# callmeray/PointMVSNet

Hardware: NVIDIA H100
Metric: PointFlow iters/sec (higher is better)
Workload: dtype f32

## Files before the change

include/pmvs_b200.h:

```cpp
#ifndef PMVS_B200_H_
#define PMVS_B200_H_

#include <stddef.h>
#include <stdint.h>

#ifdef __cplusplus
extern "C" {
#endif

#define PMVS_OK 0
#define PMVS_ERR_ARG 1
#define PMVS_ERR_CUDA 2
#define PMVS_ERR_WORKSPACE 3

#define PMVS_NUM_HYP 5
#define PMVS_FEAT_CH 136
#define PMVS_KNN 16
#define PMVS_MAX_VIEWS 12

typedef void* pmvs_stream_t;

int pmvs_version(void);
const char* pmvs_last_error(void);
unsigned long long pmvs_launch_count(void);

int pmvs_set_gemm_mode(int mode);
int pmvs_get_gemm_mode(void);

#define PMVS_OPT_EDGE 1
#define PMVS_OPT_KNN 2
#define PMVS_OPT_FETCH 3
#define PMVS_OPT_GEMM 4
#define PMVS_OPT_DEBUG_IDX 5
#define PMVS_OPT_GEMM_STRICT 6
int pmvs_set_option(int key, int value);
int pmvs_get_option(int key);

int pmvs_profile_enable(int on);
int pmvs_profile_collect(char* names, size_t names_bytes, float* ms, int max_records);

int pmvs_gather_knn_forward(const float* input, const int64_t* index, float* output,
                            int B, int C, int N, int K, pmvs_stream_t stream);
int pmvs_gather_knn_backward(const float* grad_output, const int64_t* index, float* grad_input,
                             int B, int C, int N, int K, pmvs_stream_t stream);
size_t pmvs_gather_knn_backward_det_workspace_bytes(int B, int N, int K);
int pmvs_gather_knn_backward_det(const float* grad_output, const int64_t* index, float* grad_input,
                                 int B, int C, int N, int K, void* workspace, size_t workspace_bytes,
                                 pmvs_stream_t stream);

int pmvs_knn3d(const float* xyz, int64_t* idx64, int32_t* idx32, int B, int D, int H, int W,
               int ksize, int knn, pmvs_stream_t stream);

int pmvs_feature_fetch(const float* feature_maps, const float* pts, const float* intrinsics,
                       const float* extrinsics, float* out, int B, int V, int C, int H, int W,
                       int N, pmvs_stream_t stream);
int pmvs_feature_fetch_backward(const float* grad_out, const float* pts, const float* intrinsics,
                                const float* extrinsics, float* grad_maps, int B, int V, int C,
                                int H, int W, int N, pmvs_stream_t stream);
size_t pmvs_feature_fetch_backward_det_workspace_bytes(int B, int V, int C, int H, int W, int N);
int pmvs_feature_fetch_backward_det(const float* grad_out, const float* pts, const float* intrinsics,
                                    const float* extrinsics, float* grad_maps, int B, int V, int C, int H, int W, int N,
                                    void* workspace, size_t workspace_bytes, pmvs_stream_t stream);
int pmvs_feature_fetch_taps(const float* pts, const float* intrinsics, const float* extrinsics, int64_t* texel,
                            float* weight, int B, int V, int H, int W, int N, pmvs_stream_t stream);

int pmvs_cost_volume(const float* features, const float* cam_params, float* cost, void* workspace,
                     size_t workspace_bytes, int B, int V, int C, int h, int w, int D, int is_test,
                     pmvs_stream_t stream);

size_t pmvs_cost_volume_backward_workspace_bytes(int B, int V, int C, int h, int w, int D);
int pmvs_cost_volume_backward(const float* features, const float* cam_params, const float* grad_cost,
                              float* grad_features, void* workspace, size_t workspace_bytes, int B, int V, int C,
                              int h, int w, int D, int is_test, pmvs_stream_t stream);

size_t pmvs_fuse_depth_maps_workspace_bytes(int V, int H, int W);
int pmvs_fuse_depth_maps(const float* depth, const float* cam_block, int V, int H, int W, int num_consistent,
                         float depth_thresh, float reproj_thresh, int* count_out, float* xyz_out,
                         unsigned char* used_out, void* workspace, size_t workspace_bytes, pmvs_stream_t stream);

size_t pmvs_thin_cloud_workspace_bytes(int n);
int pmvs_thin_cloud(const float* xyz, const int64_t* order, int n, float dst, float cell, int first_round, int rounds,
                    int* state, int* undecided, void* workspace, size_t workspace_bytes, pmvs_stream_t stream);
size_t pmvs_nearest_distances_workspace_bytes(int nt);
int pmvs_nearest_distances(const float* query, int nq, const float* target, int nt, float max_dist, float cell,
                           float* dist, void* workspace, size_t workspace_bytes, pmvs_stream_t stream);
int pmvs_cloud_filter(const float* xyz, int n, const float* bb, float margin, const unsigned char* obs_mask,
                      const int* mask_dims, float res, const float* plane, unsigned char* flags,
                      pmvs_stream_t stream);

typedef struct pmvs_conv_bn_weights {
  const float* weight[11];
  const float* gamma[10];
  const float* beta[10];
  const float* running_mean[10];
  const float* running_var[10];
  float eps[10];
} pmvs_conv_bn_weights;

typedef struct pmvs_conv_bn_grads {
  float* weight[11];
  float* gamma[10];
  float* beta[10];
} pmvs_conv_bn_grads;

typedef pmvs_conv_bn_weights pmvs_volume_weights;

size_t pmvs_volume_conv_workspace_bytes(int B, int in_channels, int base_channels, int D, int H, int W);
int pmvs_volume_conv(const float* x, const pmvs_volume_weights* weights, int train, float* out, double* batch_sums,
                     void* workspace, size_t workspace_bytes, int B, int in_channels, int base_channels, int D, int H,
                     int W, pmvs_stream_t stream);
int pmvs_coarse_depth(const float* filtered, const float* cams, int B, int V, int D, int H, int W, float* depth_out,
                      float* prob_out, pmvs_stream_t stream);

typedef pmvs_conv_bn_weights pmvs_image_weights;

size_t pmvs_image_conv_workspace_bytes(int B, int V, int H, int W, int base_channels);
int pmvs_image_conv(const float* img, const pmvs_image_weights* weights, int train, float* const* level_out,
                    int channels_last, double* batch_sums, void* workspace, size_t workspace_bytes, int B, int V,
                    int H, int W, int base_channels, pmvs_stream_t stream);

size_t pmvs_image_conv_keep_workspace_bytes(int B, int V, int H, int W, int base_channels);
int pmvs_image_conv_keep(const float* img, const pmvs_image_weights* weights, int train, float* const* level_out,
                         int channels_last, double* batch_sums, void* workspace, size_t workspace_bytes, int B, int V,
                         int H, int W, int base_channels, pmvs_stream_t stream);

typedef pmvs_conv_bn_grads pmvs_image_grads;

size_t pmvs_image_conv_backward_workspace_bytes(int B, int V, int H, int W, int base_channels);
int pmvs_image_conv_backward(const float* img, const pmvs_image_weights* weights, int train, const void* fwd_workspace,
                             const double* batch_sums, const float* const* grad_level, int channels_last,
                             const pmvs_image_grads* grads, void* workspace, size_t workspace_bytes, int B, int V,
                             int H, int W, int base_channels, pmvs_stream_t stream);

typedef pmvs_conv_bn_grads pmvs_volume_grads;

size_t pmvs_volume_conv_backward_workspace_bytes(int B, int in_channels, int base_channels, int D, int H, int W);
int pmvs_volume_conv_backward(const float* x, const pmvs_volume_weights* weights, int train,
                              const void* fwd_workspace, const double* batch_sums, const float* grad_out,
                              float* grad_x , const pmvs_volume_grads* grads, void* workspace,
                              size_t workspace_bytes, int B, int in_channels, int base_channels, int D, int H, int W,
                              pmvs_stream_t stream);
int pmvs_coarse_depth_backward(const float* filtered, const float* cams, const float* grad_depth,
                               float* grad_filtered, int B, int V, int D, int H, int W, pmvs_stream_t stream);

int pmvs_transpose(const float* in, float* out, int batch, int R, int C, pmvs_stream_t stream);
int pmvs_idx64_to_idx32(const int64_t* in, int32_t* out, long long n, pmvs_stream_t stream);

int pmvs_edgeconv_pm(const float* x, int ldx, const int32_t* idx32, const float* w12,
                     const float* gamma, const float* beta, float eps, int concat_central,
                     int bn_train, float* out, int ldo, float* le_scratch, double* stats_scratch,
                     int groups, int rows_per_group, int N, int K, int cin, int cout,
                     pmvs_stream_t stream);

size_t pmvs_edgeconv_pm_backward_workspace_bytes(int B, int N, int K, int cin, int cout);
int pmvs_edgeconv_pm_backward(const float* x, int ldx, const int32_t* idx32, const int64_t* idx64,
                              const float* w12, const float* gamma, const float* beta, float eps,
                              int concat_central, int bn_train, const float* le, const double* stats,
                              const float* dy, int lddy, float* dx, int lddx, float* dw12,
                              float* dgamma, float* dbeta, void* workspace, size_t workspace_bytes,
                              int B, int N, int K, int cin, int cout, pmvs_stream_t stream);

int pmvs_linear_pm(const float* x, int ldx, const float* w, float* y, int ldy, int groups,
                   int rows_per_group, int cin, int cout, const double* in_stats,
                   const float* in_gamma, const float* in_beta, double in_count, float eps,
                   double* out_stats, pmvs_stream_t stream);

typedef struct pmvs_flow_weights {
  const float* ec_w12[3];
  const float* ec_gamma[3];
  const float* ec_beta[3];
  const float* mlp_w[4];
  const float* mlp_gamma[3];
  const float* mlp_beta[3];
  float* ec_run_mean[3];
  float* ec_run_var[3];
  float* mlp_run_mean[3];
  float* mlp_run_var[3];
  float momentum;
  float eps;
  long long* ec_nbt[3];
  long long* mlp_nbt[3];
} pmvs_flow_weights;

typedef struct pmvs_flow_shape {
  int B;
  int V;
  int pyr_h[3], pyr_w[3];
  int prev_h, prev_w;
  int flow_h, flow_w;
  float image_scale;
  int ratio;
  int is_test;
  float interval_scale;
  int sub_begin, sub_count;
} pmvs_flow_shape;

size_t pmvs_point_flow_workspace_bytes(const pmvs_flow_shape* shape);

int pmvs_point_flow_iter(const pmvs_flow_shape* shape, const pmvs_flow_weights* weights,
                         const float* const pyramids_cl[3], const float* depth_prev,
                         const float* cam_params, const float* interval, const float* mean,
                         const float* std, float* depth_out, float* prob_out, void* workspace,
                         size_t workspace_bytes, pmvs_stream_t stream);

int pmvs_pyramid_to_channels_last(const float* nchw, float* nhwc, int BV, int C, int h, int w,
                                  pmvs_stream_t stream);

int pmvs_point_flow_debug_offsets(const pmvs_flow_shape* shape, size_t off[10]);

int pmvs_point_flow_debug_feature(const pmvs_flow_shape* shape, const float* depth_prev, void* workspace,
                                  pmvs_stream_t stream);

typedef struct pmvs_flow_grads {
  float* ec_dw12[3];
  float* ec_dgamma[3];
  float* ec_dbeta[3];
  float* mlp_dw[4];
  float* mlp_dgamma[3];
  float* mlp_dbeta[3];
  float* dpyramids_cl[3];
  float* ddepth_prev;
} pmvs_flow_grads;

size_t pmvs_point_flow_backward_workspace_bytes(const pmvs_flow_shape* shape);

int pmvs_point_flow_backward(const pmvs_flow_shape* shape, const pmvs_flow_weights* weights,
                             const float* const pyramids_cl[3], const float* depth_prev,
                             const float* cam_params, const float* interval, const float* mean,
                             const float* std, const void* fwd_workspace, const float* grad_depth_out,
                             const float* grad_prob_out, const pmvs_flow_grads* grads, void* workspace,
                             size_t workspace_bytes, pmvs_stream_t stream);

typedef struct pmvs_depth_terms {
  const float* pred[3];
  int h[3], w[3];
  int T;
} pmvs_depth_terms;

int pmvs_depth_loss(const pmvs_depth_terms* terms, const float* gt, int Hg, int Wg, const float* cams, int B, int V,
                    float valid_threshold, float* loss_out, float* metric_out, double* stats, pmvs_stream_t stream);
int pmvs_depth_loss_backward(const pmvs_depth_terms* terms, const float* gt, int Hg, int Wg, const float* cams, int B,
                             int V, const double* stats, const float* grad_loss, float* const grad_pred[3],
                             pmvs_stream_t stream);

#ifdef __cplusplus
}
#endif
#endif
```

pointmvsnet_b200/_lib.py:

```python
import ctypes as C
import os

import torch

_HERE = os.path.dirname(os.path.abspath(__file__))
LIB_PATH = os.path.join(_HERE, "libpmvs_b200.so")

if not os.path.exists(LIB_PATH):
    raise ImportError(
        "pointmvsnet_b200: %s is missing -- build it with pointmvsnet_b200/csrc/build.sh "
        "(nvcc, sm_90a).  There is no CPU fallback." % LIB_PATH)

lib = C.CDLL(LIB_PATH)

c_float_p = C.c_void_p
c_stream = C.c_void_p


class FlowWeights(C.Structure):
    _fields_ = [
        ("ec_w12", C.c_void_p * 3), ("ec_gamma", C.c_void_p * 3), ("ec_beta", C.c_void_p * 3),
        ("mlp_w", C.c_void_p * 4), ("mlp_gamma", C.c_void_p * 3), ("mlp_beta", C.c_void_p * 3),
        ("ec_run_mean", C.c_void_p * 3), ("ec_run_var", C.c_void_p * 3),
        ("mlp_run_mean", C.c_void_p * 3), ("mlp_run_var", C.c_void_p * 3),
        ("momentum", C.c_float), ("eps", C.c_float),
        ("ec_nbt", C.c_void_p * 3), ("mlp_nbt", C.c_void_p * 3),
    ]


class FlowShape(C.Structure):
    _fields_ = [
        ("B", C.c_int), ("V", C.c_int), ("pyr_h", C.c_int * 3), ("pyr_w", C.c_int * 3),
        ("prev_h", C.c_int), ("prev_w", C.c_int), ("flow_h", C.c_int), ("flow_w", C.c_int),
        ("image_scale", C.c_float), ("ratio", C.c_int), ("is_test", C.c_int), ("interval_scale", C.c_float),
        ("sub_begin", C.c_int), ("sub_count", C.c_int),
    ]


class FlowGrads(C.Structure):
    _fields_ = [
        ("ec_dw12", C.c_void_p * 3), ("ec_dgamma", C.c_void_p * 3), ("ec_dbeta", C.c_void_p * 3),
        ("mlp_dw", C.c_void_p * 4), ("mlp_dgamma", C.c_void_p * 3), ("mlp_dbeta", C.c_void_p * 3),
        ("dpyramids_cl", C.c_void_p * 3), ("ddepth_prev", C.c_void_p),
    ]


class ConvBnWeights(C.Structure):
    _fields_ = [
        ("weight", C.c_void_p * 11), ("gamma", C.c_void_p * 10), ("beta", C.c_void_p * 10),
        ("running_mean", C.c_void_p * 10), ("running_var", C.c_void_p * 10), ("eps", C.c_float * 10),
    ]


class ConvBnGrads(C.Structure):
    _fields_ = [("weight", C.c_void_p * 11), ("gamma", C.c_void_p * 10), ("beta", C.c_void_p * 10)]


VolumeWeights = ImageWeights = ConvBnWeights
VolumeGrads = ImageGrads = ConvBnGrads


class DepthTerms(C.Structure):
    _fields_ = [("pred", C.c_void_p * 3), ("h", C.c_int * 3), ("w", C.c_int * 3), ("T", C.c_int)]


def _sig(name, restype, argtypes):
    fn = getattr(lib, name)
    fn.restype = restype
    fn.argtypes = argtypes
    return fn


P, I, LL, F = C.c_void_p, C.c_int, C.c_longlong, C.c_float
_sig("pmvs_version", I, [])
_sig("pmvs_last_error", C.c_char_p, [])
_sig("pmvs_launch_count", C.c_ulonglong, [])
_sig("pmvs_set_gemm_mode", I, [I])
_sig("pmvs_get_gemm_mode", I, [])
_sig("pmvs_set_option", I, [I, I])
_sig("pmvs_get_option", I, [I])
_sig("pmvs_profile_enable", I, [I])
_sig("pmvs_profile_collect", I, [C.c_char_p, C.c_size_t, P, I])
_sig("pmvs_gather_knn_forward", I, [P, P, P, I, I, I, I, P])
_sig("pmvs_gather_knn_backward", I, [P, P, P, I, I, I, I, P])
_sig("pmvs_gather_knn_backward_det_workspace_bytes", C.c_size_t, [I, I, I])
_sig("pmvs_gather_knn_backward_det", I, [P, P, P, I, I, I, I, P, C.c_size_t, P])
_sig("pmvs_knn3d", I, [P, P, P, I, I, I, I, I, I, P])
_sig("pmvs_feature_fetch", I, [P, P, P, P, P, I, I, I, I, I, I, P])
_sig("pmvs_feature_fetch_backward", I, [P, P, P, P, P, I, I, I, I, I, I, P])
_sig("pmvs_feature_fetch_backward_det_workspace_bytes", C.c_size_t, [I, I, I, I, I, I])
_sig("pmvs_feature_fetch_backward_det", I, [P, P, P, P, P, I, I, I, I, I, I, P, C.c_size_t, P])
_sig("pmvs_feature_fetch_taps", I, [P, P, P, P, P, I, I, I, I, I, P])
_sig("pmvs_cost_volume", I, [P, P, P, P, C.c_size_t, I, I, I, I, I, I, I, P])
_sig("pmvs_cost_volume_backward_workspace_bytes", C.c_size_t, [I, I, I, I, I, I])
_sig("pmvs_cost_volume_backward", I, [P, P, P, P, P, C.c_size_t, I, I, I, I, I, I, I, P])
_sig("pmvs_fuse_depth_maps_workspace_bytes", C.c_size_t, [I, I, I])
_sig("pmvs_fuse_depth_maps", I, [P, P, I, I, I, I, F, F, P, P, P, P, C.c_size_t, P])
_sig("pmvs_thin_cloud_workspace_bytes", C.c_size_t, [I])
_sig("pmvs_thin_cloud", I, [P, P, I, F, F, I, I, P, P, P, C.c_size_t, P])
_sig("pmvs_nearest_distances_workspace_bytes", C.c_size_t, [I])
_sig("pmvs_nearest_distances", I, [P, I, P, I, F, F, P, P, C.c_size_t, P])
_sig("pmvs_cloud_filter", I, [P, I, P, F, P, P, F, P, P, P])
_sig("pmvs_volume_conv_workspace_bytes", C.c_size_t, [I, I, I, I, I, I])
_sig("pmvs_volume_conv", I, [P, C.POINTER(ConvBnWeights), I, P, P, P, C.c_size_t, I, I, I, I, I, I, P])
_sig("pmvs_coarse_depth", I, [P, P, I, I, I, I, I, P, P, P])
_sig("pmvs_volume_conv_backward_workspace_bytes", C.c_size_t, [I, I, I, I, I, I])
_sig("pmvs_volume_conv_backward", I, [P, C.POINTER(ConvBnWeights), I, P, P, P, P, C.POINTER(ConvBnGrads), P,
                                      C.c_size_t, I, I, I, I, I, I, P])
_sig("pmvs_coarse_depth_backward", I, [P, P, P, P, I, I, I, I, I, P])
_sig("pmvs_image_conv_workspace_bytes", C.c_size_t, [I, I, I, I, I])
_sig("pmvs_image_conv", I, [P, C.POINTER(ConvBnWeights), I, C.POINTER(C.c_void_p * 4), I, P, P, C.c_size_t, I, I, I,
                            I, I, P])
_sig("pmvs_image_conv_keep_workspace_bytes", C.c_size_t, [I, I, I, I, I])
_sig("pmvs_image_conv_keep", I, [P, C.POINTER(ConvBnWeights), I, C.POINTER(C.c_void_p * 4), I, P, P, C.c_size_t, I,
                                 I, I, I, I, P])
_sig("pmvs_image_conv_backward_workspace_bytes", C.c_size_t, [I, I, I, I, I])
_sig("pmvs_image_conv_backward", I, [P, C.POINTER(ConvBnWeights), I, P, P, C.POINTER(C.c_void_p * 4), I,
                                     C.POINTER(ConvBnGrads), P, C.c_size_t, I, I, I, I, I, P])
_sig("pmvs_transpose", I, [P, P, I, I, I, P])
_sig("pmvs_idx64_to_idx32", I, [P, P, LL, P])
_sig("pmvs_edgeconv_pm", I, [P, I, P, P, P, P, F, I, I, P, I, P, P, I, I, I, I, I, I, P])
_sig("pmvs_edgeconv_pm_backward_workspace_bytes", C.c_size_t, [I, I, I, I, I])
_sig("pmvs_edgeconv_pm_backward", I, [P, I, P, P, P, P, P, F, I, I, P, P, P, I, P, I, P, P, P, P, C.c_size_t,
                                      I, I, I, I, I, P])
_sig("pmvs_linear_pm", I, [P, I, P, P, I, I, I, I, I, P, P, P, C.c_double, F, P, P])
_sig("pmvs_point_flow_workspace_bytes", C.c_size_t, [C.POINTER(FlowShape)])
_sig("pmvs_point_flow_iter", I, [C.POINTER(FlowShape), C.POINTER(FlowWeights), C.POINTER(C.c_void_p * 3),
                                 P, P, P, P, P, P, P, P, C.c_size_t, P])
_sig("pmvs_pyramid_to_channels_last", I, [P, P, I, I, I, I, P])
_sig("pmvs_point_flow_debug_offsets", I, [C.POINTER(FlowShape), C.POINTER(C.c_size_t * 10)])
_sig("pmvs_point_flow_debug_feature", I, [C.POINTER(FlowShape), P, P, P])
_sig("pmvs_point_flow_backward_workspace_bytes", C.c_size_t, [C.POINTER(FlowShape)])
_sig("pmvs_point_flow_backward", I, [C.POINTER(FlowShape), C.POINTER(FlowWeights), C.POINTER(C.c_void_p * 3),
                                     P, P, P, P, P, P, P, P, C.POINTER(FlowGrads), P, C.c_size_t, P])
_sig("pmvs_depth_loss", I, [C.POINTER(DepthTerms), P, I, I, P, I, I, F, P, P, P, P])
_sig("pmvs_depth_loss_backward", I, [C.POINTER(DepthTerms), P, I, I, P, I, I, P, P, C.POINTER(C.c_void_p * 3), P])

EXPORTED = [
    "pmvs_version", "pmvs_last_error", "pmvs_launch_count", "pmvs_set_option", "pmvs_get_option", "pmvs_profile_enable", "pmvs_profile_collect", "pmvs_set_gemm_mode", "pmvs_get_gemm_mode", "pmvs_gather_knn_forward",
    "pmvs_gather_knn_backward", "pmvs_gather_knn_backward_det_workspace_bytes", "pmvs_gather_knn_backward_det", "pmvs_knn3d", "pmvs_feature_fetch", "pmvs_feature_fetch_backward",
    "pmvs_feature_fetch_backward_det_workspace_bytes", "pmvs_feature_fetch_backward_det", "pmvs_feature_fetch_taps",
    "pmvs_cost_volume", "pmvs_cost_volume_backward_workspace_bytes", "pmvs_cost_volume_backward",
    "pmvs_fuse_depth_maps_workspace_bytes", "pmvs_fuse_depth_maps", "pmvs_thin_cloud_workspace_bytes",
    "pmvs_thin_cloud", "pmvs_nearest_distances_workspace_bytes", "pmvs_nearest_distances", "pmvs_cloud_filter",
    "pmvs_volume_conv_workspace_bytes", "pmvs_volume_conv", "pmvs_coarse_depth",
    "pmvs_volume_conv_backward_workspace_bytes", "pmvs_volume_conv_backward", "pmvs_coarse_depth_backward",
    "pmvs_image_conv_workspace_bytes", "pmvs_image_conv", "pmvs_image_conv_keep_workspace_bytes",
    "pmvs_image_conv_keep", "pmvs_image_conv_backward_workspace_bytes", "pmvs_image_conv_backward",
    "pmvs_transpose", "pmvs_idx64_to_idx32", "pmvs_edgeconv_pm", "pmvs_edgeconv_pm_backward_workspace_bytes", "pmvs_edgeconv_pm_backward", "pmvs_linear_pm", "pmvs_point_flow_workspace_bytes",
    "pmvs_point_flow_iter", "pmvs_pyramid_to_channels_last", "pmvs_point_flow_debug_offsets",
    "pmvs_point_flow_debug_feature", "pmvs_point_flow_backward_workspace_bytes", "pmvs_point_flow_backward",
    "pmvs_depth_loss", "pmvs_depth_loss_backward",
]


def check(rc):
    if rc != 0:
        raise RuntimeError("libpmvs_b200: " + lib.pmvs_last_error().decode("utf-8", "replace"))


def stream_ptr():
    return torch.cuda.current_stream().cuda_stream


def ptr(t):
    return None if t is None else t.data_ptr()


def require_cuda(*tensors):
    for t in tensors:
        if t is not None and not t.is_cuda:
            raise RuntimeError("pointmvsnet_b200 operators need CUDA tensors (sm_90a); there is no CPU fallback")


def f32c(t):
    if t.dtype != torch.float32:
        t = t.float()
    return t.contiguous()


def workspace(nbytes, device):
    if nbytes == 0:
        check(1)
    return torch.empty(nbytes, device=device, dtype=torch.uint8)


def launch_count():
    return int(lib.pmvs_launch_count())


def profile_enable(on):
    lib.pmvs_profile_enable(1 if on else 0)


def profile_collect(max_records=65536):
    names = C.create_string_buffer(max_records * 24)
    ms = (C.c_float * max_records)()
    n = lib.pmvs_profile_collect(names, len(names), C.cast(ms, C.c_void_p), max_records)
    nm = names.value.decode().split("\n")[:n]
    return [(nm[i], float(ms[i])) for i in range(n)]


def set_gemm_mode(mode):
    check(lib.pmvs_set_gemm_mode(int(mode)))


OPTIONS = {"edge": 1, "knn": 2, "fetch": 3, "gemm": 4, "debug_idx": 5, "gemm_strict": 6}


def set_option(name, value):
    check(lib.pmvs_set_option(OPTIONS[name], int(value)))


def get_option(name):
    return int(lib.pmvs_get_option(OPTIONS[name]))


def _options_from_env():
    spec = os.environ.get("PMVS_OPTIONS", "")
    for item in spec.split(","):
        if "=" in item:
            k, v = item.split("=", 1)
            set_option(k.strip(), int(v))


_options_from_env()
```

pointmvsnet_b200/csrc/api.cu:

```cuda
#include <algorithm>
#include <atomic>
#include <cstdarg>
#include <mutex>
#include <vector>

#include "common.cuh"

namespace pmvs {

static thread_local char g_err[512] = "";
static std::atomic<unsigned long long> g_launches{0};

void set_error(const char* fmt, ...) {
  va_list ap;
  va_start(ap, fmt);
  vsnprintf(g_err, sizeof(g_err), fmt, ap);
  va_end(ap);
}
void count_launch(int n) { g_launches.fetch_add((unsigned long long)n, std::memory_order_relaxed); }

static std::atomic<int> g_opt[OPT_COUNT];
static struct OptDefaults {
  OptDefaults() {
    g_opt[OPT_EDGE].store(1);
    g_opt[OPT_KNN].store(1);
    g_opt[OPT_FETCH].store(3);
    g_opt[OPT_GEMM].store(3);
  }
} g_opt_defaults;
int opt(int key) { return (key >= 0 && key < OPT_COUNT) ? g_opt[key].load(std::memory_order_relaxed) : 0; }

struct ProfRec {
  const char* name;
  cudaEvent_t a, b;
};
static std::mutex g_prof_mu;
static std::vector<ProfRec> g_prof;
static std::atomic<int> g_prof_on{0};
static thread_local int g_prof_open = -1;

void prof_begin(const char* what, cudaStream_t st) {
  if (!g_prof_on.load(std::memory_order_relaxed)) return;
  ProfRec r;
  r.name = what;
  if (cudaEventCreate(&r.a) != cudaSuccess || cudaEventCreate(&r.b) != cudaSuccess) return;
  cudaEventRecord(r.a, st);
  std::lock_guard<std::mutex> lk(g_prof_mu);
  g_prof.push_back(r);
  g_prof_open = (int)g_prof.size() - 1;
}
void prof_end(cudaStream_t st) {
  if (g_prof_open < 0) return;
  std::lock_guard<std::mutex> lk(g_prof_mu);
  if (g_prof_open < (int)g_prof.size()) cudaEventRecord(g_prof[g_prof_open].b, st);
  g_prof_open = -1;
}

__global__ void __launch_bounds__(256) transpose_kernel(const float* __restrict__ in, float* __restrict__ out, int R,
                                                        int C) {
  __shared__ float tile[32][33];
  const size_t boff = (size_t)blockIdx.z * R * C;
  const int c0 = blockIdx.x * 32, r0 = blockIdx.y * 32;
  const int tx = threadIdx.x & 31, ty = threadIdx.x >> 5;
#pragma unroll
  for (int j = 0; j < 32; j += 8) {
    const int r = r0 + ty + j, c = c0 + tx;
    if (r < R && c < C) tile[ty + j][tx] = __ldg(in + boff + (size_t)r * C + c);
  }
  __syncthreads();
#pragma unroll
  for (int j = 0; j < 32; j += 8) {
    const int c = c0 + ty + j, r = r0 + tx;
    if (r < R && c < C) out[boff + (size_t)c * R + r] = tile[tx][ty + j];
  }
}

int launch_transpose(const float* in, float* out, int batch, int R, int C, cudaStream_t st) {
  PMVS_REQUIRE(in && out && batch > 0 && R > 0 && C > 0, "transpose: bad arguments");
  PMVS_REQUIRE(batch <= 65535 && cdiv(R, 32) <= 65535, "transpose: shape too large");
  dim3 grid(cdiv(C, 32), cdiv(R, 32), batch);
  prof_begin("transpose", st);
  transpose_kernel<<<grid, 256, 0, st>>>(in, out, R, C);
  return check_launch("transpose_kernel", st);
}

__global__ void idx_convert_kernel(const int64_t* __restrict__ in, int32_t* __restrict__ out, long long n) {
  for (long long i = blockIdx.x * (long long)blockDim.x + threadIdx.x; i < n; i += (long long)gridDim.x * blockDim.x)
    out[i] = (int32_t)in[i];
}

__global__ void __launch_bounds__(256)
    gather_fwd_kernel(const float* __restrict__ in, const int64_t* __restrict__ idx, float* __restrict__ out, int C,
                      int N, int K, long long total) {
  for (long long o = blockIdx.x * (long long)blockDim.x + threadIdx.x; o < total;
       o += (long long)gridDim.x * blockDim.x) {
    const int k = (int)(o % K);
    long long t = o / K;
    const int n = (int)(t % N);
    t /= N;
    const long long b = t / C;
    const int64_t j = idx[(b * N + n) * K + k];
    out[o] = (j >= 0 && j < N) ? __ldg(in + t * N + j) : 0.f;
  }
}
__global__ void __launch_bounds__(256)
    gather_bwd_kernel(const float* __restrict__ gout, const int64_t* __restrict__ idx, float* __restrict__ gin, int C,
                      int N, int K, long long total) {
  for (long long o = blockIdx.x * (long long)blockDim.x + threadIdx.x; o < total;
       o += (long long)gridDim.x * blockDim.x) {
    const int k = (int)(o % K);
    long long t = o / K;
    const int n = (int)(t % N);
    t /= N;
    const long long b = t / C;
    const int64_t j = idx[(b * N + n) * K + k];
    if (j >= 0 && j < N) atomicAdd(gin + t * N + j, gout[o]);
  }
}

struct FlowPlan {
  int S, hs, ws, N;
  int sub_begin;
  size_t R;
  size_t cam, feature, xyz, idx, le, ecat, h0, h1, h2, stats, total;
  size_t warp_src;
  size_t cand;
  size_t st_ec[3], st_ecn[3], st_mlp[3];
  size_t st_ticket;
  size_t stats_doubles;
  size_t coef;
};

static int make_plan(const pmvs_flow_shape* s, FlowPlan& p) {
  PMVS_REQUIRE(s != nullptr, "point_flow: NULL shape");
  PMVS_REQUIRE(s->B > 0 && s->V > 0 && s->V <= PMVS_MAX_VIEWS, "point_flow: B=%d V=%d (V <= %d)", s->B, s->V,
               PMVS_MAX_VIEWS);
  PMVS_REQUIRE(s->ratio >= 1 && s->flow_h > 0 && s->flow_w > 0, "point_flow: bad flow size / ratio");
  PMVS_REQUIRE(s->flow_h % s->ratio == 0 && s->flow_w % s->ratio == 0,
               "point_flow: flow size %dx%d not divisible by ratio %d", s->flow_h, s->flow_w, s->ratio);
  PMVS_REQUIRE(s->prev_h > 0 && s->prev_w > 0, "point_flow: bad previous depth size");
  for (int l = 0; l < 3; ++l) PMVS_REQUIRE(s->pyr_h[l] > 0 && s->pyr_w[l] > 0, "point_flow: bad pyramid size");
  PMVS_REQUIRE(s->flow_h > 1 && s->flow_w > 1, "point_flow: flow size must be > 1");
  const int s_all = s->ratio * s->ratio;
  PMVS_REQUIRE(s->sub_count >= 0 && s->sub_begin >= 0 && s->sub_begin + s->sub_count <= s_all &&
                   (s->sub_count > 0 || s->sub_begin == 0),
               "point_flow: sub-cloud range [%d, %d) outside the %d sub-clouds", s->sub_begin,
               s->sub_begin + s->sub_count, s_all);
  p.S = s->sub_count > 0 ? s->sub_count : s_all;
  p.sub_begin = s->sub_begin;
  p.hs = s->flow_h / s->ratio;
  p.ws = s->flow_w / s->ratio;
  p.N = PMVS_NUM_HYP * p.hs * p.ws;
  p.R = (size_t)p.S * s->B * p.N;
  PMVS_REQUIRE(p.R * 224 < (size_t)1 << 40, "point_flow: problem too large");
  size_t o = 0;
  p.cam = o; o += up256(cam_block_bytes(s->B, s->V));
  p.feature = o; o += up256(p.R * PMVS_FEAT_CH * 4);
  p.xyz = o; o += up256(p.R * 3 * 4);
  p.idx = o; o += up256(p.R * PMVS_KNN * 4);
  p.le = o; o += up256(p.R * 128 * 4);
  p.ecat = o; o += up256(p.R * 224 * 4);
  p.h0 = o; o += up256(p.R * 64 * 4);
  p.h1 = o; o += up256(p.R * 64 * 4);
  p.h2 = o; o += up256(p.R * 16 * 4);
  p.warp_src = o; o += up256(warp_source_bytes(s->B, s->V, s->flow_h, s->flow_w));
  p.cand = o; o += up256(p.R * PMVS_KNN * 2);
  size_t d = 0;
  const int ec_cout[3] = {32, 32, 64};
  const int mlp_cout[3] = {64, 64, 16};
  for (int l = 0; l < 3; ++l) {
    p.st_ec[l] = d; d += (size_t)p.S * 4 * ec_cout[l];
    p.st_ecn[l] = d; d += (size_t)p.S * 2 * ec_cout[l];
  }
  for (int l = 0; l < 3; ++l) { p.st_mlp[l] = d; d += (size_t)p.S * 2 * mlp_cout[l]; }
  p.st_ticket = d; d += (3 * (size_t)p.S + 1) / 2 + 1;
  p.stats_doubles = d;
  p.stats = o; o += up256(d * 8);
  p.coef = o; o += up256(3 * (size_t)p.S * 6 * 64 * sizeof(float));
  p.total = o;
  return PMVS_OK;
}

static FusedFetchParams fetch_params(const pmvs_flow_shape* s, const FlowPlan& p, char* ws, const float* depth_prev) {
  FusedFetchParams f{};
  f.src = (const float*)(ws + p.warp_src);
  f.depth_prev = depth_prev; f.cam_blocks = (const float*)(ws + p.cam); f.feature = (float*)(ws + p.feature);
  f.xyz = (float*)(ws + p.xyz);
  f.B = s->B; f.V = s->V; f.h = s->flow_h; f.w = s->flow_w; f.hp = s->prev_h; f.wp = s->prev_w;
  f.ratio = s->ratio; f.sub_begin = p.sub_begin; f.sub_count = p.S;
  return f;
}

int flow_regions(const pmvs_flow_shape* s, FlowRegions& r) {
  FlowPlan p;
  PMVS_TRY(make_plan(s, p));
  r.cam = p.cam; r.feature = p.feature; r.xyz = p.xyz; r.idx = p.idx; r.le = p.le; r.ecat = p.ecat; r.h0 = p.h0;
  r.h1 = p.h1; r.h2 = p.h2; r.warp_src = p.warp_src; r.cand = p.cand; r.stats = p.stats; r.coef = p.coef;
  r.total = p.total;
  for (int l = 0; l < 3; ++l) { r.st_ec[l] = p.st_ec[l]; r.st_ecn[l] = p.st_ecn[l]; r.st_mlp[l] = p.st_mlp[l]; }
  r.S = p.S;
  return PMVS_OK;
}

}

using namespace pmvs;

extern "C" int pmvs_version(void) { return 100; }
extern "C" const char* pmvs_last_error(void) { return g_err; }
extern "C" unsigned long long pmvs_launch_count(void) { return g_launches.load(); }

extern "C" int pmvs_set_option(int key, int value) {
  PMVS_REQUIRE(key > 0 && key < OPT_COUNT, "set_option: unknown key %d", key);
  g_opt[key].store(value);
  return PMVS_OK;
}
extern "C" int pmvs_get_option(int key) { return opt(key); }

extern "C" int pmvs_profile_enable(int on) {
  g_prof_on.store(on ? 1 : 0);
  return PMVS_OK;
}

extern "C" int pmvs_profile_collect(char* names, size_t names_bytes, float* ms, int max_records) {
  std::lock_guard<std::mutex> lk(g_prof_mu);
  int n = 0;
  size_t pos = 0;
  if (names && names_bytes) names[0] = 0;
  for (auto& r : g_prof) {
    float t = -1.f;
    if (cudaEventSynchronize(r.b) == cudaSuccess) cudaEventElapsedTime(&t, r.a, r.b);
    if (n < max_records && ms && names) {
      const size_t len = strlen(r.name);
      if (pos + len + 2 < names_bytes) {
        memcpy(names + pos, r.name, len);
        pos += len;
        names[pos++] = '\n';
        names[pos] = 0;
        ms[n++] = t;
      }
    }
    cudaEventDestroy(r.a);
    cudaEventDestroy(r.b);
  }
  g_prof.clear();
  return n;
}

extern "C" int pmvs_transpose(const float* in, float* out, int batch, int R, int C, pmvs_stream_t stream) {
  return launch_transpose(in, out, batch, R, C, (cudaStream_t)stream);
}

extern "C" int pmvs_pyramid_to_channels_last(const float* nchw, float* nhwc, int BV, int C, int h, int w,
                                             pmvs_stream_t stream) {
  PMVS_REQUIRE((long long)h * w < (1ll << 31), "pyramid_to_channels_last: plane too large");
  return launch_transpose(nchw, nhwc, BV, C, h * w, (cudaStream_t)stream);
}

extern "C" int pmvs_idx64_to_idx32(const int64_t* in, int32_t* out, long long n, pmvs_stream_t stream) {
  PMVS_REQUIRE(in && out && n >= 0, "idx64_to_idx32: bad arguments");
  if (n == 0) return PMVS_OK;
  idx_convert_kernel<<<(int)std::min<long long>(cdiv(n, 256), sm_count() * 8), 256, 0, (cudaStream_t)stream>>>(in, out, n);
  return check_launch("idx_convert_kernel");
}

extern "C" int pmvs_gather_knn_forward(const float* input, const int64_t* index, float* output, int B, int C, int N,
                                       int K, pmvs_stream_t stream) {
  PMVS_REQUIRE(B >= 0 && C >= 0 && N >= 0 && K >= 0, "gather_knn_forward: negative size");
  const long long total = (long long)B * C * N * K;
  if (total == 0) return PMVS_OK;
  PMVS_REQUIRE(input && index && output, "gather_knn_forward: NULL pointer");
  const int grid = (int)std::min<long long>(cdiv(total, 256), sm_count() * 16);
  gather_fwd_kernel<<<grid, 256, 0, (cudaStream_t)stream>>>(input, index, output, C, N, K, total);
  return check_launch("gather_fwd_kernel");
}

extern "C" int pmvs_gather_knn_backward(const float* grad_output, const int64_t* index, float* grad_input, int B,
                                        int C, int N, int K, pmvs_stream_t stream) {
  PMVS_REQUIRE(B >= 0 && C >= 0 && N >= 0 && K >= 0, "gather_knn_backward: negative size");
  if ((long long)B * C * N == 0) return PMVS_OK;
  PMVS_REQUIRE(grad_output && index && grad_input, "gather_knn_backward: NULL pointer");
  cudaStream_t st = (cudaStream_t)stream;
  PMVS_TRY(memset_async("gather_knn_backward", grad_input, (size_t)B * C * N * sizeof(float), st));
  const long long total = (long long)B * C * N * K;
  if (total == 0) return PMVS_OK;
  const int grid = (int)std::min<long long>(cdiv(total, 256), sm_count() * 16);
  gather_bwd_kernel<<<grid, 256, 0, st>>>(grad_output, index, grad_input, C, N, K, total);
  return check_launch("gather_bwd_kernel");
}

extern "C" int pmvs_edgeconv_pm(const float* x, int ldx, const int32_t* idx32, const float* w12, const float* gamma,
                                const float* beta, float eps, int concat_central, int bn_train, float* out, int ldo,
                                float* le_scratch, double* stats_scratch, int groups, int rows_per_group, int N,
                                int K, int cin, int cout, pmvs_stream_t stream) {
  PMVS_REQUIRE(x && idx32 && w12 && gamma && beta && out && le_scratch && stats_scratch, "edgeconv: NULL pointer");
  PMVS_REQUIRE(groups > 0 && rows_per_group > 0 && N > 0 && K > 0, "edgeconv: bad sizes");
  cudaStream_t st = (cudaStream_t)stream;
  if (bn_train) PMVS_TRY(memset_async("edgeconv", stats_scratch, (size_t)groups * 4 * cout * sizeof(double), st));
  GemmArgs g{};
  g.x = x; g.ldx = ldx; g.w = w12; g.y = le_scratch; g.ldy = 2 * cout;
  g.groups = groups; g.rows_per_group = rows_per_group; g.cin = cin; g.cout = 2 * cout; g.eps = eps;
  PMVS_TRY(launch_gemm(g, st));
  EdgeArgs e{};
  e.le = le_scratch; e.idx = idx32; e.stats = stats_scratch; e.gamma = gamma; e.beta = beta; e.eps = eps;
  e.concat_central = concat_central; e.out = out; e.ldo = ldo; e.groups = groups;
  e.rows_per_group = rows_per_group; e.N = N; e.K = K; e.cout = cout;
  if (bn_train) PMVS_TRY(launch_edge_stats(e, st));
  PMVS_TRY(launch_edge_apply(e, st));
  return PMVS_OK;
}

extern "C" int pmvs_linear_pm(const float* x, int ldx, const float* w, float* y, int ldy, int groups,
                              int rows_per_group, int cin, int cout, const double* in_stats, const float* in_gamma,
                              const float* in_beta, double in_count, float eps, double* out_stats,
                              pmvs_stream_t stream) {
  PMVS_REQUIRE(x && w && y, "linear_pm: NULL pointer");
  PMVS_REQUIRE(groups > 0 && rows_per_group > 0 && cin > 0 && cout > 0, "linear_pm: bad sizes");
  PMVS_REQUIRE(in_stats == nullptr || (in_gamma && in_beta && in_count > 0), "linear_pm: incomplete input BN");
  GemmArgs g{};
  g.x = x; g.ldx = ldx; g.w = w; g.y = y; g.ldy = ldy; g.groups = groups; g.rows_per_group = rows_per_group;
  g.cin = cin; g.cout = cout; g.in_stats = in_stats; g.in_gamma = in_gamma; g.in_beta = in_beta;
  g.in_count = in_count; g.eps = eps; g.out_stats = out_stats;
  return launch_gemm(g, (cudaStream_t)stream);
}

extern "C" size_t pmvs_point_flow_workspace_bytes(const pmvs_flow_shape* shape) {
  FlowPlan p;
  if (make_plan(shape, p) != PMVS_OK) return 0;
  return p.total;
}

extern "C" int pmvs_point_flow_debug_offsets(const pmvs_flow_shape* shape, size_t off[10]) {
  FlowPlan p;
  PMVS_TRY(make_plan(shape, p));
  off[0] = p.feature; off[1] = p.xyz; off[2] = p.idx; off[3] = p.ecat; off[4] = p.h2;
  off[5] = p.le; off[6] = p.stats; off[7] = p.total;
  off[8] = p.cand;
  off[9] = (opt(OPT_EDGE) == 0 || opt(OPT_DEBUG_IDX) != 0) ? 1 : 0;
  return PMVS_OK;
}

extern "C" int pmvs_point_flow_debug_feature(const pmvs_flow_shape* shape, const float* depth_prev, void* workspace,
                                             pmvs_stream_t stream) {
  FlowPlan p;
  PMVS_TRY(make_plan(shape, p));
  PMVS_REQUIRE(depth_prev && workspace, "point_flow_debug_feature: NULL pointer");
  return launch_fused_fetch(fetch_params(shape, p, (char*)workspace, depth_prev), (cudaStream_t)stream);
}

extern "C" int pmvs_point_flow_iter(const pmvs_flow_shape* shape, const pmvs_flow_weights* wts,
                                    const float* const pyramids_cl[3], const float* depth_prev,
                                    const float* cam_params, const float* interval, const float* mean,
                                    const float* stdv, float* depth_out, float* prob_out, void* workspace,
                                    size_t workspace_bytes, pmvs_stream_t stream) {
  FlowPlan p;
  PMVS_TRY(make_plan(shape, p));
  PMVS_REQUIRE(wts && pyramids_cl && depth_prev && cam_params && interval && mean && stdv && depth_out && workspace,
               "point_flow: NULL pointer");
  PMVS_TRY(check_workspace("point_flow", workspace, workspace_bytes, p.total));
  cudaStream_t st = (cudaStream_t)stream;
  char* ws = (char*)workspace;
  float* cam = (float*)(ws + p.cam);
  const float* feature = (const float*)(ws + p.feature);
  const float* xyz = (const float*)(ws + p.xyz);
  int32_t* idx = (int32_t*)(ws + p.idx);
  float* le = (float*)(ws + p.le);
  float* ecat = (float*)(ws + p.ecat);
  float* h0 = (float*)(ws + p.h0);
  float* h1 = (float*)(ws + p.h1);
  float* h2 = (float*)(ws + p.h2);
  double* stats = (double*)(ws + p.stats);
  const int B = shape->B, S = p.S;
  const int rows_per_group = B * p.N;

  PMVS_TRY(memset_async("point_flow", stats, p.stats_doubles * sizeof(double), st));
  const float kscale = shape->is_test ? shape->image_scale : (float)(4.0 * (double)shape->image_scale);
  PMVS_TRY(launch_cam_setup(cam_params, interval, mean, stdv, cam, B, shape->V, kscale, shape->interval_scale, st));

  float* warp_src = (float*)(ws + p.warp_src);
  PMVS_TRY(launch_warp_source(pyramids_cl, shape->pyr_h, shape->pyr_w, warp_src, B, shape->V, shape->flow_h,
                              shape->flow_w, st));
  const int edge_impl = opt(OPT_EDGE);
  const FusedFetchParams f = fetch_params(shape, p, ws, depth_prev);
  bool fused_le0 = false;
  if (opt(OPT_FETCH) == 3 && opt(OPT_GEMM) == 3 && pmvs_get_gemm_mode() == 3 && edge_impl != 0) {
    const int rc = launch_fetch_gemm(f, wts->ec_w12[0], le, st);
    if (rc > 0) return rc;
    fused_le0 = rc == 0;
    if (!fused_le0 && opt(OPT_GEMM_STRICT)) {
      set_error("point_flow: fetch_gemm_kernel does not take V=%d (strict mode)", shape->V);
      return PMVS_ERR_ARG;
    }
  }
  if (!fused_le0) PMVS_TRY(launch_fused_fetch(f, st));

  unsigned short* cand = (unsigned short*)(ws + p.cand);
  if (edge_impl != 0)
    PMVS_TRY(launch_knn3d_cand(xyz, opt(OPT_DEBUG_IDX) ? idx : nullptr, cand, S * B, PMVS_NUM_HYP, p.hs, p.ws, st));
  else
    PMVS_TRY(launch_knn3d(xyz, nullptr, idx, S * B, PMVS_NUM_HYP, p.hs, p.ws, PMVS_NUM_HYP, PMVS_KNN, st));

  const int cin[3] = {136, 32, 64}, cout[3] = {32, 32, 64}, in_off[3] = {0, 0, 32}, out_off[3] = {0, 32, 96};
  for (int l = 0; l < 3; ++l) {
    GemmArgs g{};
    g.x = l == 0 ? feature : ecat + in_off[l];
    g.ldx = l == 0 ? PMVS_FEAT_CH : 224;
    g.w = wts->ec_w12[l]; g.y = le; g.ldy = 2 * cout[l];
    g.groups = S; g.rows_per_group = rows_per_group; g.cin = cin[l]; g.cout = 2 * cout[l]; g.eps = wts->eps;
    if (edge_impl != 0 && l > 0) g.out_stats = stats + p.st_ec[l];
    if (l > 0 || !fused_le0) PMVS_TRY(launch_gemm(g, st));
    if (edge_impl != 0) {
      EdgeTileArgs e{};
      e.le = le; e.cand = cand; e.cstats = stats + p.st_ec[l]; e.nstats = stats + p.st_ecn[l];
      e.coef = (float*)(ws + p.coef) + (size_t)l * S * 6 * 64;
      e.ticket = (unsigned*)(stats + p.st_ticket) + (size_t)l * S;
      e.gamma = wts->ec_gamma[l]; e.beta = wts->ec_beta[l]; e.eps = wts->eps; e.concat_central = l > 0;
      e.out = ecat + out_off[l]; e.ldo = 224; e.groups = S; e.clouds_per_group = B; e.gh = p.hs; e.gw = p.ws;
      e.cout = cout[l];
      const int tile_w = edge_impl == 2 ? 16 : 8;
      PMVS_TRY(launch_edge_tile_stats(e, tile_w, st));
      PMVS_TRY(launch_edge_tile_apply(e, tile_w, st));
    } else {
      EdgeArgs e{};
      e.le = le; e.idx = idx; e.stats = stats + p.st_ec[l]; e.gamma = wts->ec_gamma[l]; e.beta = wts->ec_beta[l];
      e.eps = wts->eps; e.concat_central = l > 0; e.out = ecat + out_off[l]; e.ldo = 224; e.groups = S;
      e.rows_per_group = rows_per_group; e.N = p.N; e.K = PMVS_KNN; e.cout = cout[l];
      PMVS_TRY(launch_edge_stats(e, st));
      PMVS_TRY(launch_edge_apply(e, st));
    }
  }

  {
    const float* xin[3] = {ecat, h0, h1};
    float* yout[3] = {h0, h1, h2};
    const int mcin[3] = {224, 64, 64}, mcout[3] = {64, 64, 16};
    for (int l = 0; l < 3; ++l) {
      GemmArgs g{};
      g.x = xin[l]; g.ldx = mcin[l]; g.w = wts->mlp_w[l]; g.y = yout[l]; g.ldy = mcout[l];
      g.groups = S; g.rows_per_group = rows_per_group; g.cin = mcin[l]; g.cout = mcout[l]; g.eps = wts->eps;
      if (l > 0) {
        g.in_stats = stats + p.st_mlp[l - 1]; g.in_gamma = wts->mlp_gamma[l - 1]; g.in_beta = wts->mlp_beta[l - 1];
        g.in_count = (double)rows_per_group;
      }
      g.out_stats = stats + p.st_mlp[l];
      PMVS_TRY(launch_gemm(g, st));
    }
  }
  HeadArgs h{};
  h.h2 = h2; h.stats = stats + p.st_mlp[2]; h.gamma = wts->mlp_gamma[2]; h.beta = wts->mlp_beta[2];
  h.w3 = wts->mlp_w[3]; h.depth_prev = depth_prev; h.interval = interval; h.depth_out = depth_out;
  h.prob_out = prob_out; h.eps = wts->eps; h.interval_scale = shape->interval_scale; h.B = B; h.S = S; h.ratio = shape->ratio; h.sub_begin = p.sub_begin; h.h = shape->flow_h;
  h.w = shape->flow_w; h.hp = shape->prev_h; h.wp = shape->prev_w;
  PMVS_TRY(launch_flow_head(h, st));

  RunUpdateBatch rb{};
  rb.groups = S; rb.momentum = wts->momentum;
  for (int l = 0; l < 3; ++l) {
    if (wts->ec_run_mean[l] && wts->ec_run_var[l]) {
      const int c = cout[l];
      const double* sl = stats + p.st_ec[l];
      const bool tile = edge_impl != 0;
      if (l > 0) {
        RunUpdate& u = rb.u[rb.n++];
        u.stats = sl; u.run_mean = wts->ec_run_mean[l]; u.run_var = wts->ec_run_var[l]; u.C = c;
        u.off_sum = 0; u.off_sq = tile ? 2 * c : c; u.gstride = 4 * c; u.count = (double)rows_per_group;
        u.ncorr = (double)rows_per_group * PMVS_KNN;
      }
      RunUpdate& u = rb.u[rb.n++];
      u.run_mean = wts->ec_run_mean[l] + (l > 0 ? c : 0); u.run_var = wts->ec_run_var[l] + (l > 0 ? c : 0);
      u.C = c;
      if (tile) {
        u.stats = stats + p.st_ecn[l]; u.off_sum = 0; u.off_sq = c; u.gstride = 2 * c;
      } else {
        u.stats = sl; u.off_sum = 2 * c; u.off_sq = 3 * c; u.gstride = 4 * c;
      }
      u.count = (double)rows_per_group * PMVS_KNN;
      u.ncorr = u.count; u.nbt = wts->ec_nbt[l];
    }
  }
  const int mcout2[3] = {64, 64, 16};
  for (int l = 0; l < 3; ++l) {
    if (wts->mlp_run_mean[l] && wts->mlp_run_var[l]) {
      RunUpdate& u = rb.u[rb.n++];
      u.stats = stats + p.st_mlp[l]; u.run_mean = wts->mlp_run_mean[l]; u.run_var = wts->mlp_run_var[l];
      u.C = mcout2[l]; u.off_sum = 0; u.off_sq = mcout2[l]; u.gstride = 2 * mcout2[l];
      u.count = (double)rows_per_group; u.ncorr = u.count; u.nbt = wts->mlp_nbt[l];
    }
  }
  PMVS_TRY(launch_bn_running_update(rb, st));
  return PMVS_OK;
}
```

pointmvsnet_b200/csrc/common.cuh:

```cuda
#pragma once
#include <cuda_runtime.h>
#include <float.h>
#include <stdint.h>
#include <stdio.h>
#include <string.h>

#include "../../include/pmvs_b200.h"

namespace pmvs {

void set_error(const char* fmt, ...);
void count_launch(int n = 1);

void prof_begin(const char* what, cudaStream_t st);
void prof_end(cudaStream_t st);

inline int check_launch(const char* what, cudaStream_t st = nullptr) {
  cudaError_t e = cudaPeekAtLastError();
  if (e != cudaSuccess) {
    cudaGetLastError();
    set_error("%s: %s", what, cudaGetErrorString(e));
    return PMVS_ERR_CUDA;
  }
  prof_end(st);
  count_launch();
  return PMVS_OK;
}

#define PMVS_REQUIRE(cond, ...)     \
  do {                              \
    if (!(cond)) {                  \
      pmvs::set_error(__VA_ARGS__); \
      return PMVS_ERR_ARG;          \
    }                               \
  } while (0)

#define PMVS_TRY(expr)           \
  do {                           \
    int _rc = (expr);            \
    if (_rc != PMVS_OK) return _rc; \
  } while (0)

static inline int cdiv(long long a, long long b) { return (int)((a + b - 1) / b); }

inline size_t up256(size_t x) { return (x + 255) & ~(size_t)255; }

inline bool finite_nonneg(float t) { return t >= 0.f && t <= FLT_MAX; }

inline int check_workspace_size(const char* what, size_t bytes, size_t need) {
  if (bytes < need) {
    set_error("%s: workspace %zu bytes < required %zu", what, bytes, need);
    return PMVS_ERR_WORKSPACE;
  }
  return PMVS_OK;
}
inline int check_workspace(const char* what, const void* ws, size_t bytes, size_t need) {
  PMVS_REQUIRE(ws != nullptr && ((uintptr_t)ws & 255) == 0, "%s: workspace must be non-NULL and 256-byte aligned",
               what);
  return check_workspace_size(what, bytes, need);
}

inline int memset_async(const char* what, void* p, size_t bytes, cudaStream_t st) {
  if (bytes != 0 && cudaMemsetAsync(p, 0, bytes, st) != cudaSuccess) {
    cudaGetLastError();
    set_error("%s: cudaMemsetAsync failed", what);
    return PMVS_ERR_CUDA;
  }
  return PMVS_OK;
}

inline int sm_count() {
  static int n = 0;
  if (n == 0) {
    int dev = 0, v = 0;
    cudaGetDevice(&dev);
    n = (cudaDeviceGetAttribute(&v, cudaDevAttrMultiProcessorCount, dev) == cudaSuccess && v > 0) ? v : 132;
  }
  return n;
}

__device__ __forceinline__ float4 ldg4(const float* p) { return __ldg(reinterpret_cast<const float4*>(p)); }
__device__ __forceinline__ void st4(float* p, float4 v) { *reinterpret_cast<float4*>(p) = v; }

typedef float2 f32x2;
__device__ __forceinline__ f32x2 pack2(float a, float b) { return make_float2(a, b); }
__device__ __forceinline__ void unpack2(f32x2 v, float& a, float& b) { a = v.x; b = v.y; }
__device__ __forceinline__ f32x2 fma2(f32x2 a, f32x2 b, f32x2 c) { return make_float2(__fmaf_rn(a.x, b.x, c.x), __fmaf_rn(a.y, b.y, c.y)); }
__device__ __forceinline__ f32x2 add2(f32x2 a, f32x2 b) { return make_float2(__fadd_rn(a.x, b.x), __fadd_rn(a.y, b.y)); }
__device__ __forceinline__ f32x2 mul2(f32x2 a, f32x2 b) { return make_float2(__fmul_rn(a.x, b.x), __fmul_rn(a.y, b.y)); }
__device__ __forceinline__ f32x2 sub2(f32x2 a, f32x2 b) { return make_float2(__fsub_rn(a.x, b.x), __fsub_rn(a.y, b.y)); }

enum {
  OPT_EDGE = 1,
  OPT_KNN = 2,
  OPT_FETCH = 3,
  OPT_GEMM = 4,
  OPT_DEBUG_IDX = 5,
  OPT_GEMM_STRICT = 6,
  OPT_COUNT = 16
};
int opt(int key);

template <typename K>
inline int ensure_dyn_smem(K kernel, int bytes, unsigned long long& done_mask, const char* what) {
  int dev = 0;
  if (cudaGetDevice(&dev) != cudaSuccess || dev < 0 || dev > 63) dev = 0;
  if (done_mask & (1ull << dev)) return PMVS_OK;
  if (cudaFuncSetAttribute(kernel, cudaFuncAttributeMaxDynamicSharedMemorySize, bytes) != cudaSuccess) {
    cudaGetLastError();
    set_error("%s: cannot reserve %d bytes of shared memory", what, bytes);
    return PMVS_ERR_CUDA;
  }
  done_mask |= 1ull << dev;
  return PMVS_OK;
}

struct BnCoef {
  float mean, invstd;
};
__device__ __forceinline__ BnCoef bn_coef(double s1, double s2, double count, float eps) {
  double m = s1 / count;
  double var = s2 / count - m * m;
  if (var < 0.0) var = 0.0;
  BnCoef c;
  c.mean = (float)m;
  c.invstd = (float)(1.0 / sqrt(var + (double)eps));
  return c;
}
__device__ __forceinline__ float bn_apply(float x, float mean, float invstd, float g, float b) {
  return __fadd_rn(__fmul_rn(__fmul_rn(__fsub_rn(x, mean), invstd), g), b);
}
__device__ __forceinline__ float edge_nb_scale(float invstd, float gamma) { return __fmul_rn(invstd, gamma); }
__device__ __forceinline__ float edge_nb_offset(float mean, float local, float A, float beta) {
  return __fmaf_rn(-__fadd_rn(mean, local), A, beta);
}
__device__ __forceinline__ float edge_nb_pre(float e, float A, float c0) { return __fmaf_rn(e, A, c0); }

int launch_knn3d_cand(const float* xyz, int32_t* idx32, unsigned short* cand, int clouds, int D, int H, int W,
                      cudaStream_t st);
int launch_knn3d(const float* xyz, int64_t* idx64, int32_t* idx32, int clouds, int D, int H, int W,
                 int ksize, int knn, cudaStream_t st);
int launch_transpose(const float* in, float* out, int batch, int R, int C, cudaStream_t st);

struct GemmArgs {
  const float* x;
  int ldx;
  const float* w;
  float* y;
  int ldy;
  int groups, rows_per_group, cin, cout;
  const double* in_stats;
  const float* in_gamma;
  const float* in_beta;
  double in_count;
  float eps;
  double* out_stats;
};
int launch_gemm(const GemmArgs& a, cudaStream_t st);
int launch_gemm_tc(const GemmArgs& a, cudaStream_t st, const char* name);
int launch_gemm_ws(const GemmArgs& a, cudaStream_t st, const char* name);

struct EdgeArgs {
  const float* le;
  const int32_t* idx;
  double* stats;
  const float* gamma;
  const float* beta;
  float eps;
  int concat_central;
  float* out;
  int ldo;
  int groups, rows_per_group, N, K, cout;
};
int launch_edge_stats(const EdgeArgs& a, cudaStream_t st);
int launch_edge_apply(const EdgeArgs& a, cudaStream_t st);

size_t inv_lists_bytes(long long B, long long N, long long K);
int build_inv_lists(const int64_t* idx, int B, int N, int K, void* ws, const int** off, const int** list,
                    const char* prof_name, cudaStream_t st);
int launch_texel_sum(const int* off, const int* list, const float* rec_w, const float* g, float* out, int T, int nrec,
                     int B, int C, long long out_bstride, int out_tstride, const char* prof_name, cudaStream_t st);

struct EdgeLayerBwd {
  const float* x;
  int ldx;
  const int32_t* idx32;
  const int* inv_off;
  const int* inv_list;
  const float* w12;
  const float* gamma;
  const float* beta;
  float eps;
  int concat_central, bn_train;
  const float* le;
  const double* stats;
  const float* tile_coef;
  const float* dy;
  int lddy;
  float* dx;
  int lddx;
  float* dw12;
  float* dgamma;
  float* dbeta;
  float* dle;
  char* scratch;
  int B, N, K, cin, cout;
};
size_t edge_layer_bwd_scratch_bytes(long long R, int cin, int cout);
int edge_layer_backward(const EdgeLayerBwd& L, cudaStream_t st);
size_t weight_grad_scratch_bytes(long long R, int M2, int cin);
int launch_weight_grad(const float* dy, const float* x, int ldx, int cin, int M2, int R, float* wpart, float* dw,
                       const char* simt_name, cudaStream_t st);

struct EdgeTileArgs {
  const float* le;
  const unsigned short* cand;
  const double* cstats;
  double* nstats;
  float* coef;
  unsigned* ticket;
  const float* gamma;
  const float* beta;
  float eps;
  int concat_central;
  float* out;
  int ldo;
  int groups, clouds_per_group, gh, gw, cout;
};
int launch_edge_tile_stats(const EdgeTileArgs& a, int tile_w, cudaStream_t st);
int launch_edge_tile_apply(const EdgeTileArgs& a, int tile_w, cudaStream_t st);

struct FusedFetchParams {
  const float* src;
  const float* depth_prev;
  const float* cam_blocks;
  float* feature;
  float* xyz;
  int B, V, h, w, hp, wp, ratio;
  int sub_begin, sub_count;
  int ppw, hs, ws, rlog2;
};
int launch_warp_source(const float* const pyr[3], const int hl[3], const int wl[3], float* out, int B, int V, int h,
                       int w, cudaStream_t st);
size_t warp_source_bytes(int B, int V, int h, int w);
int launch_cam_setup(const float* cam_params, const float* interval, const float* mean, const float* stdv,
                     float* blocks, int B, int V, float kscale, float iscale, cudaStream_t st);
int launch_fused_fetch(const FusedFetchParams& p, cudaStream_t st);
int launch_fetch_gemm(const FusedFetchParams& p, const float* w12, float* le, cudaStream_t st);
size_t cam_block_bytes(int B, int V);
int cost_volume_check_shape(const char* what, int B, int V, int C, int h, int w, int D);
struct FetchBwdParams {
  FusedFetchParams f;
  const float* ddepth_out;
  float* ddup;
  float* dfv;
  int64_t* rec_idx;
  float* rec_w;
};
int launch_fetch_backward(const FetchBwdParams& p, cudaStream_t st);
int launch_warp_source_backward(const float* dsrc, const int hl[3], const int wl[3], float* const dpyr[3], int B, int V,
                                int h, int w, cudaStream_t st);

struct HeadArgs {
  const float* h2;
  const double* stats;
  const float* gamma;
  const float* beta;
  const float* w3;
  const float* depth_prev;
  const float* interval;
  float* depth_out;
  float* prob_out;
  float eps, interval_scale;
  int B, S, ratio, h, w, hp, wp;
  int sub_begin;
};
int launch_flow_head(const HeadArgs& a, cudaStream_t st);
struct FlowRegions {
  size_t cam, feature, xyz, idx, le, ecat, h0, h1, h2, warp_src, cand, stats, coef, total;
  size_t st_ec[3], st_ecn[3], st_mlp[3];
  int S;
};
int flow_regions(const pmvs_flow_shape* s, FlowRegions& r);
bool gemm_in_bn_fma_form(const GemmArgs& a);

struct RunUpdate {
  const double* stats;
  float* run_mean;
  float* run_var;
  int C, off_sum, off_sq, gstride;
  double count;
  double ncorr;
  long long* nbt;
};
struct RunUpdateBatch {
  RunUpdate u[9];
  int n, groups;
  float momentum;
};
int launch_bn_running_update(const RunUpdateBatch& rb, cudaStream_t st);

}
```

pointmvsnet_b200/csrc/edge_tile.cu:

```cuda
#include <algorithm>

#include "common.cuh"
#include "tensor_map.cuh"

namespace pmvs {

namespace {

constexpr int ET_THREADS = 256;
constexpr int ET_WARPS = ET_THREADS / 32;
constexpr int ET_CP = 32;
constexpr int ET_LPP = ET_CP / 4;
constexpr int ET_PPW = 32 / ET_LPP;

__device__ __forceinline__ unsigned smem_u32(const void* p) { return (unsigned)__cvta_generic_to_shared(p); }

template <int TX, int TY>
struct TileGeom {
  static constexpr int HX = TX + 4, HY = TY + 4;
  static constexpr int ROWS = PMVS_NUM_HYP * HY * HX;
  static constexpr int NPTS = PMVS_NUM_HYP * TY * TX;
  static constexpr int BYTES = ROWS * ET_CP * 4;
  static constexpr int SMEM = BYTES;
};

constexpr int ET_COEF = 6;

template <int COUT, bool APPLY, int TX, int TY>
__global__ void __launch_bounds__(ET_THREADS, 3) edge_tile_kernel(const __grid_constant__ CUtensorMap tm,
                                                                   const EdgeTileArgs a) {
  using G = TileGeom<TX, TY>;
  static_assert(COUT % ET_CP == 0, "edge_tile: channels must be a multiple of 32");
  static_assert(G::NPTS % (ET_WARPS * ET_PPW) == 0, "edge_tile: every thread owns NPTS / 32 points");
  constexpr int LD = 2 * COUT;
  constexpr int SLABS = COUT / ET_CP;
  constexpr int STEPS = G::NPTS / (ET_WARPS * ET_PPW);
  static_assert(G::HX == 12 && G::HY == 8, "the kNN kernel's 16-bit codes are row offsets of a 12 x 8 x 5 halo tile");
  extern __shared__ __align__(128) float halo[];
  __shared__ __align__(8) unsigned long long bar;
  __shared__ float part[APPLY ? 1 : ET_WARPS][APPLY ? 1 : 2 * ET_CP];
  __shared__ __align__(16) float coef[APPLY ? ET_COEF * COUT : 4];
  __shared__ int s_last;

  const int g = blockIdx.z;
  const int tid = threadIdx.x, warp = tid >> 5, lane = tid & 31;
  const int sub = lane / ET_LPP, cl = (lane % ET_LPP) * 4;
  const int gh = a.gh, gw = a.gw;
  const int tiles_x = (gw + TX - 1) / TX, tiles_per_cloud = tiles_x * ((gh + TY - 1) / TY);
  const int tiles_per_group = tiles_per_cloud * a.clouds_per_group;
  const int HW = gh * gw, N = PMVS_NUM_HYP * HW;
  const int rows_per_group = a.clouds_per_group * N;
  const unsigned bar_addr = smem_u32(&bar);

  if (tid == 0) {
    asm volatile("mbarrier.init.shared::cta.b64 [%0], 1;" ::"r"(bar_addr));
    asm volatile("fence.mbarrier_init.release.cluster;" ::: "memory");
  }
  if (APPLY) {
    const float* cg = a.coef + (size_t)g * ET_COEF * COUT;
    for (int c = tid; c < ET_COEF * COUT; c += ET_THREADS) coef[c] = __ldg(cg + c);
  }
  static_assert(TX * TY == ET_WARPS * ET_PPW && STEPS == PMVS_NUM_HYP, "edge_tile: one layer of the tile per step");
  const int tq = warp * ET_PPW + sub, tx = tq % TX, ty = tq / TX;
  const int pb0 = ((-2 * G::HY + ty) * G::HX + tx) * ET_CP + cl;
  constexpr int LAYER = G::HY * G::HX * ET_CP;
  __syncthreads();

  unsigned loads = 0;
#pragma unroll 1
  for (int slab = 0; slab < SLABS; ++slab) {
    const int ch0 = slab * ET_CP;
    f32x2 n1_lo = pack2(0.f, 0.f), n1_hi = n1_lo, n2_lo = n1_lo, n2_hi = n1_lo;
#pragma unroll 1
    for (int tile = blockIdx.x; tile < tiles_per_group; tile += gridDim.x) {
    const int b = tile / tiles_per_cloud, tr = tile - b * tiles_per_cloud;
    const int y0 = (tr / tiles_x) * TY, x0 = (tr % tiles_x) * TX;
    const size_t cloud_base = (size_t)g * rows_per_group + (size_t)b * N;
    const bool ok = y0 + ty < gh && x0 + tx < gw;
    const int pq = (y0 + ty) * gw + x0 + tx;
    auto load_codes = [&](int s, uint4& c0, uint4& c1) {
      if (ok) {
        const uint4* cp = reinterpret_cast<const uint4*>(a.cand + (cloud_base + (size_t)(s * HW + pq)) * PMVS_KNN);
        c0 = __ldg(cp);
        c1 = __ldg(cp + 1);
      } else {
        c0 = c1 = make_uint4(0u, 0u, 0u, 0u);
      }
    };
    if (loads > 0) __syncthreads();
    if (tid == 0) {
      asm volatile("mbarrier.arrive.expect_tx.shared::cta.b64 _, [%0], %1;" ::"r"(bar_addr), "r"((unsigned)G::BYTES)
                   : "memory");
      asm volatile(
          "cp.async.bulk.tensor.4d.shared::cluster.global.mbarrier::complete_tx::bytes [%0], [%1, {%2, %3, %4, %5}], [%6];"
          ::"r"(smem_u32(halo)), "l"(&tm), "r"(COUT + ch0), "r"(x0 - 2), "r"(y0 - 2),
          "r"((g * a.clouds_per_group + b) * PMVS_NUM_HYP), "r"(bar_addr)
          : "memory");
    }
    float4 loc[STEPS];
#pragma unroll
    for (int s = 0; s < STEPS; ++s)
      loc[s] = ok ? ldg4(a.le + (cloud_base + (size_t)(s * HW + pq)) * LD + ch0 + cl) : make_float4(0.f, 0.f, 0.f, 0.f);
    {
      unsigned done = 0;
      const unsigned parity = loads & 1u;
      while (!done) {
        asm volatile(
            "{\n\t.reg .pred p;\n\t"
            "mbarrier.try_wait.parity.shared::cta.b64 p, [%1], %2;\n\t"
            "selp.u32 %0, 1, 0, p;\n\t}"
            : "=r"(done)
            : "r"(bar_addr), "r"(parity)
            : "memory");
      }
      ++loads;
    }

    uint4 nx0, nx1;
    load_codes(0, nx0, nx1);
#pragma unroll
    for (int s = 0; s < STEPS; ++s) {
      const uint4 ca = nx0, cb = nx1;
      if (s + 1 < STEPS) load_codes(s + 1, nx0, nx1);
      if (!ok) continue;
      const int n = s * HW + pq;
      const size_t row = cloud_base + (size_t)n;
      const float4 lc = loc[s];
      const bool esc = ((ca.x | ca.y | ca.z | ca.w | cb.x | cb.y | cb.z | cb.w) & 0x80008000u) != 0u;
      const float* hbase = halo + pb0 + s * LAYER;
      f32x2 o_lo = pack2(0.f, 0.f), o_hi = o_lo, A_lo = o_lo, A_hi = o_lo, c_lo = o_lo, c_hi = o_lo;
      const f32x2 l_lo = pack2(lc.x, lc.y), l_hi = pack2(lc.z, lc.w);
      if (APPLY) {
        const float4 A4 = *reinterpret_cast<const float4*>(&coef[ch0 + cl]);
        const float4 B4 = *reinterpret_cast<const float4*>(&coef[COUT + ch0 + cl]);
        A_lo = pack2(A4.x, A4.y); A_hi = pack2(A4.z, A4.w);
        c_lo = pack2(fmaf(-lc.x, A4.x, B4.x), fmaf(-lc.y, A4.y, B4.y));
        c_hi = pack2(fmaf(-lc.z, A4.z, B4.z), fmaf(-lc.w, A4.w, B4.w));
      }
      auto body = [&](const float4 e) {
        const f32x2 e_lo = pack2(e.x, e.y), e_hi = pack2(e.z, e.w);
        if (APPLY) {
          float t0, t1f, t2, t3;
          unpack2(fma2(e_lo, A_lo, c_lo), t0, t1f);
          unpack2(fma2(e_hi, A_hi, c_hi), t2, t3);
          o_lo = add2(o_lo, pack2(fmaxf(t0, 0.f), fmaxf(t1f, 0.f)));
          o_hi = add2(o_hi, pack2(fmaxf(t2, 0.f), fmaxf(t3, 0.f)));
        } else {
          const f32x2 d_lo = sub2(e_lo, l_lo), d_hi = sub2(e_hi, l_hi);
          n1_lo = add2(n1_lo, d_lo); n1_hi = add2(n1_hi, d_hi);
          n2_lo = fma2(d_lo, d_lo, n2_lo); n2_hi = fma2(d_hi, d_hi, n2_hi);
        }
      };
      auto code_of = [&](int k) -> unsigned {
        const int wq = k >> 1;
        const unsigned wd = wq == 0 ? ca.x : wq == 1 ? ca.y : wq == 2 ? ca.z : wq == 3 ? ca.w
                          : wq == 4 ? cb.x : wq == 5 ? cb.y : wq == 6 ? cb.z : cb.w;
        return (k & 1) ? wd >> 16 : wd & 0xffffu;
      };
      if (!esc) {
#pragma unroll
        for (int k = 0; k < PMVS_KNN; ++k) body(*reinterpret_cast<const float4*>(hbase + code_of(k) * ET_CP));
      } else {
#pragma unroll 1
        for (int k = 0; k < PMVS_KNN; ++k) {
          const unsigned c = code_of(k);
          if (c & 0x8000u) {
            const int j = (int)(c & 127u);
            int t = n + (j / 25 - 2) * HW + ((j % 25) / 5 - 2) * gw + (j % 5 - 2);
            t = t < 0 ? 0 : (t > N - 1 ? N - 1 : t);
            body(ldg4(a.le + (cloud_base + (size_t)t) * LD + COUT + ch0 + cl));
          } else {
            body(*reinterpret_cast<const float4*>(hbase + c * ET_CP));
          }
        }
      }
      if (APPLY) {
        float4 o;
        unpack2(o_lo, o.x, o.y);
        unpack2(o_hi, o.z, o.w);
        float* orow = a.out + row * a.ldo;
        if (a.concat_central) {
          const float4 m = *reinterpret_cast<const float4*>(&coef[2 * COUT + ch0 + cl]);
          const float4 is = *reinterpret_cast<const float4*>(&coef[3 * COUT + ch0 + cl]);
          const float4 gm = *reinterpret_cast<const float4*>(&coef[4 * COUT + ch0 + cl]);
          const float4 bt = *reinterpret_cast<const float4*>(&coef[5 * COUT + ch0 + cl]);
          float4 c;
          c.x = fmaxf(bn_apply(lc.x, m.x, is.x, gm.x, bt.x), 0.f);
          c.y = fmaxf(bn_apply(lc.y, m.y, is.y, gm.y, bt.y), 0.f);
          c.z = fmaxf(bn_apply(lc.z, m.z, is.z, gm.z, bt.z), 0.f);
          c.w = fmaxf(bn_apply(lc.w, m.w, is.w, gm.w, bt.w), 0.f);
          st4(orow + ch0 + cl, c);
          orow += COUT;
        }
        constexpr float rk = 1.f / (float)PMVS_KNN;
        static_assert(PMVS_KNN == 16, "mean over K uses an exact power-of-two reciprocal");
        st4(orow + ch0 + cl, make_float4(__fmul_rn(o.x, rk), __fmul_rn(o.y, rk), __fmul_rn(o.z, rk), __fmul_rn(o.w, rk)));
      }
    }

    }

    if (!APPLY) {
      float v[8];
      unpack2(n1_lo, v[0], v[1]); unpack2(n1_hi, v[2], v[3]);
      unpack2(n2_lo, v[4], v[5]); unpack2(n2_hi, v[6], v[7]);
#pragma unroll
      for (int off = ET_LPP; off < 32; off <<= 1) {
#pragma unroll
        for (int q = 0; q < 8; ++q) v[q] += __shfl_xor_sync(0xffffffffu, v[q], off);
      }
      if (sub == 0) {
#pragma unroll
        for (int q = 0; q < 8; ++q) part[warp][(q >> 2) * ET_CP + cl + (q & 3)] = v[q];
      }
      __syncthreads();
      double* o = a.nstats + (size_t)g * 2 * COUT;
      if (tid < 2 * ET_CP) {
        double t = 0.0;
#pragma unroll
        for (int wq = 0; wq < ET_WARPS; ++wq) t += (double)part[wq][tid];
        atomicAdd(o + (tid / ET_CP) * COUT + ch0 + (tid % ET_CP), t);
      }
    }
  }

  if (!APPLY) {
    __threadfence();
    __syncthreads();
    if (tid == 0) {
      const unsigned t = atomicAdd(a.ticket + g, 1u);
      s_last = t == gridDim.x - 1;
    }
    __syncthreads();
    if (s_last) {
      __threadfence();
      const double* sc = a.cstats + (size_t)g * 4 * COUT;
      const double* sn = a.nstats + (size_t)g * 2 * COUT;
      float* cg = a.coef + (size_t)g * ET_COEF * COUT;
      const double cnt_c = (double)rows_per_group, cnt_n = (double)rows_per_group * PMVS_KNN;
      for (int c = tid; c < COUT; c += ET_THREADS) {
        const BnCoef kn = bn_coef(__ldcg(sn + c), __ldcg(sn + COUT + c), cnt_n, a.eps);
        const int gn = a.concat_central ? COUT + c : c;
        const float A = kn.invstd * a.gamma[gn];
        cg[c] = A;
        cg[COUT + c] = fmaf(-kn.mean, A, a.beta[gn]);
        if (a.concat_central) {
          const BnCoef kc = bn_coef(sc[c], sc[2 * COUT + c], cnt_c, a.eps);
          cg[2 * COUT + c] = kc.mean; cg[3 * COUT + c] = kc.invstd; cg[4 * COUT + c] = a.gamma[c]; cg[5 * COUT + c] = a.beta[c];
        }
      }
    }
  }
}

template <int COUT, bool APPLY, int TX, int TY>
int launch_variant(const EdgeTileArgs& a, cudaStream_t st) {
  using G = TileGeom<TX, TY>;
  EncodeTiledFn enc = encode_tiled_fn();
  if (enc == nullptr) {
    set_error("edge_tile: cuTensorMapEncodeTiled is not available from this driver");
    return PMVS_ERR_CUDA;
  }
  const int N = PMVS_NUM_HYP * a.gh * a.gw;
  const long long layers = (long long)a.groups * a.clouds_per_group * PMVS_NUM_HYP;
  PMVS_REQUIRE(a.groups <= 65535 && a.clouds_per_group <= 65535, "edge_tile: too many clouds");
  PMVS_REQUIRE(layers < (1ll << 31) && (long long)a.groups * a.clouds_per_group * N < (1ll << 40), "edge_tile: too large");
  PMVS_REQUIRE(((uintptr_t)a.le & 15) == 0, "edge_tile: LE must be 16-byte aligned");
  CUtensorMap tm;
  const cuuint64_t gdim[4] = {(cuuint64_t)(2 * COUT), (cuuint64_t)a.gw, (cuuint64_t)a.gh, (cuuint64_t)layers};
  const cuuint64_t gstr[3] = {(cuuint64_t)(2 * COUT) * 4, (cuuint64_t)a.gw * 2 * COUT * 4,
                              (cuuint64_t)a.gh * a.gw * 2 * COUT * 4};
  const cuuint32_t box[4] = {ET_CP, (cuuint32_t)G::HX, (cuuint32_t)G::HY, PMVS_NUM_HYP};
  const cuuint32_t estr[4] = {1, 1, 1, 1};
  const CUresult r = enc(&tm, CU_TENSOR_MAP_DATA_TYPE_FLOAT32, 4, const_cast<float*>(a.le), gdim, gstr, box, estr,
                         CU_TENSOR_MAP_INTERLEAVE_NONE, CU_TENSOR_MAP_SWIZZLE_NONE, CU_TENSOR_MAP_L2_PROMOTION_L2_128B,
                         CU_TENSOR_MAP_FLOAT_OOB_FILL_NONE);
  if (r != CUDA_SUCCESS) {
    set_error("edge_tile: cuTensorMapEncodeTiled failed (%d) for %dx%d, cout %d", (int)r, a.gh, a.gw, COUT);
    return PMVS_ERR_CUDA;
  }
  static unsigned long long smem_done = 0;
  PMVS_TRY(ensure_dyn_smem(edge_tile_kernel<COUT, APPLY, TX, TY>, G::SMEM, smem_done, "edge_tile"));
  static int slots = 0;
  if (slots == 0) {
    slots = 3 * sm_count();
  }
  const int tiles_per_group = cdiv(a.gw, TX) * cdiv(a.gh, TY) * a.clouds_per_group;
  int ctas = APPLY ? tiles_per_group : std::min(tiles_per_group, std::max(1, slots / a.groups));
  ctas = cdiv(tiles_per_group, cdiv(tiles_per_group, ctas));
  PMVS_REQUIRE(ctas <= 0x7fffffff / 2, "edge_tile: too many tiles");
  dim3 grid(ctas, 1, a.groups);
  static const char* const names[2][2] = {{"edge_stats_32", "edge_stats_64"}, {"edge_apply_32", "edge_apply_64"}};
  prof_begin(names[APPLY ? 1 : 0][COUT == 32 ? 0 : 1], st);
  edge_tile_kernel<COUT, APPLY, TX, TY><<<grid, ET_THREADS, G::SMEM, st>>>(tm, a);
  return check_launch(APPLY ? "edge_tile_apply_kernel" : "edge_tile_stats_kernel", st);
}

template <bool APPLY>
int launch_edge_tile(const EdgeTileArgs& a, int tile_w, cudaStream_t st) {
  PMVS_REQUIRE(a.le && a.cand && a.cstats && a.nstats && a.gamma && a.beta && a.coef && a.ticket && (!APPLY || a.out),
               "edge_tile: NULL pointer");
  PMVS_REQUIRE(a.cout == 32 || a.cout == 64, "edge_tile: out_channels %d (supported: 32, 64)", a.cout);
  PMVS_REQUIRE(a.gh > 0 && a.gw > 0 && a.groups > 0 && a.clouds_per_group > 0, "edge_tile: bad cloud shape");
  (void)tile_w;
  return a.cout == 32 ? launch_variant<32, APPLY, 8, 4>(a, st) : launch_variant<64, APPLY, 8, 4>(a, st);
}

}

int launch_edge_tile_stats(const EdgeTileArgs& a, int tile_w, cudaStream_t st) {
  return launch_edge_tile<false>(a, tile_w, st);
}
int launch_edge_tile_apply(const EdgeTileArgs& a, int tile_w, cudaStream_t st) {
  return launch_edge_tile<true>(a, tile_w, st);
}

}
```

pointmvsnet_b200/csrc/flow_bwd.cu:

```cuda
#include <algorithm>

#include "common.cuh"

namespace pmvs {

namespace {

constexpr int FB_ROWS = 128;
constexpr int HEAD_THREADS = 256;

__global__ void __launch_bounds__(256) flow_idx_kernel(const unsigned short* __restrict__ cand,
                                                       const int32_t* __restrict__ idx_in, int32_t* __restrict__ idx32,
                                                       int64_t* __restrict__ idx64, long long total, int N, int HW, int W) {
  const long long e = (long long)blockIdx.x * blockDim.x + threadIdx.x;
  if (e >= total) return;
  int t;
  if (cand != nullptr) {
    const int c = cand[e];
    const bool out = (c & 0x8000) != 0;
    const int j = c & 127;
    const int dd = (out ? j / 25 : c / 96) - 2, dh = (out ? (j % 25) / 5 : (c % 96) / 12) - 2,
              dw = (out ? j % 5 : c % 12) - 2;
    const int n = (int)((e / PMVS_KNN) % N);
    t = n + dd * HW + dh * W + dw;
    t = t < 0 ? 0 : (t > N - 1 ? N - 1 : t);
  } else {
    t = idx_in[e];
  }
  idx32[e] = t;
  idx64[e] = t;
}

__global__ void __launch_bounds__(HEAD_THREADS) head_bwd_kernel(const HeadArgs a, const float* __restrict__ dprob,
                                                                const float* __restrict__ ddepth, float* __restrict__ dA,
                                                                float* __restrict__ part) {
  __shared__ float cm[16], ci[16], cg[16], cb[16], cw[16];
  __shared__ float red[HEAD_THREADS / 32][16];
  const int P = a.h * a.w, N = PMVS_NUM_HYP * P;
  if (threadIdx.x < 16) {
    BnCoef k = bn_coef(a.stats[threadIdx.x], a.stats[16 + threadIdx.x], (double)a.B * N, a.eps);
    cm[threadIdx.x] = k.mean; ci[threadIdx.x] = k.invstd;
    cg[threadIdx.x] = a.gamma[threadIdx.x]; cb[threadIdx.x] = a.beta[threadIdx.x]; cw[threadIdx.x] = a.w3[threadIdx.x];
  }
  __syncthreads();
  const int t = blockIdx.x * blockDim.x + threadIdx.x;
  float dw[16];
#pragma unroll
  for (int c = 0; c < 16; ++c) dw[c] = 0.f;
  if (t < a.B * P) {
    const int b = t / P, pp = t - b * P;
    float act[PMVS_NUM_HYP][16], raw[PMVS_NUM_HYP];
#pragma unroll
    for (int m = 0; m < PMVS_NUM_HYP; ++m) {
      const float* hrow = a.h2 + ((size_t)b * N + (size_t)m * P + pp) * 16;
      float acc = 0.f;
#pragma unroll
      for (int q = 0; q < 4; ++q) {
        const float4 v = ldg4(hrow + q * 4);
        const float vv[4] = {v.x, v.y, v.z, v.w};
#pragma unroll
        for (int r = 0; r < 4; ++r) {
          const int c = q * 4 + r;
          act[m][c] = fmaxf(bn_apply(vv[r], cm[c], ci[c], cg[c], cb[c]), 0.f);
          acc = fmaf(act[m][c], cw[c], acc);
        }
      }
      raw[m] = acc;
    }
    float mx = -raw[0];
#pragma unroll
    for (int m = 1; m < PMVS_NUM_HYP; ++m) mx = fmaxf(mx, -raw[m]);
    float e[PMVS_NUM_HYP], sum = 0.f;
#pragma unroll
    for (int m = 0; m < PMVS_NUM_HYP; ++m) {
      e[m] = expf(-raw[m] - mx);
      sum += e[m];
    }
    const float itv = __fmul_rn(a.interval_scale, a.interval[b]);
    const float gd = ddepth[(size_t)b * P + pp];
    float pr[PMVS_NUM_HYP], dpr[PMVS_NUM_HYP], s = 0.f;
#pragma unroll
    for (int m = 0; m < PMVS_NUM_HYP; ++m) {
      pr[m] = __fdiv_rn(e[m], sum);
      dpr[m] = __fmul_rn(gd, __fmul_rn((float)(m - 2), itv));
      if (dprob) dpr[m] = __fadd_rn(dpr[m], dprob[((size_t)b * PMVS_NUM_HYP + m) * P + pp]);
      s = fmaf(pr[m], dpr[m], s);
    }
#pragma unroll
    for (int m = 0; m < PMVS_NUM_HYP; ++m) {
      const float draw = -__fmul_rn(pr[m], __fsub_rn(dpr[m], s));
      float* drow = dA + ((size_t)b * N + (size_t)m * P + pp) * 16;
#pragma unroll
      for (int q = 0; q < 4; ++q)
        st4(drow + 4 * q, make_float4(__fmul_rn(draw, cw[4 * q]), __fmul_rn(draw, cw[4 * q + 1]),
                                      __fmul_rn(draw, cw[4 * q + 2]), __fmul_rn(draw, cw[4 * q + 3])));
#pragma unroll
      for (int c = 0; c < 16; ++c) dw[c] = fmaf(draw, act[m][c], dw[c]);
    }
  }
#pragma unroll
  for (int off = 16; off > 0; off >>= 1)
#pragma unroll
    for (int c = 0; c < 16; ++c) dw[c] += __shfl_xor_sync(0xffffffffu, dw[c], off);
  if ((threadIdx.x & 31) == 0)
#pragma unroll
    for (int c = 0; c < 16; ++c) red[threadIdx.x >> 5][c] = dw[c];
  __syncthreads();
  if (threadIdx.x < 16) {
    float v = 0.f;
    for (int wq = 0; wq < HEAD_THREADS / 32; ++wq) v += red[wq][threadIdx.x];
    part[(size_t)blockIdx.x * 16 + threadIdx.x] = v;
  }
}

__global__ void __launch_bounds__(256) ordered_sum_kernel(const float* __restrict__ part, float* __restrict__ out, int n,
                                                          int parts) {
  const int i = blockIdx.x * blockDim.x + threadIdx.x;
  if (i >= n) return;
  double s = 0.0;
  for (int q = 0; q < parts; ++q) s += (double)__ldg(part + (size_t)q * n + i);
  out[i] = (float)s;
}

struct MlpBn {
  const float* h;
  const double* stats;
  const float* gamma;
  const float* beta;
  double count;
  float eps;
  int fma_form;
  int R, C;
};
struct MlpCoef {
  float mean, istd, A, B;
};
__device__ __forceinline__ MlpCoef mlp_coef(const MlpBn& a, int c) {
  const BnCoef k = bn_coef(a.stats[c], a.stats[a.C + c], a.count, a.eps);
  MlpCoef o;
  o.mean = k.mean; o.istd = k.invstd;
  o.A = __fmul_rn(k.invstd, a.gamma[c]);
  o.B = fmaf(-k.mean, o.A, a.beta[c]);
  return o;
}
__device__ __forceinline__ float mlp_pre(const MlpBn& a, const MlpCoef& k, float x, int c) {
  return a.fma_form ? fmaf(x, k.A, k.B) : bn_apply(x, k.mean, k.istd, a.gamma[c], a.beta[c]);
}

__global__ void __launch_bounds__(256) mlp_act_kernel(const MlpBn a, float* __restrict__ out) {
  const long long e = (long long)blockIdx.x * blockDim.x + threadIdx.x;
  if (e >= (long long)a.R * a.C) return;
  const int c = (int)(e % a.C);
  out[e] = fmaxf(mlp_pre(a, mlp_coef(a, c), a.h[e], c), 0.f);
}

__global__ void __launch_bounds__(256) mlp_bwd_stats_kernel(const MlpBn a, const float* __restrict__ dA,
                                                            double* __restrict__ part) {
  __shared__ float red[256][2];
  const int C = a.C, slots = 256 / C, c = threadIdx.x % C, slot = threadIdx.x / C;
  const MlpCoef k = mlp_coef(a, c);
  float s1 = 0.f, s2 = 0.f;
  const int r0 = blockIdx.x * FB_ROWS;
  for (int r = r0 + slot; r < min(r0 + FB_ROWS, a.R); r += slots) {
    const float x = a.h[(size_t)r * C + c];
    const float g = mlp_pre(a, k, x, c) > 0.f ? dA[(size_t)r * C + c] : 0.f;
    s1 += g;
    s2 = fmaf(g, __fmul_rn(__fsub_rn(x, k.mean), k.istd), s2);
  }
  red[threadIdx.x][0] = s1;
  red[threadIdx.x][1] = s2;
  __syncthreads();
  if (threadIdx.x < C) {
    double t1 = 0.0, t2 = 0.0;
    for (int q = 0; q < slots; ++q) {
      t1 += (double)red[q * C + threadIdx.x][0];
      t2 += (double)red[q * C + threadIdx.x][1];
    }
    part[(size_t)blockIdx.x * 2 * C + threadIdx.x] = t1;
    part[(size_t)blockIdx.x * 2 * C + C + threadIdx.x] = t2;
  }
}

__global__ void __launch_bounds__(256) mlp_bwd_finish_kernel(const double* __restrict__ part, int ctas, int C,
                                                             double count, float* __restrict__ dgamma,
                                                             float* __restrict__ dbeta, float* __restrict__ coef) {
  __shared__ double red[256];
  __shared__ double sums[2];
  const int c = blockIdx.x, tid = threadIdx.x;
  for (int q = 0; q < 2; ++q) {
    double t = 0.0;
    for (int i = tid; i < ctas; i += 256) t += part[(size_t)i * 2 * C + q * C + c];
    red[tid] = t;
    __syncthreads();
    for (int s = 128; s > 0; s >>= 1) {
      if (tid < s) red[tid] += red[tid + s];
      __syncthreads();
    }
    if (tid == 0) sums[q] = red[0];
    __syncthreads();
  }
  if (tid != 0) return;
  dbeta[c] = (float)sums[0];
  dgamma[c] = (float)sums[1];
  coef[2 * c] = (float)(sums[0] / count);
  coef[2 * c + 1] = (float)(sums[1] / count);
}

__global__ void __launch_bounds__(256) mlp_bwd_apply_kernel(const MlpBn a, const float* __restrict__ dA,
                                                            const float* __restrict__ coef, float* __restrict__ dh) {
  const long long e = (long long)blockIdx.x * blockDim.x + threadIdx.x;
  if (e >= (long long)a.R * a.C) return;
  const int c = (int)(e % a.C);
  const MlpCoef k = mlp_coef(a, c);
  const float x = a.h[e];
  const float g = mlp_pre(a, k, x, c) > 0.f ? dA[e] : 0.f;
  const float xh = __fmul_rn(__fsub_rn(x, k.mean), k.istd);
  dh[e] = __fmul_rn(k.A, __fsub_rn(__fsub_rn(g, coef[2 * c]), __fmul_rn(xh, coef[2 * c + 1])));
}

__global__ void __launch_bounds__(256) add_cols_kernel(float* __restrict__ y, int ldy, const float* __restrict__ x, int n,
                                                       long long R) {
  const long long e = (long long)blockIdx.x * blockDim.x + threadIdx.x;
  if (e >= R * (n / 4)) return;
  const long long r = e / (n / 4);
  const int c = (int)(e % (n / 4)) * 4;
  float4 v = ldg4(x + r * n + c);
  float* yp = y + r * ldy + c;
  const float4 o = *reinterpret_cast<const float4*>(yp);
  st4(yp, make_float4(__fadd_rn(o.x, v.x), __fadd_rn(o.y, v.y), __fadd_rn(o.z, v.z), __fadd_rn(o.w, v.w)));
}

__global__ void __launch_bounds__(256) nearest_bwd_kernel(const float* __restrict__ ddup, float* __restrict__ dprev,
                                                          int B, int h, int w, int hp, int wp) {
  const long long e = (long long)blockIdx.x * blockDim.x + threadIdx.x;
  if (e >= (long long)B * hp * wp) return;
  const int b = (int)(e / ((long long)hp * wp)), r = (int)(e % ((long long)hp * wp));
  const int yp = r / wp, xp = r - yp * wp;
  const float nsy = (float)hp / (float)h, nsx = (float)wp / (float)w;
  auto near = [](int o, float s, int n) {
    const int i = (int)floorf((float)o * s);
    return i < n - 1 ? i : n - 1;
  };
  const int ylo = max((int)floorf((float)yp / nsy) - 2, 0);
  const int yhi = yp == hp - 1 ? h - 1 : min((int)ceilf((float)(yp + 1) / nsy) + 1, h - 1);
  const int xlo = max((int)floorf((float)xp / nsx) - 2, 0);
  const int xhi = xp == wp - 1 ? w - 1 : min((int)ceilf((float)(xp + 1) / nsx) + 1, w - 1);
  float acc = 0.f;
  for (int Y = ylo; Y <= yhi; ++Y) {
    if (near(Y, nsy, hp) != yp) continue;
    for (int X = xlo; X <= xhi; ++X)
      if (near(X, nsx, wp) == xp) acc = __fadd_rn(acc, ddup[((size_t)b * h + Y) * w + X]);
  }
  dprev[e] = acc;
}

struct BwdFlowPlan {
  size_t R, npix, nrec;
  int N, head_ctas, mlp_ctas;
  size_t idx32, idx64, inv, f0, xyz, le, dle, decat, dtmp, df0, dA, dh, act, st4, wt, layer, wpart, hpart, mpart, mcoef;
  size_t ddup, dfv, rec_idx, rec_w, rec_inv, dsrc, total;
};

int bwd_flow_plan(const pmvs_flow_shape* s, BwdFlowPlan& p) {
  PMVS_REQUIRE(s != nullptr, "point_flow_backward: NULL shape");
  PMVS_REQUIRE(s->ratio == 1 && s->sub_count == 0 && s->sub_begin == 0,
               "point_flow_backward: only one cloud per call (ratio 1, no sub_count); got ratio %d, sub_count %d",
               s->ratio, s->sub_count);
  PMVS_REQUIRE(pmvs_point_flow_workspace_bytes(s) != 0, "%s", pmvs_last_error());
  p.N = PMVS_NUM_HYP * s->flow_h * s->flow_w;
  p.R = (size_t)s->B * p.N;
  p.npix = (size_t)s->B * s->flow_h * s->flow_w;
  p.nrec = p.npix * PMVS_NUM_HYP * s->V * 4;
  PMVS_REQUIRE(p.R * PMVS_KNN < ((size_t)1 << 31) && p.nrec < ((size_t)1 << 31) &&
                   (size_t)s->B * (p.nrec / 4 + 1) < ((size_t)1 << 31),
               "point_flow_backward: problem too large");
  p.head_ctas = cdiv((long long)p.npix, HEAD_THREADS);
  p.mlp_ctas = cdiv((long long)p.R, FB_ROWS);
  const long long R = (long long)p.R;
  size_t lay = 0;
  const int cin[3] = {136, 32, 64}, cout[3] = {32, 32, 64};
  for (int l = 0; l < 3; ++l) lay = std::max(lay, edge_layer_bwd_scratch_bytes(R, cin[l], cout[l]));
  size_t wp = weight_grad_scratch_bytes(R, 64, 224);
  wp = std::max(wp, weight_grad_scratch_bytes(R, 64, 64));
  wp = std::max(wp, weight_grad_scratch_bytes(R, 16, 64));
  size_t o = 0;
  p.idx32 = o; o += up256(p.R * PMVS_KNN * 4);
  p.idx64 = o; o += up256(p.R * PMVS_KNN * 8);
  p.inv = o; o += up256(inv_lists_bytes(s->B, p.N, PMVS_KNN));
  p.f0 = o; o += up256(p.R * PMVS_FEAT_CH * 4);
  p.xyz = o; o += up256(p.R * 3 * 4);
  p.le = o; o += up256(p.R * 128 * 4);
  p.dle = o; o += up256(p.R * 128 * 4);
  p.decat = o; o += up256(p.R * 224 * 4);
  p.dtmp = o; o += up256(p.R * 64 * 4);
  p.df0 = o; o += up256(p.R * PMVS_FEAT_CH * 4);
  p.dA = o; o += up256(p.R * 64 * 4);
  p.dh = o; o += up256(p.R * 64 * 4);
  p.act = o; o += up256(p.R * 64 * 4);
  p.st4 = o; o += up256(3 * 4 * 64 * 8);
  p.wt = o; o += up256(224 * 64 * 4);
  p.layer = o; o += up256(lay);
  p.wpart = o; o += up256(wp);
  p.hpart = o; o += up256((size_t)p.head_ctas * 16 * 4);
  p.mpart = o; o += up256((size_t)p.mlp_ctas * 2 * 64 * 8);
  p.mcoef = o; o += up256(2 * 64 * 4);
  p.ddup = o; o += up256(p.npix * 4);
  p.dfv = o; o += up256(p.nrec / 4 * 112 * 4);
  p.rec_idx = o; o += up256(p.nrec * 8);
  p.rec_w = o; o += up256(p.nrec * 4);
  p.rec_inv = o; o += up256(inv_lists_bytes(s->B, (long long)(p.nrec / 4 / s->B), 4));
  p.dsrc = o; o += up256(warp_source_bytes(s->B, s->V, s->flow_h, s->flow_w));
  p.total = o;
  return PMVS_OK;
}

int mlp_layer_backward(const MlpBn& a, const float* dA, float* dh, double* part, float* coef, float* dgamma,
                       float* dbeta, int ctas, cudaStream_t st) {
  prof_begin("mlp_bwd_stats", st);
  mlp_bwd_stats_kernel<<<ctas, 256, 0, st>>>(a, dA, part);
  PMVS_TRY(check_launch("mlp_bwd_stats_kernel", st));
  prof_begin("mlp_bwd_finish", st);
  mlp_bwd_finish_kernel<<<a.C, 256, 0, st>>>(part, ctas, a.C, a.count, dgamma, dbeta, coef);
  PMVS_TRY(check_launch("mlp_bwd_finish_kernel", st));
  prof_begin("mlp_bwd_apply", st);
  mlp_bwd_apply_kernel<<<cdiv((long long)a.R * a.C, 256), 256, 0, st>>>(a, dA, coef, dh);
  return check_launch("mlp_bwd_apply_kernel", st);
}

int mlp_act(const MlpBn& a, float* out, cudaStream_t st) {
  prof_begin("mlp_bwd_act", st);
  mlp_act_kernel<<<cdiv((long long)a.R * a.C, 256), 256, 0, st>>>(a, out);
  return check_launch("mlp_act_kernel", st);
}

int contract_dx(const float* dy, int cout, const float* w, int cin, float* wt, float* dx, int ldx, int R, float eps,
                cudaStream_t st) {
  PMVS_TRY(launch_transpose(w, wt, 1, cout, cin, st));
  GemmArgs g{};
  g.x = dy; g.ldx = cout; g.w = wt; g.y = dx; g.ldy = ldx;
  g.groups = 1; g.rows_per_group = R; g.cin = cout; g.cout = cin; g.eps = eps;
  return launch_gemm(g, st);
}

int add_cols(float* y, int ldy, const float* x, int n, long long R, cudaStream_t st) {
  prof_begin("flow_bwd_add", st);
  add_cols_kernel<<<cdiv(R * (n / 4), 256), 256, 0, st>>>(y, ldy, x, n, R);
  return check_launch("add_cols_kernel", st);
}

}

}

using namespace pmvs;

extern "C" size_t pmvs_point_flow_backward_workspace_bytes(const pmvs_flow_shape* shape) {
  BwdFlowPlan p;
  if (bwd_flow_plan(shape, p) != PMVS_OK) return 0;
  return p.total;
}

extern "C" int pmvs_point_flow_backward(const pmvs_flow_shape* shape, const pmvs_flow_weights* wts,
                                        const float* const pyramids_cl[3], const float* depth_prev,
                                        const float* cam_params, const float* interval, const float* mean,
                                        const float* stdv, const void* fwd_workspace, const float* grad_depth_out,
                                        const float* grad_prob_out, const pmvs_flow_grads* grads, void* workspace,
                                        size_t workspace_bytes, pmvs_stream_t stream) {
  BwdFlowPlan p;
  PMVS_TRY(bwd_flow_plan(shape, p));
  PMVS_REQUIRE(wts && pyramids_cl && depth_prev && cam_params && interval && mean && stdv && fwd_workspace &&
                   grad_depth_out && grads && workspace,
               "point_flow_backward: NULL pointer");
  for (int l = 0; l < 3; ++l)
    PMVS_REQUIRE(grads->ec_dw12[l] && grads->ec_dgamma[l] && grads->ec_dbeta[l] && grads->mlp_dw[l] &&
                     grads->mlp_dgamma[l] && grads->mlp_dbeta[l] && pyramids_cl[l],
                 "point_flow_backward: NULL pointer");
  PMVS_REQUIRE(grads->mlp_dw[3] != nullptr, "point_flow_backward: NULL pointer");
  PMVS_REQUIRE(((uintptr_t)fwd_workspace & 255) == 0, "point_flow_backward: fwd_workspace must be 256-byte aligned");
  PMVS_TRY(check_workspace("point_flow_backward", workspace, workspace_bytes, p.total));
  (void)cam_params; (void)mean; (void)stdv;
  FlowRegions fr;
  PMVS_TRY(flow_regions(shape, fr));
  const bool gather = opt(OPT_EDGE) == 0;
  cudaStream_t st = (cudaStream_t)stream;
  const char* fw = (const char*)fwd_workspace;
  char* ws = (char*)workspace;
  const int B = shape->B, N = p.N, R = (int)p.R, h = shape->flow_h, w = shape->flow_w;
  const float eps = wts->eps;
  const float* ecat = (const float*)(fw + fr.ecat);
  const float* h0 = (const float*)(fw + fr.h0);
  const float* h1 = (const float*)(fw + fr.h1);
  const float* h2 = (const float*)(fw + fr.h2);
  const float* le2 = (const float*)(fw + fr.le);
  const double* stats = (const double*)(fw + fr.stats);
  const float* fcoef = (const float*)(fw + fr.coef);
  const float* warp_src = (const float*)(fw + fr.warp_src);
  const float* cam_blocks = (const float*)(fw + fr.cam);
  const int ec_cout[3] = {32, 32, 64}, ec_cin[3] = {136, 32, 64}, mlp_cout[3] = {64, 64, 16}, mlp_cin[3] = {224, 64, 64};
  const size_t* st_ec = fr.st_ec;
  const size_t* st_ecn = fr.st_ecn;
  const size_t* st_mlp = fr.st_mlp;

  auto F = [&](size_t o) { return (float*)(ws + o); };
  double* part = (double*)(ws + p.mpart);
  float* mcoef = F(p.mcoef);
  const bool need_fetch = grads->ddepth_prev || grads->dpyramids_cl[0] || grads->dpyramids_cl[1] ||
                          grads->dpyramids_cl[2];
  const bool need_pyr = grads->dpyramids_cl[0] || grads->dpyramids_cl[1] || grads->dpyramids_cl[2];

  HeadArgs ha{};
  ha.h2 = h2; ha.stats = stats + st_mlp[2]; ha.gamma = wts->mlp_gamma[2]; ha.beta = wts->mlp_beta[2];
  ha.w3 = wts->mlp_w[3]; ha.interval = interval; ha.eps = eps; ha.interval_scale = shape->interval_scale;
  ha.B = B; ha.S = 1; ha.ratio = 1; ha.h = h; ha.w = w;
  prof_begin("head_bwd", st);
  head_bwd_kernel<<<p.head_ctas, HEAD_THREADS, 0, st>>>(ha, grad_prob_out, grad_depth_out, F(p.dA), F(p.hpart));
  PMVS_TRY(check_launch("head_bwd_kernel", st));
  prof_begin("head_bwd_reduce", st);
  ordered_sum_kernel<<<1, 256, 0, st>>>(F(p.hpart), grads->mlp_dw[3], 16, p.head_ctas);
  PMVS_TRY(check_launch("ordered_sum_kernel", st));

  {
    const float* hs[3] = {h0, h1, h2};
    auto bn = [&](int l, int fma_form) {
      MlpBn a{};
      a.h = hs[l]; a.stats = stats + st_mlp[l]; a.gamma = wts->mlp_gamma[l]; a.beta = wts->mlp_beta[l];
      a.count = (double)R; a.eps = eps; a.fma_form = fma_form; a.R = R; a.C = mlp_cout[l];
      return a;
    };
    auto consumer_fma = [&](int l) {
      if (l == 2) return 0;
      GemmArgs g{};
      g.x = hs[l]; g.ldx = mlp_cout[l]; g.w = wts->mlp_w[l + 1]; g.y = (float*)hs[l + 1]; g.ldy = mlp_cout[l + 1];
      g.groups = 1; g.rows_per_group = R; g.cin = mlp_cin[l + 1]; g.cout = mlp_cout[l + 1];
      return gemm_in_bn_fma_form(g) ? 1 : 0;
    };
    float* dA = F(p.dA);
    float* dh = F(p.dh);
    for (int l = 2; l >= 0; --l) {
      const MlpBn a = bn(l, consumer_fma(l));
      PMVS_TRY(mlp_layer_backward(a, dA, dh, part, mcoef, grads->mlp_dgamma[l], grads->mlp_dbeta[l], p.mlp_ctas, st));
      const float* x = ecat;
      if (l > 0) {
        PMVS_TRY(mlp_act(bn(l - 1, consumer_fma(l - 1)), F(p.act), st));
        x = F(p.act);
      }
      PMVS_TRY(launch_weight_grad(dh, x, mlp_cin[l], mlp_cin[l], mlp_cout[l], R, F(p.wpart), grads->mlp_dw[l],
                                  "mlp_bwd_wgrad_simt", st));
      PMVS_TRY(contract_dx(dh, mlp_cout[l], wts->mlp_w[l], mlp_cin[l], F(p.wt), l > 0 ? dA : F(p.decat), mlp_cin[l],
                           R, eps, st));
    }
  }

  {
    const long long total = (long long)p.R * PMVS_KNN;
    prof_begin("flow_bwd_idx", st);
    flow_idx_kernel<<<cdiv(total, 256), 256, 0, st>>>(gather ? nullptr : (const unsigned short*)(fw + fr.cand),
                                                     gather ? (const int32_t*)(fw + fr.idx) : nullptr,
                                                     (int32_t*)(ws + p.idx32), (int64_t*)(ws + p.idx64), total, N,
                                                     h * w, w);
    PMVS_TRY(check_launch("flow_idx_kernel", st));
  }
  const int* inv_off = nullptr;
  const int* inv_list = nullptr;
  PMVS_TRY(build_inv_lists((const int64_t*)(ws + p.idx64), B, N, PMVS_KNN, ws + p.inv, &inv_off, &inv_list,
                           "flow_bwd_lists", st));
  FusedFetchParams ff{};
  ff.src = warp_src; ff.depth_prev = depth_prev; ff.cam_blocks = cam_blocks; ff.feature = F(p.f0); ff.xyz = F(p.xyz);
  ff.B = B; ff.V = shape->V; ff.h = h; ff.w = w; ff.hp = shape->prev_h; ff.wp = shape->prev_w; ff.ratio = 1;
  ff.sub_begin = 0; ff.sub_count = 1;
  PMVS_TRY(launch_fused_fetch(ff, st));

  {
    const int in_off[3] = {0, 0, 32}, out_off[3] = {0, 32, 96};
    double* st4 = (double*)(ws + p.st4);
    for (int l = 2; l >= 0; --l) {
      const int c = ec_cout[l];
      double* s4 = st4 + (size_t)l * 4 * 64;
      if (gather) {
        if (cudaMemcpyAsync(s4, stats + st_ec[l], 4 * c * sizeof(double), cudaMemcpyDeviceToDevice, st) != cudaSuccess) {
          set_error("point_flow_backward: copy failed");
          return PMVS_ERR_CUDA;
        }
      } else {
        const double* cs = stats + st_ec[l];
        const double* ns = stats + st_ecn[l];
        const double* srcs[4] = {cs, cs + 2 * c, ns, ns + c};
        for (int q = (l > 0 ? 0 : 2); q < 4; ++q)
          if (cudaMemcpyAsync(s4 + q * c, srcs[q], c * sizeof(double), cudaMemcpyDeviceToDevice, st) != cudaSuccess) {
            set_error("point_flow_backward: copy failed");
            return PMVS_ERR_CUDA;
          }
      }
      const float* x = l == 0 ? F(p.f0) : ecat + in_off[l];
      const int ldx = l == 0 ? PMVS_FEAT_CH : 224;
      const float* le = le2;
      if (l < 2) {
        GemmArgs g{};
        g.x = x; g.ldx = ldx; g.w = wts->ec_w12[l]; g.y = F(p.le); g.ldy = 2 * c;
        g.groups = 1; g.rows_per_group = R; g.cin = ec_cin[l]; g.cout = 2 * c; g.eps = eps;
        PMVS_TRY(launch_gemm(g, st));
        le = F(p.le);
      }
      EdgeLayerBwd L{};
      L.x = x; L.ldx = ldx; L.idx32 = (const int32_t*)(ws + p.idx32); L.inv_off = inv_off; L.inv_list = inv_list;
      L.w12 = wts->ec_w12[l]; L.gamma = wts->ec_gamma[l]; L.beta = wts->ec_beta[l]; L.eps = eps;
      L.concat_central = l > 0; L.bn_train = 1; L.le = le; L.stats = s4;
      L.tile_coef = gather ? nullptr : fcoef + (size_t)l * 6 * 64;
      L.dy = F(p.decat) + out_off[l]; L.lddy = 224;
      L.dx = l > 0 ? F(p.dtmp) : (need_fetch ? F(p.df0) : nullptr);
      L.lddx = l > 0 ? ec_cin[l] : PMVS_FEAT_CH;
      L.dw12 = grads->ec_dw12[l]; L.dgamma = grads->ec_dgamma[l]; L.dbeta = grads->ec_dbeta[l];
      L.dle = F(p.dle); L.scratch = ws + p.layer; L.B = B; L.N = N; L.K = PMVS_KNN; L.cin = ec_cin[l]; L.cout = c;
      PMVS_TRY(edge_layer_backward(L, st));
      if (l > 0) PMVS_TRY(add_cols(F(p.decat) + in_off[l], 224, F(p.dtmp), ec_cin[l], R, st));
    }
  }
  if (!need_fetch) return PMVS_OK;

  FetchBwdParams fb{};
  fb.f = ff;
  fb.f.feature = F(p.df0);
  fb.ddepth_out = grad_depth_out; fb.ddup = F(p.ddup);
  fb.dfv = need_pyr ? F(p.dfv) : nullptr;
  fb.rec_idx = (int64_t*)(ws + p.rec_idx); fb.rec_w = F(p.rec_w);
  PMVS_TRY(launch_fetch_backward(fb, st));
  if (grads->ddepth_prev) {
    const long long n = (long long)B * shape->prev_h * shape->prev_w;
    prof_begin("nearest_bwd", st);
    nearest_bwd_kernel<<<cdiv(n, 256), 256, 0, st>>>(F(p.ddup), grads->ddepth_prev, B, h, w, shape->prev_h,
                                                     shape->prev_w);
    PMVS_TRY(check_launch("nearest_bwd_kernel", st));
  }
  if (need_pyr) {
    const int T = shape->V * h * w, nrec = (int)(p.nrec / B);
    const int* roff = nullptr;
    const int* rlist = nullptr;
    PMVS_TRY(build_inv_lists((const int64_t*)(ws + p.rec_idx), B, nrec / 4, 4, ws + p.rec_inv, &roff, &rlist,
                             "flow_bwd_tap_lists", st));
    PMVS_TRY(launch_texel_sum(roff, rlist, F(p.rec_w), F(p.dfv), F(p.dsrc), T, nrec, B, 112, (long long)(T + 1) * 112,
                              112, "texel_sum", st));
    PMVS_TRY(launch_warp_source_backward(F(p.dsrc), shape->pyr_h, shape->pyr_w, grads->dpyramids_cl, B, shape->V, h,
                                         w, st));
  }
  return PMVS_OK;
}
```

pointmvsnet_b200/csrc/gemm_ws.cu:

```cuda
#include <algorithm>
#include <type_traits>

#include "common.cuh"
#include "tensor_map.cuh"
#include "wgmma.cuh"

namespace pmvs {

namespace ws {

using namespace wg;

constexpr int NT = 128;
constexpr int KC = 32;
constexpr int PLANE_BYTES = NT * KC * 4;
constexpr int STAGE_BYTES = 2 * PLANE_BYTES;
constexpr int CONS_WARPS = 8, CONS_THREADS = CONS_WARPS * 32;
constexpr int PROD_WARPS = 8, PROD_WARP0 = CONS_WARPS, PROD_THREADS = PROD_WARPS * 32;
constexpr int THREADS = CONS_THREADS + PROD_THREADS;
constexpr int A_LD = NT * 8 / PROD_THREADS;
static_assert(A_LD * PROD_THREADS == NT * 8, "the producers share a chunk evenly");
constexpr int MAXK = 224;
constexpr int SMEM_MAX = 227 * 1024;

template <int ASYNC, int NSTAGES>
struct Layout {
  static constexpr int NST = NSTAGES;
  static constexpr int RING = 0;
  static constexpr int STAGING = RING + NST * STAGE_BYTES;
  static constexpr int W = STAGING + ASYNC * PLANE_BYTES;
};
__host__ __device__ constexpr int weight_bytes(int cout, int nch) { return nch * 2 * cout * 128; }
constexpr int TAIL_BN = 0, TAIL_RED = TAIL_BN + 2 * MAXK * 4;
__host__ __device__ constexpr int tail_bar(int cout) { return TAIL_RED + 2 * cout * 8; }
__host__ __device__ constexpr int tail_bytes(int cout) { return tail_bar(cout) + 128; }

__device__ __forceinline__ void sts128(uint32_t addr, float4 v) {
  asm volatile("st.shared.v4.f32 [%0], {%1, %2, %3, %4};" ::"r"(addr), "f"(v.x), "f"(v.y), "f"(v.z), "f"(v.w) : "memory");
}
__device__ __forceinline__ float4 lds128(uint32_t addr) {
  float4 v;
  asm volatile("ld.shared.v4.f32 {%0, %1, %2, %3}, [%4];" : "=f"(v.x), "=f"(v.y), "=f"(v.z), "=f"(v.w) : "r"(addr) : "memory");
  return v;
}

struct TileRange {
  int first, count;
};
__device__ __forceinline__ TileRange my_tiles(int total) {
  const long long G = gridDim.x, b = blockIdx.x;
  const int lo = (int)(b * total / G), hi = (int)((b + 1) * total / G);
  return TileRange{lo, hi - lo};
}

template <int COUT, bool IN_BN, int ASYNC, int NSTAGES>
__global__ void __launch_bounds__(THREADS, 1) gemm_ws_kernel(const GemmArgs a) {
  using LY = Layout<ASYNC, NSTAGES>;
  constexpr int STAGES = LY::NST;
  constexpr int SM_RING = LY::RING, SM_STAGING = LY::STAGING, SM_W = LY::W;
  constexpr int PF = ASYNC > 0 ? ASYNC - 1 : 4;
  constexpr bool STACKED = COUT <= 64;
  constexpr int W_CHUNK = 2 * COUT * 128;
  extern __shared__ __align__(1024) unsigned char smem[];
  const uint32_t smem_base = smem_u32(smem);

  const int K = a.cin;
  const int nch = (K + KC - 1) / KC;
  const int tid = threadIdx.x, warp = __shfl_sync(0xffffffffu, tid >> 5, 0), lane = tid & 31;
  const int tpg = (a.rows_per_group + NT - 1) / NT;
  const TileRange tr = my_tiles(a.groups * tpg);

  unsigned char* tail = smem + SM_W + weight_bytes(COUT, nch);
  float* sBN = (float*)(tail + TAIL_BN);
  double* sRed = (double*)(tail + TAIL_RED);
  const uint32_t bar0 = smem_u32(tail + tail_bar(COUT));
  auto bar_full = [&](int s) { return bar0 + 8u * (uint32_t)s; };
  auto bar_empty = [&](int s) { return bar0 + 8u * (uint32_t)(STAGES + s); };

  if (tid == 0) {
    for (int s = 0; s < STAGES; ++s) {
      mbar_init(bar_full(s), PROD_WARPS);
      mbar_init(bar_empty(s), CONS_WARPS);
    }
    asm volatile("fence.mbarrier_init.release.cluster;" ::: "memory");
  }
  for (int i = tid; i < 2 * COUT; i += THREADS) sRed[i] = 0.0;
  for (int e = tid; e < COUT * nch * 8; e += THREADS) {
    const int n = e / (nch * 8), rem = e - n * (nch * 8), c = rem >> 3, pc = rem & 7;
    const int k0 = c * KC + pc * 4;
    const float4 v = k0 < K ? ldg4(a.w + (size_t)n * K + k0) : make_float4(0.f, 0.f, 0.f, 0.f);
    float4 hi, lo;
    hi.x = tf32_hi(v.x); hi.y = tf32_hi(v.y); hi.z = tf32_hi(v.z); hi.w = tf32_hi(v.w);
    lo.x = __fsub_rn(v.x, hi.x); lo.y = __fsub_rn(v.y, hi.y); lo.z = __fsub_rn(v.z, hi.z); lo.w = __fsub_rn(v.w, hi.w);
    const uint32_t dst = smem_base + SM_W + c * W_CHUNK + swz128(n, pc);
    sts128(dst, hi);
    sts128(dst + COUT * 128, lo);
  }
  fence_proxy_async();
  __syncthreads();

  if (warp >= PROD_WARP0) {
    const int ptid = tid - PROD_WARP0 * 32;
    const int pc = ptid & 7;
    const int prow = ptid >> 3;
    constexpr int ROWS_STEP = PROD_THREADS / 8;
    const int total = tr.count * nch;
    int cur_g = -1;
    float4 buf[ASYNC > 0 ? 1 : PF + 1][A_LD];
    int soff[A_LD];
#pragma unroll
    for (int i = 0; i < A_LD; ++i) {
      const int r = prow + ROWS_STEP * i;
      soff[i] = swz128(r, pc);
    }

    struct Cursor {
      int g, row0, c;
      const float* ptr;
    };
    Cursor ci, cp;
    {
      const int t0 = tr.first;
      ci.g = t0 / tpg; ci.row0 = (t0 - ci.g * tpg) * NT; ci.c = 0;
      ci.ptr = a.x + ((size_t)ci.g * a.rows_per_group + ci.row0 + prow) * a.ldx + pc * 4;
      cp = ci;
    }
    const bool last_kvalid = (nch - 1) * KC + pc * 4 < K;
    const size_t tile_step = (size_t)NT * a.ldx - (size_t)(nch - 1) * KC;
    int n_issued = 0;
    auto issue = [&](float4 (&xa)[A_LD]) {
      const int rows_valid = a.rows_per_group - ci.row0;
      const bool kvalid = ci.c != nch - 1 || last_kvalid;
#pragma unroll
      for (int i = 0; i < A_LD; ++i) {
        const int r = prow + ROWS_STEP * i;
        const bool ok = kvalid && r < rows_valid;
        if (ASYNC > 0) {
          const uint32_t dst = smem_base + SM_STAGING + (n_issued % (ASYNC > 0 ? ASYNC : 1)) * PLANE_BYTES + (ptid + PROD_THREADS * i) * 16;
          const float* src = ok ? ci.ptr + (size_t)(ROWS_STEP * i) * a.ldx : a.x;
          asm volatile("cp.async.cg.shared.global [%0], [%1], 16, %2;" ::"r"(dst), "l"(src), "r"(ok ? 16 : 0) : "memory");
        } else {
          xa[i] = ok ? ldg4(ci.ptr + (size_t)(ROWS_STEP * i) * a.ldx) : make_float4(0.f, 0.f, 0.f, 0.f);
        }
      }
      ++n_issued;
      if (++ci.c == nch) {
        ci.c = 0;
        ci.row0 += NT;
        ci.ptr += tile_step;
        if (ci.row0 >= a.rows_per_group) {
          ci.row0 = 0;
          ++ci.g;
          ci.ptr = a.x + ((size_t)ci.g * a.rows_per_group + prow) * a.ldx + pc * 4;
        }
      } else {
        ci.ptr += KC;
      }
    };
    auto advance = [&](Cursor& cu) {
      if (++cu.c == nch) {
        cu.c = 0;
        cu.row0 += NT;
        if (cu.row0 >= a.rows_per_group) {
          cu.row0 = 0;
          ++cu.g;
        }
      }
    };
    auto put = [&](const float4 (&xa)[A_LD], int n) {
      const int k0 = cp.c * KC + pc * 4;
      if (IN_BN) {
        const int g = cp.g;
        if (g != cur_g) {
          named_bar_sync(1, PROD_THREADS);
          const double* s = a.in_stats + (size_t)g * 2 * K;
          for (int cc = ptid; cc < K; cc += PROD_THREADS) {
            const BnCoef k = bn_coef(s[cc], s[K + cc], a.in_count, a.eps);
            const float A = __fmul_rn(k.invstd, a.in_gamma[cc]);
            sBN[cc] = A;
            sBN[MAXK + cc] = fmaf(-k.mean, A, a.in_beta[cc]);
          }
          named_bar_sync(1, PROD_THREADS);
          cur_g = g;
        }
      }
      const int stage = n % STAGES;
      mbar_wait(bar_empty(stage), (uint32_t)(((n / STAGES) & 1) ^ 1));
      const uint32_t hi_plane = smem_base + SM_RING + stage * STAGE_BYTES;
      if (ASYNC > 0) {
        asm volatile("cp.async.wait_group %0;" ::"n"(PF) : "memory");
      }
#pragma unroll
      for (int i = 0; i < A_LD; ++i) {
        float4 v = ASYNC > 0 ? lds128(smem_base + SM_STAGING + (n % (ASYNC > 0 ? ASYNC : 1)) * PLANE_BYTES + (ptid + PROD_THREADS * i) * 16)
                             : xa[i];
        if (IN_BN) {
          const int r = prow + ROWS_STEP * i;
          if (k0 < K && r < a.rows_per_group - cp.row0) {
            const float4 A4 = *reinterpret_cast<const float4*>(&sBN[k0]);
            const float4 B4 = *reinterpret_cast<const float4*>(&sBN[MAXK + k0]);
            v.x = fmaxf(fmaf(v.x, A4.x, B4.x), 0.f);
            v.y = fmaxf(fmaf(v.y, A4.y, B4.y), 0.f);
            v.z = fmaxf(fmaf(v.z, A4.z, B4.z), 0.f);
            v.w = fmaxf(fmaf(v.w, A4.w, B4.w), 0.f);
          }
        }
        float4 hi, lo;
        hi.x = tf32_hi(v.x); hi.y = tf32_hi(v.y); hi.z = tf32_hi(v.z); hi.w = tf32_hi(v.w);
        lo.x = __fsub_rn(v.x, hi.x); lo.y = __fsub_rn(v.y, hi.y); lo.z = __fsub_rn(v.z, hi.z); lo.w = __fsub_rn(v.w, hi.w);
        sts128(hi_plane + soff[i], hi);
        sts128(hi_plane + PLANE_BYTES + soff[i], lo);
      }
      fence_proxy_async();
      __syncwarp();
      if (lane == 0) mbar_arrive(bar_full(stage));
      advance(cp);
    };

    if (ASYNC > 0) {
      for (int i = 0; i < PF; ++i) {
        if (i < total) issue(buf[0]);
        asm volatile("cp.async.commit_group;" ::: "memory");
      }
      for (int m = 0; m < total; ++m) {
        if (m + PF < total) issue(buf[0]);
        asm volatile("cp.async.commit_group;" ::: "memory");
        put(buf[0], m);
      }
    } else {
#pragma unroll
      for (int i = 0; i < PF; ++i)
        if (i < total) issue(buf[i]);
      for (int n = 0; n < total; n += PF + 1) {
#pragma unroll
        for (int u = 0; u <= PF; ++u) {
          const int m = n + u;
          if (m < total) {
            if (m + PF < total) issue(buf[ASYNC > 0 ? 0 : (u + PF) % (PF + 1)]);
            put(buf[ASYNC > 0 ? 0 : u], m);
          }
        }
      }
    }
  } else {
    const int wgi = warp >> 2;
    const int frow = wgi * 64 + (warp & 3) * 16 + (lane >> 2);
    const int fcol = 2 * (lane & 3);
    constexpr int ACC_REGS = (STACKED ? 2 * COUT : COUT) / 2;
    constexpr int BLK = COUT < 64 ? COUT : 64;
    float acc[ACC_REGS];
    const uint32_t w_base = smem_base + SM_W;
    double racc = 0.0;
    int acc_g = -1;
    auto flush = [&]() {
      if (a.out_stats != nullptr && acc_g >= 0 && tid < 2 * COUT) atomicAdd(a.out_stats + (size_t)acc_g * 2 * a.cout + tid, racc);
      racc = 0.0;
    };
    int n = 0;
    for (int it = 0; it < tr.count; ++it) {
      const int t = tr.first + it;
      const int g = t / tpg, row0 = (t - g * tpg) * NT;
      const int rows_valid = min(NT, a.rows_per_group - row0);
      const size_t grow0 = (size_t)g * a.rows_per_group + row0;
      if (g != acc_g) {
        flush();
        acc_g = g;
      }
      for (int c = 0; c < nch; ++c, ++n) {
        const int stage = n % STAGES;
        mbar_wait(bar_full(stage), (uint32_t)((n / STAGES) & 1));
        const uint32_t x_hi = smem_base + SM_RING + stage * STAGE_BYTES + wgi * 64 * 128, x_lo = x_hi + PLANE_BYTES;
        const uint32_t w_hi = w_base + c * W_CHUNK, w_lo = w_hi + COUT * 128;
        const int ksteps = min(KC, K - c * KC) / 8;
        fence();
        for (int j = 0; j < ksteps; ++j) {
          const uint32_t first = (c | j) != 0 ? 1u : 0u;
          if (STACKED) {
            mma_tile<2 * COUT, BLK>(acc, x_hi + j * 32, w_hi + j * 32, first);
            mma_tile<COUT, BLK>(acc + COUT / 2, x_lo + j * 32, w_hi + j * 32, 1u);
          } else {
            mma_tile<COUT, BLK>(acc, x_lo + j * 32, w_hi + j * 32, first);
            mma_tile<COUT, BLK>(acc, x_hi + j * 32, w_lo + j * 32, 1u);
            mma_tile<COUT, BLK>(acc, x_hi + j * 32, w_hi + j * 32, 1u);
          }
        }
        commit();
        wait_all();
        fence_regs(acc);
        __syncwarp();
        if (lane == 0) mbar_arrive(bar_empty(stage));
      }
      const bool ok0 = frow < rows_valid, ok1 = frow + 8 < rows_valid;
      float* y0 = a.y + (grow0 + frow) * a.ldy + fcol;
      float* y1 = y0 + (size_t)8 * a.ldy;
#pragma unroll
      for (int i = 0; i < COUT / 8; ++i) {
        float v[4];
#pragma unroll
        for (int e = 0; e < 4; ++e) v[e] = STACKED ? acc[4 * i + e] + acc[COUT / 2 + 4 * i + e] : acc[4 * i + e];
        if (ok0) *reinterpret_cast<float2*>(y0 + 8 * i) = make_float2(v[0], v[1]);
        if (ok1) *reinterpret_cast<float2*>(y1 + 8 * i) = make_float2(v[2], v[3]);
        if (a.out_stats != nullptr) {
          if (!ok0) v[0] = v[1] = 0.f;
          if (!ok1) v[2] = v[3] = 0.f;
          float s[4] = {v[0] + v[2], v[1] + v[3], fmaf(v[0], v[0], v[2] * v[2]), fmaf(v[1], v[1], v[3] * v[3])};
#pragma unroll
          for (int e = 0; e < 4; ++e) {
            s[e] += __shfl_xor_sync(0xffffffffu, s[e], 4);
            s[e] += __shfl_xor_sync(0xffffffffu, s[e], 8);
            s[e] += __shfl_xor_sync(0xffffffffu, s[e], 16);
          }
          if (lane < 4) {
            atomicAdd(&sRed[8 * i + fcol], (double)s[0]);
            atomicAdd(&sRed[8 * i + fcol + 1], (double)s[1]);
            atomicAdd(&sRed[COUT + 8 * i + fcol], (double)s[2]);
            atomicAdd(&sRed[COUT + 8 * i + fcol + 1], (double)s[3]);
          }
        }
      }
      if (a.out_stats != nullptr) {
        named_bar_sync(2, CONS_THREADS);
        if (tid < 2 * COUT) {
          racc += sRed[tid];
          sRed[tid] = 0.0;
        }
        named_bar_sync(2, CONS_THREADS);
      }
    }
    flush();
  }
}

constexpr int DEEP_K = 160;
template <int ASYNC, int NSTAGES>
constexpr int smem_bytes(int cout, int cin) {
  return Layout<ASYNC, NSTAGES>::W + weight_bytes(cout, (cin + KC - 1) / KC) + tail_bytes(cout);
}
constexpr bool fits(int cin, int cout) {
  return cin <= DEEP_K ? (smem_bytes<4, 2>(cout, cin) <= SMEM_MAX && smem_bytes<0, 4>(cout, cin) <= SMEM_MAX)
                       : (smem_bytes<3, 2>(cout, cin) <= SMEM_MAX && smem_bytes<0, 3>(cout, cin) <= SMEM_MAX);
}
static_assert(fits(136, 64) && fits(32, 64) && fits(64, 128) && fits(224, 64) && fits(64, 64) && fits(64, 16),
              "a hot-path GEMM shape no longer fits the shared memory of gemm_ws_kernel");

template <int COUT, bool IN_BN, int ASYNC, int NSTAGES>
static int launch_pf(const GemmArgs& a, cudaStream_t st, const char* name) {
  const int smem_total = smem_bytes<ASYNC, NSTAGES>(COUT, a.cin);
  if (smem_total > SMEM_MAX) return -1;
  static unsigned long long smem_done = 0;
  PMVS_TRY((ensure_dyn_smem(gemm_ws_kernel<COUT, IN_BN, ASYNC, NSTAGES>, SMEM_MAX, smem_done, "gemm_ws")));
  const long long tiles = (long long)a.groups * cdiv(a.rows_per_group, NT);
  const int grid = (int)std::min<long long>(tiles, sm_count());
  prof_begin(name, st);
  gemm_ws_kernel<COUT, IN_BN, ASYNC, NSTAGES><<<grid, THREADS, smem_total, st>>>(a);
  return check_launch("gemm_ws_kernel", st);
}
namespace tma {
constexpr int NT = 64;
constexpr int STAGE_BYTES = NT * KC * 4;
constexpr int CONS_THREADS = 256;
constexpr int THREADS = CONS_THREADS + 64;
constexpr int MAX_STAGES = 32, MIN_STAGES = 8;
constexpr int BN_FLOATS = (MAXK / KC) * 4 * 16;
constexpr int TAIL_BN = 0, TAIL_RED = TAIL_BN + 2 * BN_FLOATS * 4;
__host__ __device__ constexpr int tail_bar(int cout) { return TAIL_RED + 2 * 2 * cout * 8; }
__host__ __device__ constexpr int tail_bytes(int cout) { return tail_bar(cout) + 2 * MAX_STAGES * 8; }
__host__ __device__ constexpr int stages_for(int cin, int cout) {
  return (SMEM_MAX - weight_bytes(cout, (cin + KC - 1) / KC) - tail_bytes(cout)) / STAGE_BYTES < MAX_STAGES
             ? (SMEM_MAX - weight_bytes(cout, (cin + KC - 1) / KC) - tail_bytes(cout)) / STAGE_BYTES
             : MAX_STAGES;
}
}

template <int N>
__device__ __forceinline__ void reduce_scatter_round(float* sv, int lane, int m) {
  const bool up = (lane & m) != 0;
#pragma unroll
  for (int k = 0; k < N / 2; ++k) {
    const float keep = up ? sv[k + N / 2] : sv[k], send = up ? sv[k] : sv[k + N / 2];
    sv[k] = keep + __shfl_xor_sync(0xffffffffu, send, m);
  }
}

template <int COUT, bool IN_BN>
__global__ void __launch_bounds__(tma::THREADS, 1) gemm_tma_kernel(const __grid_constant__ CUtensorMap tmx,
                                                                   const GemmArgs a, const int wstages) {
  constexpr int NT = tma::NT, STAGE_BYTES = tma::STAGE_BYTES, CONS_THREADS = tma::CONS_THREADS;
  constexpr int MAX_STAGES = tma::MAX_STAGES, BN_FLOATS = tma::BN_FLOATS, TAIL_BN = tma::TAIL_BN, TAIL_RED = tma::TAIL_RED;
  constexpr bool STACKED = COUT <= 64;
  constexpr int W_CHUNK = 2 * COUT * 128;
  constexpr int ACC_REGS = (STACKED ? 2 * COUT : COUT) / 2;
  extern __shared__ __align__(1024) unsigned char smem[];
  const uint32_t smem_base = smem_u32(smem);

  const int K = a.cin;
  const int nch = (K + KC - 1) / KC;
  const int tid = threadIdx.x, warp = __shfl_sync(0xffffffffu, tid >> 5, 0), lane = tid & 31;
  const int tpg = (a.rows_per_group + NT - 1) / NT;
  const TileRange tr = my_tiles(a.groups * tpg);
  unsigned char* tail = smem + weight_bytes(COUT, nch) + 2 * wstages * STAGE_BYTES;
  const uint32_t bar0 = smem_u32(tail + tma::tail_bar(COUT));
  auto bar_full = [&](int w, int s) { return bar0 + 8u * (uint32_t)(w * (MAX_STAGES / 2) + s); };
  auto bar_empty = [&](int w, int s) { return bar0 + 8u * (uint32_t)(MAX_STAGES + w * (MAX_STAGES / 2) + s); };

  if (tid == 0) {
    for (int w = 0; w < 2; ++w)
      for (int s = 0; s < wstages; ++s) {
        mbar_init(bar_full(w, s), 1);
        mbar_init(bar_empty(w, s), 4);
      }
    asm volatile("fence.mbarrier_init.release.cluster;" ::: "memory");
  }
  __syncthreads();

  if (warp >= CONS_THREADS / 32) {
    const int w = warp - CONS_THREADS / 32;
    if (lane == 0) {
      const uint32_t ring = smem_base + weight_bytes(COUT, nch) + w * wstages * STAGE_BYTES;
      int stage = 0;
      uint32_t phase = 0;
      for (int i = w; i < tr.count; i += 2) {
        const int t = tr.first + i, g = t / tpg, row0 = (t - g * tpg) * NT;
        for (int c = 0; c < nch; ++c) {
          mbar_wait(bar_empty(w, stage), phase ^ 1u);
          mbar_arrive_expect_tx(bar_full(w, stage), STAGE_BYTES);
          tma_load_3d(ring + stage * STAGE_BYTES, &tmx, c * KC, row0, g, bar_full(w, stage));
          if (++stage == wstages) {
            stage = 0;
            phase ^= 1u;
          }
        }
      }
    }
    return;
  }

  const int wgi = warp >> 2, wtid = tid & 127;
  const uint32_t ring = smem_base + weight_bytes(COUT, nch) + wgi * wstages * STAGE_BYTES;
  float* sBN = (float*)(tail + TAIL_BN) + wgi * BN_FLOATS;
  double* sRed = (double*)(tail + TAIL_RED) + wgi * 2 * COUT;
  for (int i = wtid; i < 2 * COUT; i += 128) sRed[i] = 0.0;
  store_weight_planes<COUT>(smem_base, a.w, K, tid, CONS_THREADS);
  fence_proxy_async();
  named_bar_sync(1, CONS_THREADS);

  const int r = (warp & 3) * 16 + (lane >> 2), q = lane & 3;
  const uint32_t fbase = r * 128 + q * 4, fx = (r & 7) << 4;
  const int frow = r, fcol = 2 * q;
  const uint32_t w_base = smem_base;
  float acc[ACC_REGS];
  uint32_t fh[16], fl[16];
  const uint32_t wg_bar = 2 + wgi;

  constexpr int HC = COUT < 64 ? COUT : 64, NH = COUT / HC;
  constexpr int NV = HC / 16;
  const int kofs = ((lane >> 2) & 1) * (8 * NV / 2) + ((lane >> 3) & 1) * (8 * NV / 4) + ((lane >> 4) & 1) * (8 * NV / 8);
  double racc[NH][NV];
#pragma unroll
  for (int h = 0; h < NH; ++h)
#pragma unroll
    for (int j = 0; j < NV; ++j) racc[h][j] = 0.0;
  auto flush = [&](int g) {
    if (a.out_stats == nullptr) return;
#pragma unroll
    for (int h = 0; h < NH; ++h)
#pragma unroll
      for (int j = 0; j < NV; ++j) {
        const int k = kofs + j, i = (k >> 2) + h * (HC / 8), e = k & 3;
        atomicAdd(&sRed[(e >> 1) * COUT + 8 * i + fcol + (e & 1)], racc[h][j]);
        racc[h][j] = 0.0;
      }
    named_bar_sync(wg_bar, 128);
    for (int s = wtid; s < 2 * COUT; s += 128) {
      atomicAdd(a.out_stats + (size_t)g * 2 * a.cout + s, sRed[s]);
      sRed[s] = 0.0;
    }
  };

  auto chunk = [&](auto KSTEPS, int c, int m) {
    constexpr int ksteps = decltype(KSTEPS)::value;
    const int stage = m % wstages;
    mbar_wait(bar_full(wgi, stage), (uint32_t)((m / wstages) & 1));
    mma_chunk_3xtf32<COUT, IN_BN, ksteps>(acc, fh, fl, ring + stage * STAGE_BYTES + fbase, fx, sBN + (c * 4 + q) * 16,
                                          w_base + c * W_CHUNK, c);
    __syncwarp();
    if (lane == 0) mbar_arrive(bar_empty(wgi, stage));
  };
  auto chunk_ks = [&](int c, int m) {
    switch (min(KC, K - c * KC) / 8) {
      case 4: chunk(std::integral_constant<int, 4>(), c, m); break;
      case 3: chunk(std::integral_constant<int, 3>(), c, m); break;
      case 2: chunk(std::integral_constant<int, 2>(), c, m); break;
      default: chunk(std::integral_constant<int, 1>(), c, m); break;
    }
  };

  int cur_g = -1;
  for (int i = wgi; i < tr.count; i += 2) {
    const int t = tr.first + i;
    const int g = t / tpg, row0 = (t - g * tpg) * NT;
    const int rows_valid = min(NT, a.rows_per_group - row0);
    const size_t grow0 = (size_t)g * a.rows_per_group + row0;
    if (g != cur_g) {
      named_bar_sync(wg_bar, 128);
      if (cur_g >= 0) flush(cur_g);
      if (IN_BN) {
        const double* s = a.in_stats + (size_t)g * 2 * K;
        for (int e = wtid; e < nch * 64; e += 128) {
          const int c = e >> 6, qq = (e >> 4) & 3, k = e & 15, jh = k & 7;
          const int col = c * KC + 8 * (jh >> 1) + qq + 4 * (jh & 1);
          float val = 0.f;
          if (col < K) {
            const BnCoef bc = bn_coef(s[col], s[K + col], a.in_count, a.eps);
            const float A = __fmul_rn(bc.invstd, a.in_gamma[col]);
            val = k < 8 ? A : fmaf(-bc.mean, A, a.in_beta[col]);
          }
          sBN[e] = val;
        }
      }
      named_bar_sync(wg_bar, 128);
      cur_g = g;
    }
    const int m0 = (i >> 1) * nch;
    for (int c = 0; c < nch; ++c) chunk_ks(c, m0 + c);
    fence_regs(acc);
    const bool ok0 = frow < rows_valid, ok1 = frow + 8 < rows_valid;
    float* y0 = a.y + (grow0 + frow) * a.ldy + fcol;
    float* y1 = y0 + (size_t)8 * a.ldy;
#pragma unroll
    for (int h = 0; h < NH; ++h) {
      float sv[HC / 2];
#pragma unroll
      for (int il = 0; il < HC / 8; ++il) {
        const int ii = h * (HC / 8) + il;
        float v[4];
#pragma unroll
        for (int e = 0; e < 4; ++e) v[e] = STACKED ? acc[4 * ii + e] + acc[COUT / 2 + 4 * ii + e] : acc[4 * ii + e];
        if (ok0) *reinterpret_cast<float2*>(y0 + 8 * ii) = make_float2(v[0], v[1]);
        if (ok1) *reinterpret_cast<float2*>(y1 + 8 * ii) = make_float2(v[2], v[3]);
        if (!ok0) v[0] = v[1] = 0.f;
        if (!ok1) v[2] = v[3] = 0.f;
        sv[4 * il + 0] = v[0] + v[2];
        sv[4 * il + 1] = v[1] + v[3];
        sv[4 * il + 2] = fmaf(v[0], v[0], v[2] * v[2]);
        sv[4 * il + 3] = fmaf(v[1], v[1], v[3] * v[3]);
      }
      if (a.out_stats != nullptr) {
        reduce_scatter_round<HC / 2>(sv, lane, 4);
        reduce_scatter_round<HC / 4>(sv, lane, 8);
        reduce_scatter_round<HC / 8>(sv, lane, 16);
#pragma unroll
        for (int j = 0; j < NV; ++j) racc[h][j] += (double)sv[j];
      }
    }
  }
  if (cur_g >= 0) flush(cur_g);
}

static_assert(tma::stages_for(136, 64) >= tma::MIN_STAGES && tma::stages_for(32, 64) >= tma::MIN_STAGES &&
                  tma::stages_for(64, 128) >= tma::MIN_STAGES && tma::stages_for(224, 64) >= tma::MIN_STAGES &&
                  tma::stages_for(64, 64) >= tma::MIN_STAGES && tma::stages_for(64, 16) >= tma::MIN_STAGES,
              "a hot-path GEMM shape no longer gets the minimum ring depth of gemm_tma_kernel");

template <int COUT, bool IN_BN>
static int launch_tma(const GemmArgs& a, cudaStream_t st, const char* name) {
  const int stages = tma::stages_for(a.cin, COUT);
  if (stages < tma::MIN_STAGES) return -1;
  const int wstages = stages / 2;
  const unsigned long long row_bytes = (unsigned long long)a.ldx * 4, group_bytes = row_bytes * a.rows_per_group;
  if (group_bytes >= (1ull << 40) || (unsigned long long)a.groups > 0xffffffffull) return -1;
  EncodeTiledFn enc = encode_tiled_fn();
  if (enc == nullptr) return -1;
  CUtensorMap tm;
  const cuuint64_t gdim[3] = {(cuuint64_t)a.cin, (cuuint64_t)a.rows_per_group, (cuuint64_t)a.groups};
  const cuuint64_t gstr[2] = {row_bytes, group_bytes};
  const cuuint32_t box[3] = {KC, tma::NT, 1};
  const cuuint32_t estr[3] = {1, 1, 1};
  if (enc(&tm, CU_TENSOR_MAP_DATA_TYPE_FLOAT32, 3, const_cast<float*>(a.x), gdim, gstr, box, estr,
          CU_TENSOR_MAP_INTERLEAVE_NONE, CU_TENSOR_MAP_SWIZZLE_128B, CU_TENSOR_MAP_L2_PROMOTION_L2_256B,
          CU_TENSOR_MAP_FLOAT_OOB_FILL_NONE) != CUDA_SUCCESS)
    return -1;
  const int smem_total = weight_bytes(COUT, cdiv(a.cin, KC)) + 2 * wstages * tma::STAGE_BYTES + tma::tail_bytes(COUT);
  static unsigned long long smem_done = 0;
  PMVS_TRY((ensure_dyn_smem(gemm_tma_kernel<COUT, IN_BN>, SMEM_MAX, smem_done, "gemm_tma")));
  const long long tiles = (long long)a.groups * cdiv(a.rows_per_group, tma::NT);
  const int grid = (int)std::min<long long>(tiles, sm_count());
  prof_begin(name, st);
  gemm_tma_kernel<COUT, IN_BN><<<grid, tma::THREADS, smem_total, st>>>(tm, a, wstages);
  return check_launch("gemm_tma_kernel", st);
}

template <int COUT, bool IN_BN>
static int launch_one(const GemmArgs& a, cudaStream_t st, const char* name) {
  if (opt(OPT_GEMM) == 3) {
    const int rc = launch_tma<COUT, IN_BN>(a, st, name);
    if (rc >= 0 || opt(OPT_GEMM_STRICT)) return rc;
  }
  const bool deep = a.cin <= DEEP_K;
  if (opt(OPT_GEMM) == 1)
    return deep ? launch_pf<COUT, IN_BN, 0, 4>(a, st, name) : launch_pf<COUT, IN_BN, 0, 3>(a, st, name);
  return deep ? launch_pf<COUT, IN_BN, 4, 2>(a, st, name) : launch_pf<COUT, IN_BN, 3, 2>(a, st, name);
}

}

static int launch_gemm_ws_any(const GemmArgs& a, cudaStream_t st, const char* name) {
  if (a.cin % 8 != 0 || a.cin > ws::MAXK || a.ldx % 4 != 0 || a.ldy % 2 != 0 || a.groups <= 0 || a.rows_per_group <= 0) return -1;
  if (((uintptr_t)a.x & 15) || ((uintptr_t)a.w & 15) || ((uintptr_t)a.y & 7)) return -1;
  if ((long long)a.groups * cdiv(a.rows_per_group, ws::NT) >= (1ll << 31) / ws::MAXK) return -1;
  const bool bn = a.in_stats != nullptr;
  switch (a.cout) {
    case 16: return bn ? ws::launch_one<16, true>(a, st, name) : ws::launch_one<16, false>(a, st, name);
    case 32: return bn ? ws::launch_one<32, true>(a, st, name) : ws::launch_one<32, false>(a, st, name);
    case 64: return bn ? ws::launch_one<64, true>(a, st, name) : ws::launch_one<64, false>(a, st, name);
    case 128: return bn ? ws::launch_one<128, true>(a, st, name) : ws::launch_one<128, false>(a, st, name);
  }
  return -1;
}

bool gemm_in_bn_fma_form(const GemmArgs& a) {
  if (opt(OPT_GEMM) == 0 || pmvs_get_gemm_mode() != 3) return false;
  if (a.cin % 8 != 0 || a.cin > ws::MAXK || a.ldx % 4 != 0 || a.ldy % 2 != 0 || a.groups <= 0 || a.rows_per_group <= 0) return false;
  if (((uintptr_t)a.x & 15) || ((uintptr_t)a.w & 15) || ((uintptr_t)a.y & 7)) return false;
  if ((long long)a.groups * cdiv(a.rows_per_group, ws::NT) >= (1ll << 31) / ws::MAXK) return false;
  return a.cout == 16 || a.cout == 32 || a.cout == 64 || a.cout == 128;
}

int launch_gemm_ws(const GemmArgs& a, cudaStream_t st, const char* name) {
  const int rc = launch_gemm_ws_any(a, st, name);
  if (rc < 0 && opt(OPT_GEMM) == 3 && opt(OPT_GEMM_STRICT)) {
    set_error("gemm: gemm_tma_kernel does not take cin %d, cout %d, ldx %d, %d groups of %d rows (strict mode)", a.cin,
              a.cout, a.ldx, a.groups, a.rows_per_group);
    return PMVS_ERR_ARG;
  }
  return rc;
}

}
```

pointmvsnet_b200/csrc/wgmma.cuh:

```cuda
#pragma once
#include <stdint.h>

namespace pmvs {
namespace wg {

__device__ __forceinline__ uint32_t smem_u32(const void* p) { return (uint32_t)__cvta_generic_to_shared(p); }
__device__ __forceinline__ void mbar_init(uint32_t bar, uint32_t count) {
  asm volatile("mbarrier.init.shared::cta.b64 [%0], %1;" ::"r"(bar), "r"(count));
}
__device__ __forceinline__ void mbar_wait(uint32_t bar, uint32_t parity) {
  uint32_t done = 0;
  while (!done) {
    asm volatile(
        "{\n\t.reg .pred p;\n\t"
        "mbarrier.try_wait.parity.shared::cta.b64 p, [%1], %2;\n\t"
        "selp.u32 %0, 1, 0, p;\n\t}"
        : "=r"(done)
        : "r"(bar), "r"(parity)
        : "memory");
  }
}
__device__ __forceinline__ void mbar_arrive(uint32_t bar) {
  asm volatile("mbarrier.arrive.shared::cta.b64 _, [%0];" ::"r"(bar) : "memory");
}
__device__ __forceinline__ void fence_proxy_async() { asm volatile("fence.proxy.async.shared::cta;" ::: "memory"); }
__device__ __forceinline__ void named_bar_sync(int id, int nthreads) {
  asm volatile("bar.sync %0, %1;" ::"r"(id), "r"(nthreads) : "memory");
}
__device__ __forceinline__ void mbar_arrive_expect_tx(uint32_t bar, uint32_t bytes) {
  asm volatile("mbarrier.arrive.expect_tx.shared::cta.b64 _, [%0], %1;" ::"r"(bar), "r"(bytes) : "memory");
}
__device__ __forceinline__ void tma_load_3d(uint32_t dst, const void* tmap, int c0, int c1, int c2, uint32_t bar) {
  asm volatile(
      "cp.async.bulk.tensor.3d.shared::cluster.global.mbarrier::complete_tx::bytes [%0], [%1, {%2, %3, %4}], [%5];"
      ::"r"(dst), "l"(tmap), "r"(c0), "r"(c1), "r"(c2), "r"(bar)
      : "memory");
}

__device__ __forceinline__ int swz128(int r, int pc) { return (r >> 3) * 1024 + (r & 7) * 128 + ((pc ^ (r & 7)) << 4); }

__device__ __forceinline__ uint64_t make_desc(uint32_t smem_addr) {
  return (uint64_t)((smem_addr >> 4) & 0x3FFF) | ((uint64_t)1 << 16) | ((uint64_t)(1024 >> 4) << 32) | ((uint64_t)1 << 62);
}

__device__ __forceinline__ void fence() { asm volatile("wgmma.fence.sync.aligned;" ::: "memory"); }
__device__ __forceinline__ void commit() { asm volatile("wgmma.commit_group.sync.aligned;" ::: "memory"); }
__device__ __forceinline__ void wait_all() { asm volatile("wgmma.wait_group.sync.aligned 0;" ::: "memory"); }
template <int R>
__device__ __forceinline__ void fence_regs(float (&d)[R]) {
#pragma unroll
  for (int i = 0; i < R; ++i) asm volatile("" : "+f"(d[i])::"memory");
}

template <int N>
__device__ __forceinline__ void mma_tf32(float* d, uint64_t adesc, uint64_t bdesc, uint32_t accumulate);
template <>
__device__ __forceinline__ void mma_tf32<16>(float* d, uint64_t adesc, uint64_t bdesc, uint32_t accumulate) {
  asm volatile(
      "{\n\t.reg .pred p;\n\tsetp.ne.b32 p, %10, 0;\n\t"
      "wgmma.mma_async.sync.aligned.m64n16k8.f32.tf32.tf32 {"
      "%0, %1, %2, %3, %4, %5, %6, %7}, "
      "%8, %9, p, 1, 1;\n\t}"
      : "+f"(d[0]), "+f"(d[1]), "+f"(d[2]), "+f"(d[3]), "+f"(d[4]), "+f"(d[5]),
        "+f"(d[6]), "+f"(d[7])
      : "l"(adesc), "l"(bdesc), "r"(accumulate));
}
template <>
__device__ __forceinline__ void mma_tf32<32>(float* d, uint64_t adesc, uint64_t bdesc, uint32_t accumulate) {
  asm volatile(
      "{\n\t.reg .pred p;\n\tsetp.ne.b32 p, %18, 0;\n\t"
      "wgmma.mma_async.sync.aligned.m64n32k8.f32.tf32.tf32 {"
      "%0, %1, %2, %3, %4, %5, %6, %7, %8, %9, %10, %11, %12, %13, %14, %15}, "
      "%16, %17, p, 1, 1;\n\t}"
      : "+f"(d[0]), "+f"(d[1]), "+f"(d[2]), "+f"(d[3]), "+f"(d[4]), "+f"(d[5]),
        "+f"(d[6]), "+f"(d[7]), "+f"(d[8]), "+f"(d[9]), "+f"(d[10]), "+f"(d[11]),
        "+f"(d[12]), "+f"(d[13]), "+f"(d[14]), "+f"(d[15])
      : "l"(adesc), "l"(bdesc), "r"(accumulate));
}
template <>
__device__ __forceinline__ void mma_tf32<64>(float* d, uint64_t adesc, uint64_t bdesc, uint32_t accumulate) {
  asm volatile(
      "{\n\t.reg .pred p;\n\tsetp.ne.b32 p, %34, 0;\n\t"
      "wgmma.mma_async.sync.aligned.m64n64k8.f32.tf32.tf32 {"
      "%0, %1, %2, %3, %4, %5, %6, %7, %8, %9, %10, %11, %12, %13, %14, %15, "
      "%16, %17, %18, %19, %20, %21, %22, %23, %24, %25, %26, %27, %28, %29, %30, %31}, "
      "%32, %33, p, 1, 1;\n\t}"
      : "+f"(d[0]), "+f"(d[1]), "+f"(d[2]), "+f"(d[3]), "+f"(d[4]), "+f"(d[5]),
        "+f"(d[6]), "+f"(d[7]), "+f"(d[8]), "+f"(d[9]), "+f"(d[10]), "+f"(d[11]),
        "+f"(d[12]), "+f"(d[13]), "+f"(d[14]), "+f"(d[15]), "+f"(d[16]), "+f"(d[17]),
        "+f"(d[18]), "+f"(d[19]), "+f"(d[20]), "+f"(d[21]), "+f"(d[22]), "+f"(d[23]),
        "+f"(d[24]), "+f"(d[25]), "+f"(d[26]), "+f"(d[27]), "+f"(d[28]), "+f"(d[29]),
        "+f"(d[30]), "+f"(d[31])
      : "l"(adesc), "l"(bdesc), "r"(accumulate));
}

template <int N, int BLK>
__device__ __forceinline__ void mma_tile(float* d, uint32_t a_addr, uint32_t b_addr, uint32_t accumulate) {
  static_assert(N % BLK == 0 && (BLK == 16 || BLK == 32 || BLK == 64), "block shape");
#pragma unroll
  for (int nb = 0; nb < N / BLK; ++nb)
    mma_tf32<BLK>(d + (BLK / 2) * nb, make_desc(a_addr), make_desc(b_addr + nb * BLK * 128), accumulate);
}

template <int N>
__device__ __forceinline__ void wait() { asm volatile("wgmma.wait_group.sync.aligned %0;" ::"n"(N) : "memory"); }
template <int R>
__device__ __forceinline__ void fence_regs(uint32_t (&d)[R]) {
#pragma unroll
  for (int i = 0; i < R; ++i) asm volatile("" : "+r"(d[i])::"memory");
}

template <int N>
__device__ __forceinline__ void mma_tf32_ra(float* d, const uint32_t* a, uint64_t bdesc, uint32_t accumulate);
template <>
__device__ __forceinline__ void mma_tf32_ra<16>(float* d, const uint32_t* a, uint64_t bdesc, uint32_t accumulate) {
  asm volatile(
      "{\n\t.reg .pred p;\n\tsetp.ne.b32 p, %13, 0;\n\t"
      "wgmma.mma_async.sync.aligned.m64n16k8.f32.tf32.tf32 {"
      "%0, %1, %2, %3, %4, %5, %6, %7}, "
      "{%8, %9, %10, %11}, %12, p, 1, 1;\n\t}"
      : "+f"(d[0]), "+f"(d[1]), "+f"(d[2]), "+f"(d[3]), "+f"(d[4]), "+f"(d[5]),
        "+f"(d[6]), "+f"(d[7])
      : "r"(a[0]), "r"(a[1]), "r"(a[2]), "r"(a[3]), "l"(bdesc), "r"(accumulate));
}
template <>
__device__ __forceinline__ void mma_tf32_ra<32>(float* d, const uint32_t* a, uint64_t bdesc, uint32_t accumulate) {
  asm volatile(
      "{\n\t.reg .pred p;\n\tsetp.ne.b32 p, %21, 0;\n\t"
      "wgmma.mma_async.sync.aligned.m64n32k8.f32.tf32.tf32 {"
      "%0, %1, %2, %3, %4, %5, %6, %7, %8, %9, %10, %11, %12, %13, %14, %15}, "
      "{%16, %17, %18, %19}, %20, p, 1, 1;\n\t}"
      : "+f"(d[0]), "+f"(d[1]), "+f"(d[2]), "+f"(d[3]), "+f"(d[4]), "+f"(d[5]),
        "+f"(d[6]), "+f"(d[7]), "+f"(d[8]), "+f"(d[9]), "+f"(d[10]), "+f"(d[11]),
        "+f"(d[12]), "+f"(d[13]), "+f"(d[14]), "+f"(d[15])
      : "r"(a[0]), "r"(a[1]), "r"(a[2]), "r"(a[3]), "l"(bdesc), "r"(accumulate));
}
template <>
__device__ __forceinline__ void mma_tf32_ra<64>(float* d, const uint32_t* a, uint64_t bdesc, uint32_t accumulate) {
  asm volatile(
      "{\n\t.reg .pred p;\n\tsetp.ne.b32 p, %37, 0;\n\t"
      "wgmma.mma_async.sync.aligned.m64n64k8.f32.tf32.tf32 {"
      "%0, %1, %2, %3, %4, %5, %6, %7, %8, %9, %10, %11, %12, %13, %14, %15, "
      "%16, %17, %18, %19, %20, %21, %22, %23, %24, %25, %26, %27, %28, %29, %30, %31}, "
      "{%32, %33, %34, %35}, %36, p, 1, 1;\n\t}"
      : "+f"(d[0]), "+f"(d[1]), "+f"(d[2]), "+f"(d[3]), "+f"(d[4]), "+f"(d[5]),
        "+f"(d[6]), "+f"(d[7]), "+f"(d[8]), "+f"(d[9]), "+f"(d[10]), "+f"(d[11]),
        "+f"(d[12]), "+f"(d[13]), "+f"(d[14]), "+f"(d[15]), "+f"(d[16]), "+f"(d[17]),
        "+f"(d[18]), "+f"(d[19]), "+f"(d[20]), "+f"(d[21]), "+f"(d[22]), "+f"(d[23]),
        "+f"(d[24]), "+f"(d[25]), "+f"(d[26]), "+f"(d[27]), "+f"(d[28]), "+f"(d[29]),
        "+f"(d[30]), "+f"(d[31])
      : "r"(a[0]), "r"(a[1]), "r"(a[2]), "r"(a[3]), "l"(bdesc), "r"(accumulate));
}
template <int N, int BLK>
__device__ __forceinline__ void mma_tile_ra(float* d, const uint32_t* a, uint32_t b_addr, uint32_t accumulate) {
  static_assert(N % BLK == 0 && (BLK == 16 || BLK == 32 || BLK == 64), "block shape");
#pragma unroll
  for (int nb = 0; nb < N / BLK; ++nb) mma_tf32_ra<BLK>(d + (BLK / 2) * nb, a, make_desc(b_addr + nb * BLK * 128), accumulate);
}

__device__ __forceinline__ float tf32_hi(float x) { return __uint_as_float(__float_as_uint(x) & 0xFFFFE000u); }

template <int COUT>
__device__ __forceinline__ void store_weight_planes(uint32_t planes, const float* __restrict__ w, int K, int t,
                                                    int nthreads) {
  const int nch = (K + 31) / 32;
  for (int e = t; e < COUT * nch * 8; e += nthreads) {
    const int n = e / (nch * 8), rem = e - n * (nch * 8), c = rem >> 3, pc = rem & 7;
    const int k0 = c * 32 + pc * 4;
    const float4 v = k0 < K ? __ldg(reinterpret_cast<const float4*>(w + (size_t)n * K + k0)) : make_float4(0.f, 0.f, 0.f, 0.f);
    float4 hi, lo;
    hi.x = tf32_hi(v.x); hi.y = tf32_hi(v.y); hi.z = tf32_hi(v.z); hi.w = tf32_hi(v.w);
    lo.x = __fsub_rn(v.x, hi.x); lo.y = __fsub_rn(v.y, hi.y); lo.z = __fsub_rn(v.z, hi.z); lo.w = __fsub_rn(v.w, hi.w);
    const uint32_t dst = planes + c * (2 * COUT * 128) + swz128(n, pc);
    asm volatile("st.shared.v4.f32 [%0], {%1, %2, %3, %4};" ::"r"(dst), "f"(hi.x), "f"(hi.y), "f"(hi.z), "f"(hi.w) : "memory");
    asm volatile("st.shared.v4.f32 [%0], {%1, %2, %3, %4};" ::"r"(dst + COUT * 128), "f"(lo.x), "f"(lo.y), "f"(lo.z), "f"(lo.w)
                 : "memory");
  }
}

template <int COUT, bool IN_BN, int KSTEPS>
__device__ __forceinline__ void mma_chunk_3xtf32(float* acc, uint32_t (&fh)[16], uint32_t (&fl)[16], uint32_t st,
                                                 uint32_t fx, const float* bn, uint32_t w_hi, int c) {
  constexpr bool STACKED = COUT <= 64;
  constexpr int BLK = COUT < 64 ? COUT : 64;
  float bA[8], bB[8];
  if (IN_BN) {
    const float4* t4 = reinterpret_cast<const float4*>(bn);
    const float4 a0 = t4[0], a1 = t4[1], b0 = t4[2], b1 = t4[3];
    bA[0] = a0.x; bA[1] = a0.y; bA[2] = a0.z; bA[3] = a0.w; bA[4] = a1.x; bA[5] = a1.y; bA[6] = a1.z; bA[7] = a1.w;
    bB[0] = b0.x; bB[1] = b0.y; bB[2] = b0.z; bB[3] = b0.w; bB[4] = b1.x; bB[5] = b1.y; bB[6] = b1.z; bB[7] = b1.w;
  }
#pragma unroll
  for (int j = 0; j < 4; ++j) {
    if (j < KSTEPS) {
#pragma unroll
      for (int h = 0; h < 2; ++h) {
        const uint32_t addr = st + ((uint32_t)((2 * j + h) << 4) ^ fx);
        float v[2];
        asm volatile("ld.shared.f32 %0, [%1];" : "=f"(v[0]) : "r"(addr) : "memory");
        asm volatile("ld.shared.f32 %0, [%1];" : "=f"(v[1]) : "r"(addr + 1024) : "memory");
#pragma unroll
        for (int e = 0; e < 2; ++e) {
          float x = v[e];
          if (IN_BN) x = fmaxf(fmaf(x, bA[2 * j + h], bB[2 * j + h]), 0.f);
          const float hi = tf32_hi(x);
          fh[4 * j + 2 * h + e] = __float_as_uint(hi);
          fl[4 * j + 2 * h + e] = __float_as_uint(__fsub_rn(x, hi));
        }
      }
    }
  }
  fence();
  const uint32_t w_lo = w_hi + COUT * 128;
#pragma unroll
  for (int j = 0; j < 4; ++j) {
    if (j < KSTEPS) {
      const uint32_t first = (c | j) != 0 ? 1u : 0u;
      if (STACKED) {
        mma_tile_ra<2 * COUT, BLK>(acc, &fh[4 * j], w_hi + j * 32, first);
        mma_tile_ra<COUT, BLK>(acc + COUT / 2, &fl[4 * j], w_hi + j * 32, 1u);
      } else {
        mma_tile_ra<COUT, BLK>(acc, &fl[4 * j], w_hi + j * 32, first);
        mma_tile_ra<COUT, BLK>(acc, &fh[4 * j], w_lo + j * 32, 1u);
        mma_tile_ra<COUT, BLK>(acc, &fh[4 * j], w_hi + j * 32, 1u);
      }
    }
  }
  commit();
  wait<0>();
  fence_regs(fh);
  fence_regs(fl);
}

}
}
```

pointmvsnet_b200/point_flow.py:

```python
import ctypes as C

import torch
import torch.nn as nn
from torch.autograd.function import once_differentiable

from . import _lib
from . import networks
from ._lib import lib, check, stream_ptr, ptr, require_cuda, FlowShape, FlowWeights, FlowGrads
from .networks import EdgeConv, EdgeConvNoC
from .nn.mlp import SharedMLP

PYR_KEYS = ("conv1", "conv2", "conv3")
PYR_CH = (16, 32, 64)


def _ratio_for(image_scale, is_test):
    if not is_test:
        return 1
    if image_scale in (0.125,):
        return 1
    if image_scale in (0.25, 0.5, 1.0):
        return int(image_scale * 8)
    raise NotImplementedError("point_flow: image_scale %r (reference supports 0.125, 0.25, 0.5, 1.0)" % (image_scale,))


class PointFlow(nn.Module):
    def __init__(self, flow_channels=(64, 64, 16, 1), k=16, flow_edge_conv=None, flow_mlp=None,
                 update_running_stats=True):
        super(PointFlow, self).__init__()
        if k != 16:
            raise NotImplementedError("PointFlow: k=16 is what the reference hard-wires (model.py:20,23)")
        if tuple(flow_channels) != (64, 64, 16, 1):
            raise NotImplementedError("PointFlow: flow_channels (64, 64, 16, 1) (model.py:18)")
        self.k = k
        if flow_edge_conv is None:
            flow_edge_conv = nn.ModuleList([EdgeConvNoC(136, 32), EdgeConv(32, 32), EdgeConv(64, 64)])
        if flow_mlp is None:
            flow_mlp = nn.Sequential(SharedMLP(32 + 32 * 2 + 64 * 2, flow_channels[:-1]),
                                     nn.Conv1d(flow_channels[-2], flow_channels[-1], 1, bias=False))
        self.flow_edge_conv = flow_edge_conv
        self.flow_mlp = flow_mlp
        self.update_running_stats = update_running_stats
        self._wcache = None
        self._ws = None
        self._cl_cache = None

    EXPECTED_SHAPES = {
        "flow_edge_conv.0.conv1.weight": (32, 136, 1), "flow_edge_conv.0.conv2.weight": (32, 136, 1),
        "flow_edge_conv.0.bn.weight": (32,), "flow_edge_conv.0.bn.bias": (32,),
        "flow_edge_conv.1.conv1.weight": (32, 32, 1), "flow_edge_conv.1.conv2.weight": (32, 32, 1),
        "flow_edge_conv.1.bn.weight": (64,), "flow_edge_conv.1.bn.bias": (64,),
        "flow_edge_conv.2.conv1.weight": (64, 64, 1), "flow_edge_conv.2.conv2.weight": (64, 64, 1),
        "flow_edge_conv.2.bn.weight": (128,), "flow_edge_conv.2.bn.bias": (128,),
        "flow_mlp.0.0.conv.weight": (64, 224, 1), "flow_mlp.0.0.bn.weight": (64,), "flow_mlp.0.0.bn.bias": (64,),
        "flow_mlp.0.1.conv.weight": (64, 64, 1), "flow_mlp.0.1.bn.weight": (64,), "flow_mlp.0.1.bn.bias": (64,),
        "flow_mlp.0.2.conv.weight": (16, 64, 1), "flow_mlp.0.2.bn.weight": (16,), "flow_mlp.0.2.bn.bias": (16,),
        "flow_mlp.1.weight": (1, 16, 1),
    }

    def load_reference_state_dict(self, state_dict):
        sd = {(k[7:] if k.startswith("module.") else k): v for k, v in state_dict.items()}
        own = self.state_dict()
        for k, shape in self.EXPECTED_SHAPES.items():
            if k not in sd:
                raise KeyError("reference checkpoint lacks hot-path key %s" % k)
            if tuple(sd[k].shape) != shape:
                raise ValueError("%s: shape %s, expected %s" % (k, tuple(sd[k].shape), shape))
        self.load_state_dict({k: v for k, v in sd.items() if k in own}, strict=True)
        self._wcache = None
        return self

    def _bn_hyper(self):
        bns = self._bn_modules()
        mom, eps = bns[0].momentum, bns[0].eps
        for bn in bns:
            if bn.momentum != mom or bn.eps != eps:
                raise NotImplementedError("PointFlow: all BatchNorm layers must share momentum and eps "
                                          "(got %r/%r and %r/%r)" % (mom, eps, bn.momentum, bn.eps))
        if mom is None:
            raise NotImplementedError("PointFlow: BatchNorm momentum=None (cumulative moving average) is not supported "
                                      "by the fused path")
        return float(mom), float(eps)

    def _weights(self, device):
        mom, eps = self._bn_hyper()
        key = (str(device), mom, eps) + tuple((p.data_ptr(), p._version) for p in self.parameters())
        if self._wcache is not None and self._wcache[0] == key:
            return self._wcache[1], self._wcache[2]
        keep = []

        def dev(t):
            t = t.detach().to(device=device, dtype=torch.float32).contiguous()
            keep.append(t)
            return t

        w = FlowWeights()
        for l, ec in enumerate(self.flow_edge_conv):
            w12 = dev(torch.cat([ec.conv1.weight.detach()[:, :, 0], ec.conv2.weight.detach()[:, :, 0]], dim=0))
            w.ec_w12[l] = ptr(w12)
            w.ec_gamma[l] = ptr(dev(ec.bn.weight))
            w.ec_beta[l] = ptr(dev(ec.bn.bias))
        mlp = self.flow_mlp[0]
        for l in range(3):
            w.mlp_w[l] = ptr(dev(mlp[l].conv.weight.detach()[:, :, 0]))
            w.mlp_gamma[l] = ptr(dev(mlp[l].bn.weight))
            w.mlp_beta[l] = ptr(dev(mlp[l].bn.bias))
        w.mlp_w[3] = ptr(dev(self.flow_mlp[1].weight.detach()[:, :, 0]))
        w.momentum = mom
        w.eps = eps
        self._wcache = (key, w, keep)
        return w, keep

    def _bn_modules(self):
        return [ec.bn for ec in self.flow_edge_conv] + [self.flow_mlp[0][l].bn for l in range(3)]

    @staticmethod
    def pyramids_to_channels_last(feature_pyramids, out=None):
        levels = [feature_pyramids[k] for k in PYR_KEYS] if isinstance(feature_pyramids, dict) else list(feature_pyramids)
        res = []
        for l, t in enumerate(levels):
            require_cuda(t)
            B, V, Cc, h, w = t.shape
            if Cc != PYR_CH[l]:
                raise RuntimeError("pyramid level %d must have %d channels, got %d" % (l, PYR_CH[l], Cc))
            if t.dtype == torch.float32 and t.permute(0, 1, 3, 4, 2).is_contiguous():
                res.append(t.permute(0, 1, 3, 4, 2))
                continue
            if torch.is_grad_enabled() and t.requires_grad:
                res.append(_ToChannelsLast.apply(t))
                continue
            src = _lib.f32c(t)
            dst = out[l] if out is not None else torch.empty(B, V, h, w, Cc, device=t.device, dtype=torch.float32)
            with torch.cuda.device(t.device):
                check(lib.pmvs_pyramid_to_channels_last(ptr(src), ptr(dst), B * V, Cc, h, w, stream_ptr()))
            res.append(dst)
        return res

    @staticmethod
    def make_shape(B, V, pyr_hw, prev_hw, img_hw, image_scale, is_test, interval_scale=1.0, sub_range=None):
        s = FlowShape()
        s.B, s.V = B, V
        for l in range(3):
            s.pyr_h[l], s.pyr_w[l] = pyr_hw[l]
        s.prev_h, s.prev_w = prev_hw
        s.flow_h, s.flow_w = int(img_hw[0] * image_scale), int(img_hw[1] * image_scale)
        s.image_scale = float(image_scale)
        s.ratio = _ratio_for(image_scale, is_test)
        s.is_test = 1 if is_test else 0
        s.interval_scale = float(interval_scale)
        if sub_range is not None:
            s.sub_begin, s.sub_count = int(sub_range[0]), int(sub_range[1])
            if s.sub_count <= 0 or s.sub_begin < 0 or s.sub_begin + s.sub_count > s.ratio * s.ratio:
                raise RuntimeError("PointFlow: sub_range %r outside the %d sub-clouds" % (sub_range, s.ratio * s.ratio))
        return s

    def _workspace(self, shape, device):
        need = lib.pmvs_point_flow_workspace_bytes(C.byref(shape))
        if need == 0 or self._ws is None or self._ws.numel() < need or self._ws.device != device:
            self._ws = _lib.workspace(need, device)
        return self._ws, need

    def forward(self, estimated_depth_map, interval, image_scale, it=0, *, feature_pyramids, cam_params_list,
                mean, std, is_test=True, img_hw=None, pyramids_channels_last=None, out=None, interval_scale=1.0,
                sub_range=None):
        require_cuda(estimated_depth_map, interval, cam_params_list, mean, std)
        if not self.training:
            raise NotImplementedError("PointFlow implements the reference's inference mode (module.train(), "
                                      "batch-statistics BatchNorm, test.py:58); call .train() on it")
        if torch.is_grad_enabled() and (estimated_depth_map.requires_grad or
                                        any(p.requires_grad for p in self.parameters())):
            if not networks.backward_enabled():
                raise NotImplementedError("pointmvsnet_b200 PointFlow is forward-only; wrap the call in torch.no_grad() "
                                          "(training the flow modules needs the stand-alone operators)")
        given = pyramids_channels_last if pyramids_channels_last is not None else (
            [feature_pyramids[k] for k in PYR_KEYS] if isinstance(feature_pyramids, dict) else list(feature_pyramids))
        grad_call = networks.backward_enabled() and torch.is_grad_enabled() and (
            estimated_depth_map.requires_grad or any(t.requires_grad for t in given) or
            any(p.requires_grad for p in self.parameters()))
        if grad_call:
            if sub_range is not None or _ratio_for(image_scale, is_test) != 1:
                raise NotImplementedError("PointFlow backward: one cloud per call only (the train branch, or the test "
                                          "branch at scale 0.125); got image_scale %r, is_test %r, sub_range %r"
                                          % (image_scale, is_test, sub_range))
            for name, t in (("cam_params_list", cam_params_list), ("interval", interval), ("mean", mean), ("std", std)):
                if t.requires_grad:
                    raise RuntimeError("PointFlow backward: %s requires grad, but the fused path does not "
                                       "differentiate it (the reference's fetch coordinates are under no_grad)" % name)
            if out is not None:
                raise RuntimeError("PointFlow: `out` buffers are for inference (no_grad) calls")
        if pyramids_channels_last is None:
            pyramids_channels_last = self.pyramids_to_channels_last(feature_pyramids)
        pyr = list(pyramids_channels_last)
        if grad_call:
            params = self._grad_params()
            return _PointFlowFn.apply(self, (interval, image_scale, cam_params_list, mean, std, is_test, img_hw,
                                             interval_scale), estimated_depth_map, pyr[0], pyr[1], pyr[2], *params)
        return self._run(estimated_depth_map, interval, image_scale, cam_params_list, mean, std, is_test, img_hw,
                         pyr, out, interval_scale, sub_range, None)

    def _grad_params(self):
        ps = []
        for ec in self.flow_edge_conv:
            ps += [ec.conv1.weight, ec.conv2.weight, ec.bn.weight, ec.bn.bias]
        mlp = self.flow_mlp[0]
        for l in range(3):
            ps += [mlp[l].conv.weight, mlp[l].bn.weight, mlp[l].bn.bias]
        return ps + [self.flow_mlp[1].weight]

    def _run(self, estimated_depth_map, interval, image_scale, cam_params_list, mean, std, is_test, img_hw, pyr, out,
             interval_scale, sub_range, ctx):
        dev = estimated_depth_map.device
        B, V = cam_params_list.shape[:2]
        pyr_hw = [(int(t.shape[2]), int(t.shape[3])) for t in pyr]
        if img_hw is None:
            img_hw = (pyr_hw[0][0] * 2, pyr_hw[0][1] * 2)
        depth = _lib.f32c(estimated_depth_map.detach())
        pyr = [t.detach() for t in pyr]
        self._validate(dev, B, V, pyr, depth, interval, mean, std, cam_params_list)
        shape = self.make_shape(B, V, pyr_hw, tuple(depth.shape[2:]), img_hw, image_scale, is_test, interval_scale,
                                sub_range)
        if ctx is None:
            ws, need = self._workspace(shape, dev)
        else:
            need = lib.pmvs_point_flow_workspace_bytes(C.byref(shape))
            ws = _lib.workspace(need, dev)
        w, keep = self._weights(dev)
        track = self.update_running_stats and self.training
        bns = self._bn_modules()
        for l in range(3):
            w.ec_run_mean[l] = ptr(bns[l].running_mean) if track else None
            w.ec_run_var[l] = ptr(bns[l].running_var) if track else None
            w.mlp_run_mean[l] = ptr(bns[3 + l].running_mean) if track else None
            w.mlp_run_var[l] = ptr(bns[3 + l].running_var) if track else None
            w.ec_nbt[l] = ptr(bns[l].num_batches_tracked) if track else None
            w.mlp_nbt[l] = ptr(bns[3 + l].num_batches_tracked) if track else None
        h, wd = shape.flow_h, shape.flow_w
        if out is None:
            depth_out = torch.empty(B, 1, h, wd, device=dev, dtype=torch.float32)
            prob_out = torch.empty(B, 5, h, wd, device=dev, dtype=torch.float32)
        else:
            depth_out, prob_out = out
            for t, shp in ((depth_out, (B, 1, h, wd)), (prob_out, (B, 5, h, wd))):
                if tuple(t.shape) != shp or t.dtype != torch.float32 or t.device != dev or not t.is_contiguous():
                    raise RuntimeError("PointFlow: `out` tensors must be contiguous fp32 %s on %s" % (shp, dev))
        cams = _lib.f32c(cam_params_list.detach())
        itv = _lib.f32c(interval.detach().reshape(-1))
        mean_c, std_c = _lib.f32c(mean.detach()), _lib.f32c(std.detach())
        pyr_ptrs = (C.c_void_p * 3)(*[t.data_ptr() for t in pyr])
        with torch.cuda.device(dev):
            check(lib.pmvs_point_flow_iter(C.byref(shape), C.byref(w), C.byref(pyr_ptrs), ptr(depth), ptr(cams),
                                           ptr(itv), ptr(mean_c), ptr(std_c), ptr(depth_out), ptr(prob_out),
                                           ptr(ws), need, stream_ptr()))
        self._last = (shape, ws, depth)
        if ctx is not None:
            ctx.fwd_tensors = (depth, pyr[0], pyr[1], pyr[2], cams, itv, mean_c, std_c, ws)
            ctx.fwd = (shape, w, keep, int(B), tuple(depth.shape))
        return depth_out, prob_out

    def _validate(self, dev, B, V, pyr, depth, interval, mean, std, cams):
        for name, t in (("interval", interval), ("mean", mean), ("std", std), ("cam_params_list", cams)):
            if t.device != dev:
                raise RuntimeError("PointFlow: %s is on %s, the depth map on %s" % (name, t.device, dev))
        if tuple(cams.shape[2:]) != (2, 4, 4):
            raise RuntimeError("PointFlow: cam_params_list must be [B,V,2,4,4], got %s" % (tuple(cams.shape),))
        if interval.numel() != B:
            raise RuntimeError("PointFlow: interval has %d elements for batch %d" % (interval.numel(), B))
        if tuple(mean.shape) != (B, 3) or tuple(std.shape) != (B, 3):
            raise RuntimeError("PointFlow: mean / std must be [B,3]")
        if depth.dim() != 4 or depth.shape[0] != B or depth.shape[1] != 1:
            raise RuntimeError("PointFlow: depth map must be [B,1,h,w] with B=%d, got %s" % (B, tuple(depth.shape)))
        for l, t in enumerate(pyr):
            if t.device != dev or t.dtype != torch.float32 or tuple(t.shape[:2]) != (B, V) or t.shape[-1] != PYR_CH[l]:
                raise RuntimeError("PointFlow: pyramid level %d must be fp32 [B=%d,V=%d,h,w,%d] (channels last) on %s, "
                                   "got %s on %s" % (l, B, V, PYR_CH[l], dev, tuple(t.shape), t.device))
        for bn in self._bn_modules():
            for name in ("running_mean", "running_var", "num_batches_tracked"):
                buf = getattr(bn, name)
                if buf is not None and buf.device != dev:
                    raise RuntimeError("PointFlow: module buffers live on %s, inputs on %s (call .to(device))"
                                       % (buf.device, dev))
            if bn.running_mean is not None and (bn.running_mean.dtype != torch.float32 or
                                                bn.num_batches_tracked.dtype != torch.int64):
                raise RuntimeError("PointFlow: BatchNorm buffers must be fp32 / int64")

    def debug_stages(self):
        shape, ws, depth = self._last
        off = (C.c_size_t * 10)()
        check(lib.pmvs_point_flow_debug_offsets(C.byref(shape), C.byref(off)))
        with torch.cuda.device(ws.device):
            check(lib.pmvs_point_flow_debug_feature(C.byref(shape), ptr(depth), ptr(ws), stream_ptr()))
        S = shape.sub_count if shape.sub_count > 0 else shape.ratio * shape.ratio
        hs, wsub = shape.flow_h // shape.ratio, shape.flow_w // shape.ratio
        N = 5 * hs * wsub
        R = S * shape.B * N

        def view(o, cols, dtype=torch.float32):
            nbytes = R * cols * 4
            return ws[o:o + nbytes].view(dtype).view(S, shape.B, N, cols)

        cand = ws[off[8]:off[8] + R * 32].view(torch.int16).view(S, shape.B, N, 16)
        if off[9]:
            idx = view(off[2], 16, torch.int32)
        else:
            c = cand.to(torch.int64) & 0xFFFF
            out = (c & 0x8000) != 0
            j = c & 127
            dd = torch.where(out, j // 25, c // 96) - 2
            dh = torch.where(out, (j % 25) // 5, (c % 96) // 12) - 2
            dw = torch.where(out, j % 5, c % 12) - 2
            n = torch.arange(N, device=ws.device).view(1, 1, N, 1)
            idx = (n + dd * (hs * wsub) + dh * wsub + dw).clamp_(0, N - 1).int()
        return {
            "feature": view(off[0], 136), "xyz": ws[off[1]:off[1] + R * 12].view(torch.float32).view(S, shape.B, 3, N),
            "idx": idx, "cand": cand, "edge": view(off[3], 224), "h2": view(off[4], 16),
            "S": S, "hs": hs, "ws": wsub, "N": N,
        }


class PointFlowPass(object):

    def __init__(self, point_flow, img_scales=(0.125, 0.25, 0.5), inter_scales=(1.0, 0.75, 0.15), is_test=True):
        self.pf = point_flow
        self.img_scales = tuple(img_scales)
        self.inter_scales = tuple(inter_scales)
        self.is_test = is_test
        self.graph = None
        self.static = None

    def run(self, pyramids, coarse_depth, cam_params_list, depth_interval, mean, std, img_hw, cl_buffers=None,
            outs=None):
        pyr_cl = PointFlow.pyramids_to_channels_last(pyramids, out=cl_buffers)
        depth = coarse_depth
        results = []
        for i, (s, isc) in enumerate(zip(self.img_scales, self.inter_scales)):
            depth, prob = self.pf(depth, depth_interval, s, i, interval_scale=isc, feature_pyramids=None, cam_params_list=cam_params_list, mean=mean,
                                  std=std, is_test=self.is_test, img_hw=img_hw, pyramids_channels_last=pyr_cl,
                                  out=None if outs is None else outs[i])
            results.append((depth, prob))
        return results

    def capture(self, example):
        dev = example["coarse_depth"].device
        st = {
            "pyramids": [torch.empty_like(p).copy_(p) for p in example["pyramids"]],
            "coarse_depth": example["coarse_depth"].clone(),
            "cam_params_list": example["cam_params_list"].clone(),
            "depth_interval": example["depth_interval"].clone(),
            "mean": example["mean"].clone(), "std": example["std"].clone(),
        }
        img_hw = example["img_hw"]
        B = st["coarse_depth"].shape[0]
        cl = [torch.empty(p.shape[0], p.shape[1], p.shape[3], p.shape[4], p.shape[2], device=dev) for p in st["pyramids"]]
        outs = []
        for s in self.img_scales:
            h, w = int(img_hw[0] * s), int(img_hw[1] * s)
            outs.append((torch.empty(B, 1, h, w, device=dev), torch.empty(B, 5, h, w, device=dev)))

        def body():
            return self.run(st["pyramids"], st["coarse_depth"], st["cam_params_list"], st["depth_interval"],
                            st["mean"], st["std"], img_hw, cl_buffers=cl, outs=outs)

        side = torch.cuda.Stream(device=dev)
        side.wait_stream(torch.cuda.current_stream(dev))
        with torch.cuda.stream(side):
            body()
            body()
        torch.cuda.current_stream(dev).wait_stream(side)
        torch.cuda.synchronize(dev)
        launches0 = _lib.launch_count()
        g = torch.cuda.CUDAGraph()
        with torch.cuda.graph(g):
            body()
        self.launches_per_pass = _lib.launch_count() - launches0
        self.graph, self.static, self.outs = g, st, outs
        return self

    def copy_inputs(self, inputs, non_blocking=True):
        st = self.static
        for d, s in zip(st["pyramids"], inputs["pyramids"]):
            d.copy_(s, non_blocking=non_blocking)
        for k in ("coarse_depth", "cam_params_list", "depth_interval", "mean", "std"):
            st[k].copy_(inputs[k], non_blocking=non_blocking)

    def replay(self):
        self.graph.replay()
        return self.outs


class _ToChannelsLast(torch.autograd.Function):

    @staticmethod
    def forward(ctx, t):
        B, V, Cc, h, w = t.shape
        ctx.dtype = t.dtype
        src = _lib.f32c(t.detach())
        dst = torch.empty(B, V, h, w, Cc, device=t.device, dtype=torch.float32)
        with torch.cuda.device(t.device):
            check(lib.pmvs_pyramid_to_channels_last(ptr(src), ptr(dst), B * V, Cc, h, w, stream_ptr()))
        return dst

    @staticmethod
    @once_differentiable
    def backward(ctx, g):
        B, V, h, w, Cc = g.shape
        g = _lib.f32c(g)
        out = torch.empty(B, V, Cc, h, w, device=g.device, dtype=torch.float32)
        with torch.cuda.device(g.device):
            check(lib.pmvs_transpose(ptr(g), ptr(out), B * V, h * w, Cc, stream_ptr()))
        return out.to(ctx.dtype)


class _PointFlowFn(torch.autograd.Function):

    @staticmethod
    def forward(ctx, mod, args, depth, pyr0, pyr1, pyr2, *params):
        interval, image_scale, cams, mean, std, is_test, img_hw, interval_scale = args
        ctx.dtypes = (depth.dtype,) + tuple(p.dtype for p in params)
        res = mod._run(depth, interval, image_scale, cams, mean, std, is_test, img_hw, [pyr0, pyr1, pyr2], None,
                       interval_scale, None, ctx)
        ctx.save_for_backward(*ctx.fwd_tensors, *params)
        del ctx.fwd_tensors
        return res

    @staticmethod
    @once_differentiable
    def backward(ctx, g_depth, g_prob):
        saved = ctx.saved_tensors
        depth, p0, p1, p2, cams, itv, mean_c, std_c, ws = saved[:9]
        ps = saved[9:]
        shape, w, keep, B, dshape = ctx.fwd
        dev = depth.device
        need = ctx.needs_input_grad
        gr = FlowGrads()
        grads = [torch.empty(p.shape, device=dev, dtype=torch.float32) if p.dim() != 3 else None for p in ps]
        dw12 = []
        for l in range(3):
            c = ps[4 * l].shape[0]
            t = torch.empty(2 * c, ps[4 * l].shape[1], device=dev, dtype=torch.float32)
            dw12.append(t)
            gr.ec_dw12[l] = t.data_ptr()
            gr.ec_dgamma[l] = grads[4 * l + 2].data_ptr()
            gr.ec_dbeta[l] = grads[4 * l + 3].data_ptr()
        mlp_w = []
        for l in range(3):
            t = torch.empty(ps[12 + 3 * l].shape[:2], device=dev, dtype=torch.float32)
            mlp_w.append(t)
            gr.mlp_dw[l] = t.data_ptr()
            gr.mlp_dgamma[l] = grads[13 + 3 * l].data_ptr()
            gr.mlp_dbeta[l] = grads[14 + 3 * l].data_ptr()
        w3 = torch.empty(ps[21].shape[:2], device=dev, dtype=torch.float32)
        mlp_w.append(w3)
        gr.mlp_dw[3] = w3.data_ptr()
        dpyr = [torch.empty(p.shape, device=dev, dtype=torch.float32) if need[3 + l] else None
                for l, p in enumerate((p0, p1, p2))]
        for l in range(3):
            gr.dpyramids_cl[l] = ptr(dpyr[l])
        ddepth = torch.empty(dshape, device=dev, dtype=torch.float32) if need[2] else None
        gr.ddepth_prev = ptr(ddepth)
        gd = _lib.f32c(g_depth) if g_depth is not None else torch.zeros(B, 1, shape.flow_h, shape.flow_w, device=dev)
        gp = _lib.f32c(g_prob) if g_prob is not None else None
        nbytes = lib.pmvs_point_flow_backward_workspace_bytes(C.byref(shape))
        bws = _lib.workspace(nbytes, dev)
        pyr_ptrs = (C.c_void_p * 3)(p0.data_ptr(), p1.data_ptr(), p2.data_ptr())
        with torch.cuda.device(dev):
            check(lib.pmvs_point_flow_backward(C.byref(shape), C.byref(w), C.byref(pyr_ptrs), ptr(depth), ptr(cams),
                                               ptr(itv), ptr(mean_c), ptr(std_c), ptr(ws), ptr(gd), ptr(gp),
                                               C.byref(gr), ptr(bws), nbytes, stream_ptr()))
        out = []
        for l in range(3):
            c = ps[4 * l].shape[0]
            out += [dw12[l][:c].unsqueeze(-1), dw12[l][c:].unsqueeze(-1), grads[4 * l + 2], grads[4 * l + 3]]
        for l in range(3):
            out += [mlp_w[l].unsqueeze(-1), grads[13 + 3 * l], grads[14 + 3 * l]]
        out.append(w3.unsqueeze(-1))
        out = [g.to(dt) if n else None for g, dt, n in zip(out, ctx.dtypes[1:], need[6:])]
        dd = ddepth.to(ctx.dtypes[0]) if ddepth is not None else None
        return (None, None, dd) + tuple(dpyr) + tuple(out)
```

Before: 1420.

## Fuse central-half BN+ReLU into downstream GEMMs instead of storing to ecat

In forward-only (lean) calls, the edge-tile kernel no longer writes the BN+ReLU'd central halves into the concat buffer. The next EdgeConv GEMM and the first MLP GEMM instead read those columns straight from the raw linear outputs via per-chunk TMA source maps, applying BN+ReLU on the fly inside the 3xTF32 wgmma loader. Layer-1 linear output is parked in the feature buffer so it survives until it is consumed. The aim is to cut global writes and reads of the concat tensor. The cost is an extra kernel template, more per-element BN work in the GEMM inner loop, and a backward that refuses lean forwards.

```diff
diff --git a/include/pmvs_b200.h b/include/pmvs_b200.h
--- a/include/pmvs_b200.h
+++ b/include/pmvs_b200.h
@@ -193,6 +193,7 @@
   int is_test;
   float interval_scale;
   int sub_begin, sub_count;
+  int lean;
 } pmvs_flow_shape;
 
 size_t pmvs_point_flow_workspace_bytes(const pmvs_flow_shape* shape);
@@ -210,6 +211,8 @@
 
 int pmvs_point_flow_debug_feature(const pmvs_flow_shape* shape, const float* depth_prev, void* workspace,
                                   pmvs_stream_t stream);
+
+int pmvs_point_flow_debug_edge(const pmvs_flow_shape* shape, void* workspace, pmvs_stream_t stream);
 
 typedef struct pmvs_flow_grads {
   float* ec_dw12[3];
diff --git a/pointmvsnet_b200/_lib.py b/pointmvsnet_b200/_lib.py
--- a/pointmvsnet_b200/_lib.py
+++ b/pointmvsnet_b200/_lib.py
@@ -33,7 +33,7 @@
         ("B", C.c_int), ("V", C.c_int), ("pyr_h", C.c_int * 3), ("pyr_w", C.c_int * 3),
         ("prev_h", C.c_int), ("prev_w", C.c_int), ("flow_h", C.c_int), ("flow_w", C.c_int),
         ("image_scale", C.c_float), ("ratio", C.c_int), ("is_test", C.c_int), ("interval_scale", C.c_float),
-        ("sub_begin", C.c_int), ("sub_count", C.c_int),
+        ("sub_begin", C.c_int), ("sub_count", C.c_int), ("lean", C.c_int),
     ]
 
 
@@ -130,6 +130,7 @@
 _sig("pmvs_pyramid_to_channels_last", I, [P, P, I, I, I, I, P])
 _sig("pmvs_point_flow_debug_offsets", I, [C.POINTER(FlowShape), C.POINTER(C.c_size_t * 10)])
 _sig("pmvs_point_flow_debug_feature", I, [C.POINTER(FlowShape), P, P, P])
+_sig("pmvs_point_flow_debug_edge", I, [C.POINTER(FlowShape), P, P])
 _sig("pmvs_point_flow_backward_workspace_bytes", C.c_size_t, [C.POINTER(FlowShape)])
 _sig("pmvs_point_flow_backward", I, [C.POINTER(FlowShape), C.POINTER(FlowWeights), C.POINTER(C.c_void_p * 3),
                                      P, P, P, P, P, P, P, P, C.POINTER(FlowGrads), P, C.c_size_t, P])
@@ -149,7 +150,7 @@
     "pmvs_image_conv_keep", "pmvs_image_conv_backward_workspace_bytes", "pmvs_image_conv_backward",
     "pmvs_transpose", "pmvs_idx64_to_idx32", "pmvs_edgeconv_pm", "pmvs_edgeconv_pm_backward_workspace_bytes", "pmvs_edgeconv_pm_backward", "pmvs_linear_pm", "pmvs_point_flow_workspace_bytes",
     "pmvs_point_flow_iter", "pmvs_pyramid_to_channels_last", "pmvs_point_flow_debug_offsets",
-    "pmvs_point_flow_debug_feature", "pmvs_point_flow_backward_workspace_bytes", "pmvs_point_flow_backward",
+    "pmvs_point_flow_debug_feature", "pmvs_point_flow_debug_edge", "pmvs_point_flow_backward_workspace_bytes", "pmvs_point_flow_backward",
     "pmvs_depth_loss", "pmvs_depth_loss_backward",
 ]
 
diff --git a/pointmvsnet_b200/csrc/api.cu b/pointmvsnet_b200/csrc/api.cu
--- a/pointmvsnet_b200/csrc/api.cu
+++ b/pointmvsnet_b200/csrc/api.cu
@@ -181,6 +181,25 @@
   return PMVS_OK;
 }
 
+static bool flow_lean(const pmvs_flow_shape* s) {
+  return s->lean != 0 && opt(OPT_GEMM) == 3 && pmvs_get_gemm_mode() == 3 && opt(OPT_EDGE) != 0;
+}
+
+__global__ void central_halves_kernel(const float* __restrict__ le1, const float* __restrict__ le2,
+                                      const float* __restrict__ coef1, const float* __restrict__ coef2, float* ecat,
+                                      long long rows, int rows_per_group) {
+  const long long total = rows * 96;
+  for (long long o = blockIdx.x * (long long)blockDim.x + threadIdx.x; o < total; o += (long long)gridDim.x * blockDim.x) {
+    const long long r = o / 96;
+    const int c = (int)(o - r * 96), g = (int)(r / rows_per_group);
+    const bool l1 = c < 32;
+    const int cc = l1 ? c : c - 32, cout = l1 ? 32 : 64;
+    const float x = l1 ? le1[r * 64 + cc] : le2[r * 128 + cc];
+    const float* k = (l1 ? coef1 : coef2) + (size_t)g * 6 * cout;
+    ecat[r * 224 + (l1 ? 32 : 96) + cc] = fmaxf(bn_apply(x, k[2 * cout + cc], k[3 * cout + cc], k[4 * cout + cc], k[5 * cout + cc]), 0.f);
+  }
+}
+
 static FusedFetchParams fetch_params(const pmvs_flow_shape* s, const FlowPlan& p, char* ws, const float* depth_prev) {
   FusedFetchParams f{};
   f.src = (const float*)(ws + p.warp_src);
@@ -346,6 +365,21 @@
   PMVS_TRY(make_plan(shape, p));
   PMVS_REQUIRE(depth_prev && workspace, "point_flow_debug_feature: NULL pointer");
   return launch_fused_fetch(fetch_params(shape, p, (char*)workspace, depth_prev), (cudaStream_t)stream);
+}
+
+extern "C" int pmvs_point_flow_debug_edge(const pmvs_flow_shape* shape, void* workspace, pmvs_stream_t stream) {
+  FlowPlan p;
+  PMVS_TRY(make_plan(shape, p));
+  PMVS_REQUIRE(workspace, "point_flow_debug_edge: NULL pointer");
+  if (!flow_lean(shape)) return PMVS_OK;
+  const char* ws = (const char*)workspace;
+  const float* coef = (const float*)(ws + p.coef);
+  const long long R = (long long)p.R;
+  const int grid = (int)std::min<long long>(cdiv(R * 96, 256), sm_count() * 16);
+  central_halves_kernel<<<grid, 256, 0, (cudaStream_t)stream>>>(
+      (const float*)(ws + p.feature), (const float*)(ws + p.le), coef + (size_t)1 * p.S * 6 * 64,
+      coef + (size_t)2 * p.S * 6 * 64, (float*)(ws + p.ecat), R, shape->B * p.N);
+  return check_launch("central_halves_kernel", (cudaStream_t)stream);
 }
 
 extern "C" int pmvs_point_flow_iter(const pmvs_flow_shape* shape, const pmvs_flow_weights* wts,
@@ -381,6 +415,9 @@
   PMVS_TRY(launch_warp_source(pyramids_cl, shape->pyr_h, shape->pyr_w, warp_src, B, shape->V, shape->flow_h,
                               shape->flow_w, st));
   const int edge_impl = opt(OPT_EDGE);
+  const bool lean = flow_lean(shape);
+  float* le1 = lean ? (float*)(ws + p.feature) : le;
+  const float* coef = (const float*)(ws + p.coef);
   const FusedFetchParams f = fetch_params(shape, p, ws, depth_prev);
   bool fused_le0 = false;
   if (opt(OPT_FETCH) == 3 && opt(OPT_GEMM) == 3 && pmvs_get_gemm_mode() == 3 && edge_impl != 0) {
@@ -402,16 +439,26 @@
 
   const int cin[3] = {136, 32, 64}, cout[3] = {32, 32, 64}, in_off[3] = {0, 0, 32}, out_off[3] = {0, 32, 96};
   for (int l = 0; l < 3; ++l) {
+    float* le_l = l == 1 ? le1 : le;
     GemmArgs g{};
     g.x = l == 0 ? feature : ecat + in_off[l];
     g.ldx = l == 0 ? PMVS_FEAT_CH : 224;
-    g.w = wts->ec_w12[l]; g.y = le; g.ldy = 2 * cout[l];
+    g.w = wts->ec_w12[l]; g.y = le_l; g.ldy = 2 * cout[l];
     g.groups = S; g.rows_per_group = rows_per_group; g.cin = cin[l]; g.cout = 2 * cout[l]; g.eps = wts->eps;
     if (edge_impl != 0 && l > 0) g.out_stats = stats + p.st_ec[l];
-    if (l > 0 || !fused_le0) PMVS_TRY(launch_gemm(g, st));
+    if (lean && l == 2) {
+      GemmChunks ch{};
+      ch.nsrc = 2; ch.src[0] = le1; ch.ld[0] = 64; ch.src[1] = ecat; ch.ld[1] = 224;
+      ch.map[0] = 0; ch.col[0] = 0; ch.xf[0] = 0;
+      ch.map[1] = 1; ch.col[1] = 64; ch.xf[1] = -1;
+      ch.coef[0] = coef + (size_t)1 * S * 6 * 64; ch.coef_cout[0] = 32; ch.coef_col[0] = 0;
+      PMVS_TRY(launch_gemm_chunks(g, ch, st, "gemm_64x128"));
+    } else if (l > 0 || !fused_le0) {
+      PMVS_TRY(launch_gemm(g, st));
+    }
     if (edge_impl != 0) {
       EdgeTileArgs e{};
-      e.le = le; e.cand = cand; e.cstats = stats + p.st_ec[l]; e.nstats = stats + p.st_ecn[l];
+      e.le = le_l; e.cand = cand; e.skip_central = lean; e.cstats = stats + p.st_ec[l]; e.nstats = stats + p.st_ecn[l];
       e.coef = (float*)(ws + p.coef) + (size_t)l * S * 6 * 64;
       e.ticket = (unsigned*)(stats + p.st_ticket) + (size_t)l * S;
       e.gamma = wts->ec_gamma[l]; e.beta = wts->ec_beta[l]; e.eps = wts->eps; e.concat_central = l > 0;
@@ -443,7 +490,18 @@
         g.in_count = (double)rows_per_group;
       }
       g.out_stats = stats + p.st_mlp[l];
-      PMVS_TRY(launch_gemm(g, st));
+      if (lean && l == 0) {
+        GemmChunks ch{};
+        ch.nsrc = 3; ch.src[0] = ecat; ch.ld[0] = 224; ch.src[1] = le1; ch.ld[1] = 64; ch.src[2] = le; ch.ld[2] = 128;
+        const int map[7] = {0, 1, 0, 2, 2, 0, 0}, col[7] = {0, 0, 64, 0, 32, 160, 192}, xf[7] = {-1, 0, -1, 1, 2, -1, -1};
+        for (int c = 0; c < 7; ++c) { ch.map[c] = map[c]; ch.col[c] = col[c]; ch.xf[c] = xf[c]; }
+        ch.coef[0] = coef + (size_t)1 * S * 6 * 64; ch.coef_cout[0] = 32; ch.coef_col[0] = 0;
+        ch.coef[1] = coef + (size_t)2 * S * 6 * 64; ch.coef_cout[1] = 64; ch.coef_col[1] = 0;
+        ch.coef[2] = ch.coef[1]; ch.coef_cout[2] = 64; ch.coef_col[2] = 32;
+        PMVS_TRY(launch_gemm_chunks(g, ch, st, "gemm_224x64"));
+      } else {
+        PMVS_TRY(launch_gemm(g, st));
+      }
     }
   }
   HeadArgs h{};
diff --git a/pointmvsnet_b200/csrc/common.cuh b/pointmvsnet_b200/csrc/common.cuh
--- a/pointmvsnet_b200/csrc/common.cuh
+++ b/pointmvsnet_b200/csrc/common.cuh
@@ -159,6 +159,15 @@
 int launch_gemm(const GemmArgs& a, cudaStream_t st);
 int launch_gemm_tc(const GemmArgs& a, cudaStream_t st, const char* name);
 int launch_gemm_ws(const GemmArgs& a, cudaStream_t st, const char* name);
+struct GemmChunks {
+  const float* src[3];
+  int ld[3];
+  int nsrc;
+  int map[7], col[7], xf[7];
+  const float* coef[3];
+  int coef_cout[3], coef_col[3];
+};
+int launch_gemm_chunks(const GemmArgs& a, const GemmChunks& ch, cudaStream_t st, const char* name);
 
 struct EdgeArgs {
   const float* le;
@@ -223,6 +232,7 @@
   const float* beta;
   float eps;
   int concat_central;
+  int skip_central;
   float* out;
   int ldo;
   int groups, clouds_per_group, gh, gw, cout;
diff --git a/pointmvsnet_b200/csrc/edge_tile.cu b/pointmvsnet_b200/csrc/edge_tile.cu
--- a/pointmvsnet_b200/csrc/edge_tile.cu
+++ b/pointmvsnet_b200/csrc/edge_tile.cu
@@ -51,6 +51,7 @@
   const int HW = gh * gw, N = PMVS_NUM_HYP * HW;
   const int rows_per_group = a.clouds_per_group * N;
   const unsigned bar_addr = smem_u32(&bar);
+  const bool store_central = APPLY && a.concat_central && !a.skip_central;
 
   if (tid == 0) {
     asm volatile("mbarrier.init.shared::cta.b64 [%0], 1;" ::"r"(bar_addr));
@@ -178,8 +179,8 @@
         float4 o;
         unpack2(o_lo, o.x, o.y);
         unpack2(o_hi, o.z, o.w);
-        float* orow = a.out + row * a.ldo;
-        if (a.concat_central) {
+        float* orow = a.out + row * a.ldo + (a.concat_central ? COUT : 0);
+        if (store_central) {
           const float4 m = *reinterpret_cast<const float4*>(&coef[2 * COUT + ch0 + cl]);
           const float4 is = *reinterpret_cast<const float4*>(&coef[3 * COUT + ch0 + cl]);
           const float4 gm = *reinterpret_cast<const float4*>(&coef[4 * COUT + ch0 + cl]);
@@ -189,8 +190,7 @@
           c.y = fmaxf(bn_apply(lc.y, m.y, is.y, gm.y, bt.y), 0.f);
           c.z = fmaxf(bn_apply(lc.z, m.z, is.z, gm.z, bt.z), 0.f);
           c.w = fmaxf(bn_apply(lc.w, m.w, is.w, gm.w, bt.w), 0.f);
-          st4(orow + ch0 + cl, c);
-          orow += COUT;
+          st4(orow - COUT + ch0 + cl, c);
         }
         constexpr float rk = 1.f / (float)PMVS_KNN;
         static_assert(PMVS_KNN == 16, "mean over K uses an exact power-of-two reciprocal");
diff --git a/pointmvsnet_b200/csrc/flow_bwd.cu b/pointmvsnet_b200/csrc/flow_bwd.cu
--- a/pointmvsnet_b200/csrc/flow_bwd.cu
+++ b/pointmvsnet_b200/csrc/flow_bwd.cu
@@ -378,6 +378,8 @@
   PMVS_REQUIRE(grads->mlp_dw[3] != nullptr, "point_flow_backward: NULL pointer");
   PMVS_REQUIRE(((uintptr_t)fwd_workspace & 255) == 0, "point_flow_backward: fwd_workspace must be 256-byte aligned");
   PMVS_TRY(check_workspace("point_flow_backward", workspace, workspace_bytes, p.total));
+  PMVS_REQUIRE(shape->lean == 0, "point_flow_backward: the forward was a lean call, which does not keep what the "
+                                 "backward reads");
   (void)cam_params; (void)mean; (void)stdv;
   FlowRegions fr;
   PMVS_TRY(flow_regions(shape, fr));
diff --git a/pointmvsnet_b200/csrc/gemm_ws.cu b/pointmvsnet_b200/csrc/gemm_ws.cu
--- a/pointmvsnet_b200/csrc/gemm_ws.cu
+++ b/pointmvsnet_b200/csrc/gemm_ws.cu
@@ -370,7 +370,13 @@
              ? (SMEM_MAX - weight_bytes(cout, (cin + KC - 1) / KC) - tail_bytes(cout)) / STAGE_BYTES
              : MAX_STAGES;
 }
-}
+constexpr int CENTRAL_SLOTS = 3, CENTRAL_FLOATS = 4 * KC;
+static_assert(CENTRAL_SLOTS * CENTRAL_FLOATS <= BN_FLOATS, "the central-half slots fit a warpgroup's table");
+}
+
+struct TmaMaps {
+  CUtensorMap m[3];
+};
 
 template <int N>
 __device__ __forceinline__ void reduce_scatter_round(float* sv, int lane, int m) {
@@ -382,11 +388,14 @@
   }
 }
 
-template <int COUT, bool IN_BN>
-__global__ void __launch_bounds__(tma::THREADS, 1) gemm_tma_kernel(const __grid_constant__ CUtensorMap tmx,
-                                                                   const GemmArgs a, const int wstages) {
+template <int COUT, bool IN_BN, bool CHUNKS>
+__global__ void __launch_bounds__(tma::THREADS, 1) gemm_tma_kernel(const __grid_constant__ TmaMaps tmx,
+                                                                   const GemmArgs a,
+                                                                   const __grid_constant__ GemmChunks ch,
+                                                                   const int wstages) {
   constexpr int NT = tma::NT, STAGE_BYTES = tma::STAGE_BYTES, CONS_THREADS = tma::CONS_THREADS;
   constexpr int MAX_STAGES = tma::MAX_STAGES, BN_FLOATS = tma::BN_FLOATS, TAIL_BN = tma::TAIL_BN, TAIL_RED = tma::TAIL_RED;
+  static_assert(!CHUNKS || !IN_BN, "per-chunk sources carry their own transform");
   constexpr bool STACKED = COUT <= 64;
   constexpr int W_CHUNK = 2 * COUT * 128;
   constexpr int ACC_REGS = (STACKED ? 2 * COUT : COUT) / 2;
@@ -424,7 +433,8 @@
         for (int c = 0; c < nch; ++c) {
           mbar_wait(bar_empty(w, stage), phase ^ 1u);
           mbar_arrive_expect_tx(bar_full(w, stage), STAGE_BYTES);
-          tma_load_3d(ring + stage * STAGE_BYTES, &tmx, c * KC, row0, g, bar_full(w, stage));
+          tma_load_3d(ring + stage * STAGE_BYTES, &tmx.m[CHUNKS ? ch.map[c] : 0], CHUNKS ? ch.col[c] : c * KC, row0, g,
+                      bar_full(w, stage));
           if (++stage == wstages) {
             stage = 0;
             phase ^= 1u;
@@ -477,21 +487,29 @@
     }
   };
 
-  auto chunk = [&](auto KSTEPS, int c, int m) {
-    constexpr int ksteps = decltype(KSTEPS)::value;
+  auto chunk = [&](auto KSTEPS, auto XFORM, int c, int m) {
+    constexpr int ksteps = decltype(KSTEPS)::value, xf = decltype(XFORM)::value;
     const int stage = m % wstages;
     mbar_wait(bar_full(wgi, stage), (uint32_t)((m / wstages) & 1));
-    mma_chunk_3xtf32<COUT, IN_BN, ksteps>(acc, fh, fl, ring + stage * STAGE_BYTES + fbase, fx, sBN + (c * 4 + q) * 16,
-                                          w_base + c * W_CHUNK, c);
+    const float* bn = xf == XF_BN ? sBN + ch.xf[c] * tma::CENTRAL_FLOATS + q : sBN + (c * 4 + q) * 16;
+    mma_chunk_3xtf32<COUT, xf, ksteps>(acc, fh, fl, ring + stage * STAGE_BYTES + fbase, fx, bn, w_base + c * W_CHUNK, c);
     __syncwarp();
     if (lane == 0) mbar_arrive(bar_empty(wgi, stage));
   };
   auto chunk_ks = [&](int c, int m) {
+    using XF0 = std::integral_constant<int, IN_BN ? XF_FMA : XF_NONE>;
+    if constexpr (CHUNKS) {
+      if (ch.xf[c] >= 0)
+        chunk(std::integral_constant<int, 4>(), std::integral_constant<int, XF_BN>(), c, m);
+      else
+        chunk(std::integral_constant<int, 4>(), XF0(), c, m);
+      return;
+    }
     switch (min(KC, K - c * KC) / 8) {
-      case 4: chunk(std::integral_constant<int, 4>(), c, m); break;
-      case 3: chunk(std::integral_constant<int, 3>(), c, m); break;
-      case 2: chunk(std::integral_constant<int, 2>(), c, m); break;
-      default: chunk(std::integral_constant<int, 1>(), c, m); break;
+      case 4: chunk(std::integral_constant<int, 4>(), XF0(), c, m); break;
+      case 3: chunk(std::integral_constant<int, 3>(), XF0(), c, m); break;
+      case 2: chunk(std::integral_constant<int, 2>(), XF0(), c, m); break;
+      default: chunk(std::integral_constant<int, 1>(), XF0(), c, m); break;
     }
   };
 
@@ -518,6 +536,14 @@
           sBN[e] = val;
         }
       }
+      if (CHUNKS) {
+        for (int e = wtid; e < tma::CENTRAL_SLOTS * tma::CENTRAL_FLOATS; e += 128) {
+          const int sl = e / tma::CENTRAL_FLOATS, kind = (e / KC) & 3, col = e % KC;
+          if (ch.coef[sl] == nullptr) continue;
+          const int cc = ch.coef_cout[sl];
+          sBN[e] = ch.coef[sl][(size_t)g * 6 * cc + (2 + kind) * cc + ch.coef_col[sl] + col];
+        }
+      }
       named_bar_sync(wg_bar, 128);
       cur_g = g;
     }
@@ -561,32 +587,40 @@
                   tma::stages_for(64, 128) >= tma::MIN_STAGES && tma::stages_for(224, 64) >= tma::MIN_STAGES &&
                   tma::stages_for(64, 64) >= tma::MIN_STAGES && tma::stages_for(64, 16) >= tma::MIN_STAGES,
               "a hot-path GEMM shape no longer gets the minimum ring depth of gemm_tma_kernel");
-
-template <int COUT, bool IN_BN>
-static int launch_tma(const GemmArgs& a, cudaStream_t st, const char* name) {
+static bool encode_rows(CUtensorMap* tm, const float* x, int cols, int ld, const GemmArgs& a,
+                        CUtensorMapL2promotion promotion) {
+  const unsigned long long row_bytes = (unsigned long long)ld * 4, group_bytes = row_bytes * a.rows_per_group;
+  if (group_bytes >= (1ull << 40) || (unsigned long long)a.groups > 0xffffffffull) return false;
+  EncodeTiledFn enc = encode_tiled_fn();
+  if (enc == nullptr) return false;
+  const cuuint64_t gdim[3] = {(cuuint64_t)cols, (cuuint64_t)a.rows_per_group, (cuuint64_t)a.groups};
+  const cuuint64_t gstr[2] = {row_bytes, group_bytes};
+  const cuuint32_t box[3] = {KC, tma::NT, 1};
+  const cuuint32_t estr[3] = {1, 1, 1};
+  return enc(tm, CU_TENSOR_MAP_DATA_TYPE_FLOAT32, 3, const_cast<float*>(x), gdim, gstr, box, estr,
+             CU_TENSOR_MAP_INTERLEAVE_NONE, CU_TENSOR_MAP_SWIZZLE_128B, promotion,
+             CU_TENSOR_MAP_FLOAT_OOB_FILL_NONE) == CUDA_SUCCESS;
+}
+
+template <int COUT, bool IN_BN, bool CHUNKS = false>
+static int launch_tma(const GemmArgs& a, cudaStream_t st, const char* name, const GemmChunks& ch = GemmChunks{}) {
   const int stages = tma::stages_for(a.cin, COUT);
   if (stages < tma::MIN_STAGES) return -1;
   const int wstages = stages / 2;
-  const unsigned long long row_bytes = (unsigned long long)a.ldx * 4, group_bytes = row_bytes * a.rows_per_group;
-  if (group_bytes >= (1ull << 40) || (unsigned long long)a.groups > 0xffffffffull) return -1;
-  EncodeTiledFn enc = encode_tiled_fn();
-  if (enc == nullptr) return -1;
-  CUtensorMap tm;
-  const cuuint64_t gdim[3] = {(cuuint64_t)a.cin, (cuuint64_t)a.rows_per_group, (cuuint64_t)a.groups};
-  const cuuint64_t gstr[2] = {row_bytes, group_bytes};
-  const cuuint32_t box[3] = {KC, tma::NT, 1};
-  const cuuint32_t estr[3] = {1, 1, 1};
-  if (enc(&tm, CU_TENSOR_MAP_DATA_TYPE_FLOAT32, 3, const_cast<float*>(a.x), gdim, gstr, box, estr,
-          CU_TENSOR_MAP_INTERLEAVE_NONE, CU_TENSOR_MAP_SWIZZLE_128B, CU_TENSOR_MAP_L2_PROMOTION_L2_256B,
-          CU_TENSOR_MAP_FLOAT_OOB_FILL_NONE) != CUDA_SUCCESS)
+  TmaMaps maps{};
+  if (CHUNKS) {
+    for (int i = 0; i < ch.nsrc; ++i)
+      if (!encode_rows(&maps.m[i], ch.src[i], ch.ld[i], ch.ld[i], a, CU_TENSOR_MAP_L2_PROMOTION_L2_128B)) return -1;
+  } else if (!encode_rows(&maps.m[0], a.x, a.cin, a.ldx, a, CU_TENSOR_MAP_L2_PROMOTION_L2_256B)) {
     return -1;
+  }
   const int smem_total = weight_bytes(COUT, cdiv(a.cin, KC)) + 2 * wstages * tma::STAGE_BYTES + tma::tail_bytes(COUT);
   static unsigned long long smem_done = 0;
-  PMVS_TRY((ensure_dyn_smem(gemm_tma_kernel<COUT, IN_BN>, SMEM_MAX, smem_done, "gemm_tma")));
+  PMVS_TRY((ensure_dyn_smem(gemm_tma_kernel<COUT, IN_BN, CHUNKS>, SMEM_MAX, smem_done, "gemm_tma")));
   const long long tiles = (long long)a.groups * cdiv(a.rows_per_group, tma::NT);
   const int grid = (int)std::min<long long>(tiles, sm_count());
   prof_begin(name, st);
-  gemm_tma_kernel<COUT, IN_BN><<<grid, tma::THREADS, smem_total, st>>>(tm, a, wstages);
+  gemm_tma_kernel<COUT, IN_BN, CHUNKS><<<grid, tma::THREADS, smem_total, st>>>(maps, a, ch, wstages);
   return check_launch("gemm_tma_kernel", st);
 }
 
@@ -626,6 +660,25 @@
   return a.cout == 16 || a.cout == 32 || a.cout == 64 || a.cout == 128;
 }
 
+int launch_gemm_chunks(const GemmArgs& a, const GemmChunks& ch, cudaStream_t st, const char* name) {
+  bool ok = a.cin % ws::KC == 0 && a.cin <= ws::MAXK && a.groups > 0 && a.rows_per_group > 0 &&
+            ((uintptr_t)a.w & 15) == 0 && a.ldy % 2 == 0 && ((uintptr_t)a.y & 7) == 0 &&
+            (long long)a.groups * cdiv(a.rows_per_group, ws::NT) < (1ll << 31) / ws::MAXK && a.in_stats == nullptr &&
+            ch.nsrc >= 1 && ch.nsrc <= 3 && (a.cout == 64 || a.cout == 128);
+  for (int i = 0; ok && i < ch.nsrc; ++i) ok = ch.src[i] && ((uintptr_t)ch.src[i] & 15) == 0 && ch.ld[i] % 4 == 0;
+  for (int c = 0; ok && c < a.cin / ws::KC; ++c) {
+    ok = ch.map[c] >= 0 && ch.map[c] < ch.nsrc && ch.col[c] >= 0 && ch.col[c] + ws::KC <= ch.ld[ch.map[c]] &&
+         ch.xf[c] >= -1 && ch.xf[c] < 3 && (ch.xf[c] < 0 || ch.coef[ch.xf[c]] != nullptr);
+  }
+  const int rc = !ok ? -1
+                 : a.cout == 64 ? ws::launch_tma<64, false, true>(a, st, name, ch)
+                                : ws::launch_tma<128, false, true>(a, st, name, ch);
+  if (rc >= 0) return rc;
+  set_error("gemm: the per-chunk-source contraction does not take cin %d, cout %d, %d groups of %d rows", a.cin,
+            a.cout, a.groups, a.rows_per_group);
+  return PMVS_ERR_ARG;
+}
+
 int launch_gemm_ws(const GemmArgs& a, cudaStream_t st, const char* name) {
   const int rc = launch_gemm_ws_any(a, st, name);
   if (rc < 0 && opt(OPT_GEMM) == 3 && opt(OPT_GEMM_STRICT)) {
diff --git a/pointmvsnet_b200/csrc/wgmma.cuh b/pointmvsnet_b200/csrc/wgmma.cuh
--- a/pointmvsnet_b200/csrc/wgmma.cuh
+++ b/pointmvsnet_b200/csrc/wgmma.cuh
@@ -178,13 +178,14 @@
   }
 }
 
-template <int COUT, bool IN_BN, int KSTEPS>
+constexpr int XF_NONE = 0, XF_FMA = 1, XF_BN = 2;
+template <int COUT, int XF, int KSTEPS>
 __device__ __forceinline__ void mma_chunk_3xtf32(float* acc, uint32_t (&fh)[16], uint32_t (&fl)[16], uint32_t st,
                                                  uint32_t fx, const float* bn, uint32_t w_hi, int c) {
   constexpr bool STACKED = COUT <= 64;
   constexpr int BLK = COUT < 64 ? COUT : 64;
   float bA[8], bB[8];
-  if (IN_BN) {
+  if (XF == XF_FMA) {
     const float4* t4 = reinterpret_cast<const float4*>(bn);
     const float4 a0 = t4[0], a1 = t4[1], b0 = t4[2], b1 = t4[3];
     bA[0] = a0.x; bA[1] = a0.y; bA[2] = a0.z; bA[3] = a0.w; bA[4] = a1.x; bA[5] = a1.y; bA[6] = a1.z; bA[7] = a1.w;
@@ -202,7 +203,11 @@
 #pragma unroll
         for (int e = 0; e < 2; ++e) {
           float x = v[e];
-          if (IN_BN) x = fmaxf(fmaf(x, bA[2 * j + h], bB[2 * j + h]), 0.f);
+          if (XF == XF_FMA) x = fmaxf(fmaf(x, bA[2 * j + h], bB[2 * j + h]), 0.f);
+          if (XF == XF_BN) {
+            const int k = 8 * j + 4 * h;
+            x = fmaxf(bn_apply(x, bn[k], bn[32 + k], bn[64 + k], bn[96 + k]), 0.f);
+          }
           const float hi = tf32_hi(x);
           fh[4 * j + 2 * h + e] = __float_as_uint(hi);
           fl[4 * j + 2 * h + e] = __float_as_uint(__fsub_rn(x, hi));
diff --git a/pointmvsnet_b200/point_flow.py b/pointmvsnet_b200/point_flow.py
--- a/pointmvsnet_b200/point_flow.py
+++ b/pointmvsnet_b200/point_flow.py
@@ -219,6 +219,7 @@
         self._validate(dev, B, V, pyr, depth, interval, mean, std, cam_params_list)
         shape = self.make_shape(B, V, pyr_hw, tuple(depth.shape[2:]), img_hw, image_scale, is_test, interval_scale,
                                 sub_range)
+        shape.lean = 1 if ctx is None else 0
         if ctx is None:
             ws, need = self._workspace(shape, dev)
         else:
@@ -288,6 +289,7 @@
         off = (C.c_size_t * 10)()
         check(lib.pmvs_point_flow_debug_offsets(C.byref(shape), C.byref(off)))
         with torch.cuda.device(ws.device):
+            check(lib.pmvs_point_flow_debug_edge(C.byref(shape), ptr(ws), stream_ptr()))
             check(lib.pmvs_point_flow_debug_feature(C.byref(shape), ptr(depth), ptr(ws), stream_ptr()))
         S = shape.sub_count if shape.sub_count > 0 else shape.ratio * shape.ratio
         hs, wsub = shape.flow_h // shape.ratio, shape.flow_w // shape.ratio
```

After: 1459 (median of 6 runs). +2.7%, better.
